# pydata/sparse

Hardware: AMD Instinct MI355X
Metric: GCXS x dense SpMM throughput (GFLOP/s) (higher is better)
Workload: dtype f32; 1 GPU; GCXS(CSR) 1000000x10000 @ 0.01 (100000000 nnz, int32 idx) in 1 nnz-balanced row block(s) x dense 10000x128 fp32; world_size=1, rows_rank0=1000000, idx_dtype=int32, parallelism=row-block x1, mul_add=fma, nan_warning=deferred, prewarm_products=40, default_settings=NAN_WARNING="sync" (verdict read inside every product), kernel=spmm_tiled (cached block stream)

## Files before the change

sparse_amd/_kernels.py:

```python
import os

import numpy as np
import torch

from . import _ffi
from ._device import code_of, np_dtype, ptr, require_hip, stream_ptr, torch_dtype


def dot_dtype(dt1, dt2):
    return (np.zeros((), dtype=np_dtype(dt1)) * np.zeros((), dtype=np_dtype(dt2))).dtype


_COMPLEX_CODE = {torch.complex64: _ffi.C64, torch.complex128: _ffi.C128}


def product_code(dt):
    dt = torch_dtype(dt)
    code = _COMPLEX_CODE.get(dt)
    return code_of(dt) if code is None else code


def _as_reals(t):
    return torch.view_as_real(t).reshape(-1) if t.is_complex() else t

# ... 1310 lines not shown

def csr_tiled_layout(a_data, a_indices, a_indptr, M, Kd, force_sort=False, dtype=None, defer_check=False, balance=None):
    dev = require_hip(a_data, a_indices, a_indptr)
    if dtype is None:
        dtype = a_data.dtype if a_data.dtype in TILED_DTYPES else torch.float32
    dtype = torch_dtype(dtype)
    vc = code_of(_tiled_layout_dtype(dtype))
    rg, kb, gpb, epb, slack, direct_max, _ = tiled_params(dtype)
    nnz = int(a_data.numel())
    ntiles = -(-Kd // kb)
    groups = -(-(-(-M // rg)) // gpb) * gpb
    nseg = groups * ntiles
    s = stream_ptr(dev)
    vals = a_data.to(dtype).contiguous()
    if dtype == torch.int32:
        vals = vals.view(torch.float32)
    if not index_dtype_ok(a_indices) or a_indices.dtype != a_indptr.dtype:
        a_indices, a_indptr = a_indices.to(torch.int64), a_indptr.to(torch.int64)

    def finish(blk_off, fill):
        total = int(blk_off[-1])
        if total >= 2 ** 31:
            raise ValueError("tiled SpMM layout: more than 2^31 blocks")
        blocks = torch.empty((total + slack) * 16, dtype=torch.int32, device=dev)
        fill(blk_off, total, blocks)
        return TiledLayout(blocks, convert(blk_off, torch.int32), dtype, total / max(nseg, 1))

    may_balance = (ntiles <= direct_max and not force_sort and TILED_ONE_PASS_INSPECTOR and TILED_BALANCE and balance is not False
                   and nnz >= TILED_BALANCE_MIN_NNZ and 0 < M < 2 ** 31)
    if may_balance and (balance or not defer_check):
        lay = _balanced_tiled_layout(vals, a_indices.contiguous(), a_indptr.contiguous(), M, Kd, dtype, nnz, defer_check, dev, s)
        if lay is not None:
            return lay
        may_balance = False
    if ntiles <= direct_max and not force_sort and TILED_ONE_PASS_INSPECTOR:
        ic = code_of(a_indices.dtype)
        ind, ptr_ = a_indices.contiguous(), a_indptr.contiguous()
        upper = -(-nnz // epb) + nseg
        if upper < 2 ** 31:
            blocks = torch.empty((upper + slack) * 16, dtype=torch.int32, device=dev)
            blk_off = torch.empty(groups * (ntiles + 1), dtype=torch.int32, device=dev)
            state = torch.empty(9, dtype=torch.int64, device=dev)
            _ffi.call("spamd_spmm_tiled_inspect", vc, ic, M, Kd, ptr(vals), ptr(ind), ptr(ptr_), ptr(state), ptr(blk_off),
                      ptr(blocks), s)
            if defer_check:
                lay = TiledLayout(blocks, blk_off, dtype, nnz / epb / max(nseg, 1) + 0.5, group_ends=True, pending=state)
                if may_balance:
                    _ffi.call("spamd_spmm_tiled_map_stats", ic, M, Kd, 32, ptr(ptr_), None, None, ptr(state) + 8, s)
                    lay.skew_mean = nnz * rg / max(M, 1)
                return lay
            if int(state[0]) == 0:
                return TiledLayout(blocks, blk_off, dtype, nnz / epb / max(nseg, 1) + 0.5, group_ends=True)
    elif ntiles <= direct_max and not force_sort:
        nblk = torch.empty(nseg + 1, dtype=torch.int64, device=dev)
        flags = torch.empty(1, dtype=torch.int32, device=dev)
        ic = code_of(a_indices.dtype)
        ind, ptr_ = a_indices.contiguous(), a_indptr.contiguous()
        _ffi.call("spamd_spmm_tiled_count", vc, ic, M, Kd, ptr(ind), ptr(ptr_), ptr(nblk), ptr(flags), s)
        blk_off = exclusive_scan(nblk)
        if int(flags[0]) == 0:
            return finish(blk_off, lambda bo, total, blocks: _ffi.call(
                "spamd_spmm_tiled_fill", vc, ic, M, Kd, ptr(vals), ptr(ind), ptr(ptr_), ptr(bo), total, ptr(blocks), s))
    rc = csr_to_keys(a_indptr, a_indices, M, Kd)
    tk = torch.empty_like(rc)
    _ffi.call("spamd_spmm_tiled_keys", nnz, ptr(rc), Kd, ptr(tk), s)
    del rc
    tk, vals = sort_key_value(tk, vals, max(nseg * rg * kb - 1, 1))
    seg_start = torch.empty(nseg + 1, dtype=torch.int64, device=dev)
    nblk = torch.empty(nseg + 1, dtype=torch.int64, device=dev)
    _ffi.call("spamd_spmm_tiled_lists", vc, nnz, ptr(tk), M, Kd, ptr(seg_start), ptr(nblk), s)
    return finish(exclusive_scan(nblk), lambda bo, total, blocks: _ffi.call(
        "spamd_spmm_tiled_pack", vc, nnz, ptr(tk), ptr(vals), ptr(seg_start), ptr(bo), total, ptr(blocks), s))


TILED_BALANCE = True
TILED_BALANCE_MIN_NNZ = 1 << 20
TILED_BALANCE_SKEW = 1.6
TILED_BALANCE_CAPMUL = 2
TILED_BALANCE_STATS = {}


def _balanced_tiled_layout(vals, ind, ptr_, M, Kd, dtype, nnz, defer_check, dev, s):
    rg, kb, gpb, epb, slack, direct_max, _ = tiled_params(dtype)
    ntiles = -(-Kd // kb)
    ic, vc = code_of(ind.dtype), code_of(_tiled_layout_dtype(dtype))
    mean_group = nnz * rg / max(M, 1)
    cap = 32
    while cap < TILED_BALANCE_CAPMUL * mean_group:
        cap *= 2
    stats = torch.empty(8, dtype=torch.int64, device=dev)
    _ffi.call("spamd_spmm_tiled_map_stats", ic, M, Kd, cap, ptr(ptr_), None, None, ptr(stats), s)
    st = stats.tolist()
    skew = st[6] / max(mean_group, 1.0)
    TILED_BALANCE_STATS.update(cap=cap, class_rows=st[:6], natural_max_group=st[6], skew=skew, balanced=False)
    if skew <= TILED_BALANCE_SKEW:
        return None
    keys = torch.empty(M, dtype=torch.int64, device=dev)
    rows = torch.empty(M, dtype=torch.int32, device=dev)
    _ffi.call("spamd_spmm_tiled_map_stats", ic, M, Kd, cap, ptr(ptr_), ptr(keys), ptr(rows), ptr(stats), s)
    st = stats.tolist()
    TILED_BALANCE_STATS.update(class_rows=st[:6])
    counts = _harr64(st[:6])
    groups = int(_ffi.lib().spamd_spmm_tiled_map_groups(counts))
    nseg = groups * ntiles
    upper = -(-nnz // epb) + nseg
    if groups <= 0 or upper >= 2 ** 31:
        return None
    keys, rows = sort_key_value(keys, rows, max(Kd, 1))
    rowmap = torch.empty(groups * rg + 16, dtype=torch.int32, device=dev)
    gload = torch.empty(groups + 1, dtype=torch.int64, device=dev)
    _ffi.call("spamd_spmm_tiled_map_build", ic, M, cap, ptr(ptr_), ptr(rows), counts, ptr(rowmap), ptr(gload), s)
    vstart = exclusive_scan(gload)
    blocks = torch.empty((upper + slack) * 16, dtype=torch.int32, device=dev)
    blk_off = torch.empty(groups * (ntiles + 1), dtype=torch.int32, device=dev)
    state = torch.empty(1, dtype=torch.int64, device=dev)
    _ffi.call("spamd_spmm_tiled_inspect_mapped", vc, ic, M, Kd, groups, ptr(vals), ptr(ind), ptr(ptr_), ptr(rowmap), ptr(vstart),
              ptr(state), ptr(blk_off), ptr(blocks), s)
    TILED_BALANCE_STATS.update(balanced=True, groups=groups)
    lay = TiledLayout(blocks, blk_off, dtype, nnz / epb / max(nseg, 1) + 0.5, group_ends=True, pending=state if defer_check else None,
                      rowmap=rowmap, groups=groups)
    if not defer_check and int(state[0]) != 0:
        return None
    return lay


def csc_tiled_layout(a_data, a_indices, a_indptr, M, Kd, dtype=None):
    dev = require_hip(a_data, a_indices, a_indptr)
    if dtype is None:
        dtype = a_data.dtype if a_data.dtype in TILED_DTYPES else torch.float32
    dtype = torch_dtype(dtype)
    rg, kb, gpb, epb, slack, direct_max, _ = tiled_params(dtype)
    nnz = int(a_data.numel())
    ntiles = -(-Kd // kb)
    groups = -(-(-(-M // rg)) // gpb) * gpb
    nseg = groups * ntiles
    upper = -(-nnz // epb) + nseg
    if ntiles > direct_max or upper >= 2 ** 31 or groups == 0 or not TILED_ONE_PASS_INSPECTOR:
        return None
    if not index_dtype_ok(a_indices) or a_indices.dtype != a_indptr.dtype:
        a_indices, a_indptr = a_indices.to(torch.int64), a_indptr.to(torch.int64)
    vals = a_data.to(dtype).contiguous()
    if dtype == torch.int32:
        vals = vals.view(torch.float32)
    blocks = torch.empty((upper + slack) * 16, dtype=torch.int32, device=dev)
    blk_off = torch.empty(groups * (ntiles + 1), dtype=torch.int32, device=dev)
    split = torch.empty(int(_ffi.lib().spamd_spmm_tiled_inspect_csc_ws(M, Kd)), dtype=torch.int32, device=dev)
    state = torch.empty(1, dtype=torch.int64, device=dev)
    _ffi.call("spamd_spmm_tiled_inspect_csc", code_of(_tiled_layout_dtype(dtype)), code_of(a_indices.dtype), M, Kd, ptr(vals),
              ptr(a_indices.contiguous()), ptr(a_indptr.contiguous()), ptr(split), ptr(state), ptr(blk_off), ptr(blocks),
              stream_ptr(dev))
    return TiledLayout(blocks, blk_off, dtype, nnz / epb / max(nseg, 1) + 0.5, group_ends=True, pending=state)


def dot_csr_ndarray_tiled(layout, out_shape, Kd, b, out=None, exact=False):
    blocks, blk_off, dtype = layout
    M, N = int(out_shape[0]), int(b.shape[1])
    Nout = int(out_shape[1])
    panel = 64 if dtype == torch.float64 else 128
    if N % panel or not (N - panel < Nout <= N):
        raise ValueError(f"tiled executor: B has {N} columns (whole {panel}-column panels expected), result {Nout}")
    last_cols = (Nout - (N - panel)) % panel
    dev = require_hip(blocks, blk_off, b)
    if b.dtype != dtype:
        raise TypeError(f"tiled layout holds {dtype} values, B is {b.dtype}")
    b = b.contiguous()
    if out is None:
        out = torch.empty((M, Nout), dtype=dtype, device=dev)
    lists = max(int(blk_off.numel()) - 1, 1)
    mean_blocks = getattr(layout, "mean_blocks", None) or (int(blocks.numel()) // 16) / lists
    hint = min(64, max(6, int(1.5 * mean_blocks) + 3))
    if _TOUCH_OVERRIDE:
        hint = _TOUCH_OVERRIDE
    ends = _ffi.TILED_GROUP_ENDS if getattr(layout, "group_ends", False) else 0
    ints = _ffi.TILED_INT32 if dtype == torch.int32 else 0
    flags = (_ffi.EXACT_MULADD if exact and not ints else 0) | ends | ints | (hint << 8) | (last_cols << 16)
    rowmap = getattr(layout, "rowmap", None)
    if rowmap is not None:
        _ffi.call("spamd_spmm_tiled_mapped", code_of(_tiled_layout_dtype(dtype)), M, int(layout.groups), Kd, N, ptr(blocks), ptr(blk_off),
                  ptr(rowmap), ptr(b), N, ptr(out), Nout, flags, stream_ptr(dev))
    else:
        _ffi.call("spamd_spmm_tiled", code_of(_tiled_layout_dtype(dtype)), M, Kd, N, ptr(blocks), ptr(blk_off), ptr(b), N, ptr(out), Nout,
                  flags, stream_ptr(dev))
    pending = getattr(layout, "pending", None)
    if pending is not None:
        layout.pending = None
        words = pending.tolist()
        mean = getattr(layout, "skew_mean", None)
        if mean and len(words) >= 8 and words[7] > TILED_BALANCE_SKEW * max(mean, 1.0):
            layout.rebalance = True
        if int(words[0]) != 0:
            raise UnsortedColumns("tiled layout built from rows with unsorted column indices")
    return out
```

sparse_amd/csrc/build.py:

```python
import concurrent.futures as cf
import glob
import os
import shutil
import subprocess
import sys

HERE = os.path.dirname(os.path.abspath(__file__))
PKG = os.path.dirname(HERE)
OUT_DIR = os.path.join(PKG, "_lib")
OBJ_DIR = os.path.join(OUT_DIR, "obj")
LIB = os.path.join(OUT_DIR, "libsparse_amd.so")
ARCH = "gfx950"
CXXFLAGS = [
    f"--offload-arch={ARCH}", "-O3", "-std=c++17", "-fPIC", "-ffp-contract=off",
    "-fno-gpu-rdc", "-Wall", "-Wno-unused-function", "-Wno-unused-variable",
]


def _hipcc():
    for c in (os.environ.get("HIPCC"), shutil.which("hipcc"), "/opt/rocm/bin/hipcc"):
        if c and os.path.exists(c):
            return c
    raise RuntimeError("hipcc not found (need ROCm to build libsparse_amd.so)")


def sources():
    return sorted(glob.glob(os.path.join(HERE, "*.hip")))


def _deps():
    return sorted(glob.glob(os.path.join(HERE, "*.h"))) + sorted(glob.glob(os.path.join(HERE, "*.inc"))) + [
        os.path.join(os.path.dirname(PKG), "include", "sparse_amd.h"), os.path.abspath(__file__)]


def is_stale():
    if not os.path.exists(LIB):
        return True
    t = os.path.getmtime(LIB)
    return any(os.path.getmtime(p) > t for p in sources() + _deps())


def _own_deps(src, obj):
    dep = obj[:-2] + ".d"
    if not os.path.exists(dep):
        return _deps()
    words = open(dep).read().replace("\\\n", " ").split()
    files = [w for w in words[1:] if not w.startswith("/opt/") and not w.startswith("/usr/")]
    if any(not os.path.exists(f) for f in files):
        return _deps()
    return files + [os.path.abspath(__file__)]


NO_SPILL = {"spmm_tiled.hip": "spmm_tiled_kernel"}


def _spills(remarks, needle):
    out, name, sg = [], None, 0
    for ln in remarks.splitlines():
        if "Function Name:" in ln:
            name = ln.split("Function Name:")[1].split()[0]
        elif "SGPRs Spill:" in ln:
            sg = int(ln.split("SGPRs Spill:")[1].split()[0])
        elif "VGPRs Spill:" in ln and name is not None:
            vg = int(ln.split("VGPRs Spill:")[1].split()[0])
            if needle in name and (sg or vg):
                out.append((name, sg, vg))
    return out


def _compile(src, force):
    obj = os.path.join(OBJ_DIR, os.path.basename(src)[:-4] + ".o")
    newest = max(os.path.getmtime(p) for p in [src] + _own_deps(src, obj))
    if not force and os.path.exists(obj) and os.path.getmtime(obj) >= newest:
        return obj, ""
    needle = NO_SPILL.get(os.path.basename(src))
    extra = ["-Rpass-analysis=kernel-resource-usage"] if needle else []
    cmd = [_hipcc(), *CXXFLAGS, *extra, "-MD", "-MF", obj[:-2] + ".d", "-c", src, "-o", obj]
    r = subprocess.run(cmd, capture_output=True, text=True)
    if r.returncode != 0:
        raise RuntimeError(f"hipcc failed for {src}:\n{' '.join(cmd)}\n{r.stdout}\n{r.stderr}")
    if needle:
        bad = _spills(r.stderr, needle)
        if bad:
            os.remove(obj)
            raise RuntimeError(f"{os.path.basename(src)}: the compiler spilled registers in " +
                               ", ".join(f"{n[:60]} ({s} SGPR, {v} VGPR)" for n, s, v in bad[:4]) +
                               " - refused (see NO_SPILL in sparse_amd/csrc/build.py)")
        return obj, "\n".join(ln for ln in r.stderr.splitlines() if "-Rpass-analysis" not in ln and "remark:" not in ln)
    return obj, r.stderr


def build(force=False, verbose=False, jobs=None):
    if not force and not is_stale():
        return LIB
    os.makedirs(OBJ_DIR, exist_ok=True)
    srcs = sources()
    jobs = jobs or min(len(srcs), os.cpu_count() or 1)
    with cf.ThreadPoolExecutor(max_workers=jobs) as ex:
        results = list(ex.map(lambda s: _compile(s, force), srcs))
    objs = [o for o, _ in results]
    if verbose:
        for _, w in results:
            if w.strip():
                print(w, file=sys.stderr)
    cmd = [_hipcc(), f"--offload-arch={ARCH}", "-shared", "-fPIC", "-o", LIB + ".tmp", *objs]
    r = subprocess.run(cmd, capture_output=True, text=True)
    if r.returncode != 0:
        raise RuntimeError(f"link failed:\n{' '.join(cmd)}\n{r.stdout}\n{r.stderr}")
    os.replace(LIB + ".tmp", LIB)
    return LIB


if __name__ == "__main__":
    p = build(force="--force" in sys.argv, verbose=True)
    print(p)
```

sparse_amd/csrc/spmm_tiled.hip:

```cpp
#include "common.h"
#include "spmm_tiled_asm.inc"
#include <stdlib.h>
#include <mutex>
#include <set>

namespace spamd {

constexpr int TL_RG = TL_ASM_RG;
constexpr int TL_WAVES = TL_ASM_WAVES;
#ifndef SPAMD_TL_EXPERIMENTAL
static_assert(TL_RG == 35 && TL_WAVES == 16, "experimental tiled-SpMM geometry: build with -DSPAMD_TL_EXPERIMENTAL");
#endif
constexpr int TL_KB = TL_ASM_KB;
constexpr int TL_NBUF = 2;
__host__ __device__ constexpr int tl_d0(int lc, int lr) { return ((lc >> 1) << 11) | ((lc & 1) << 9) | (2 + 2 * lr); }
constexpr int TL_BLOCK_INTS = 16;

template <typename T>
struct TlFmt;
template <>
struct TlFmt<float> {
  static constexpr int EPB = 8, PANEL = 128;
  __device__ static void put(int* stream, int64_t entry, int d0, float v) {
    int* b = stream + (entry / EPB) * TL_BLOCK_INTS + (entry % EPB) * 2;
// ... 156 lines not shown
}

template <typename I, typename T, bool MAPPED>
__global__ void __launch_bounds__(256) tl_inspect_kernel(int64_t M, int ntiles, int64_t groups, const T* __restrict__ vals,
                                                         const I* __restrict__ indices, const I* __restrict__ indptr,
                                                         unsigned long long* __restrict__ state, int* __restrict__ blk_off,
                                                         int* __restrict__ stream, const int* __restrict__ rowmap,
                                                         const int64_t* __restrict__ vstart) {
  extern __shared__ int tl_fill_lds[];
  __shared__ __attribute__((aligned(16))) int64_t rsab[2 * (TL_RG + 1)];
  __shared__ int wtot[5];
  __shared__ int group_bad;
  constexpr int EPB = TlFmt<T>::EPB;
  int* const before = tl_fill_lds;
  int* const runstart = before + TL_RG * ntiles;
  int* const loff = runstart + TL_RG * ntiles;
  const int tid = threadIdx.x;
  const int64_t g = blockIdx.x;
  const int64_t r0 = g * TL_RG;
  if (tid < TL_RG) {
    if constexpr (MAPPED) {
      const int r = rowmap[r0 + tid];
      rsab[2 * (tid)] = r >= 0 ? (int64_t)indptr[r] : 0;
      rsab[2 * (tid) + 1] = r >= 0 ? (int64_t)indptr[r + 1] : 0;
    } else {
      const int64_t r = r0 + tid;
      rsab[2 * (tid)] = (int64_t)indptr[r < M ? r : M];
      rsab[2 * (tid) + 1] = (int64_t)indptr[r + 1 < M ? r + 1 : M];
    }
  }
  for (int i = tid; i < TL_RG * ntiles; i += 256) before[i] = 0;
  if (tid == 0) group_bad = 0;
  __syncthreads();
  const int64_t e0 = MAPPED ? vstart[g] : rsab[2 * (0)], e1 = MAPPED ? vstart[g + 1] : rsab[2 * (TL_RG - 1) + 1];
  bool bad = false;
  constexpr int RPW = (TL_RG + 3) / 4;
  constexpr int TL_PRE = 2;
  const int wv = tid >> 6, lane = tid & 63;
  unsigned cpre[RPW][TL_PRE];
  T vpre[RPW][TL_PRE];
#pragma unroll
  for (int i = 0; i < RPW; ++i) {
    const int lr = wv + 4 * i;
    const int64_t ra = lr < TL_RG ? rsab[2 * (lr)] : 0, rb = lr < TL_RG ? rsab[2 * (lr) + 1] : 0;
#pragma unroll
    for (int p = 0; p < TL_PRE; ++p) {
      const int64_t e = ra + lane + 64 * p;
      cpre[i][p] = e < rb ? (unsigned)indices[e] : 0xffffffffu;
      vpre[i][p] = e < rb ? vals[e] : T(0);
    }
  }
  auto count_one = [&](int lr, int64_t ra, int64_t e, unsigned c, unsigned cp, bool row_start) {
    const int t = (int)(c / (unsigned)TL_KB);
    atomicAdd(&before[lr * ntiles + t], 1);
    if (!row_start && cp > c) bad = true;
    if (row_start || (int)(cp / (unsigned)TL_KB) != t) runstart[lr * ntiles + t] = (int)(e - (MAPPED ? ra : e0));
  };
#pragma unroll
  for (int i = 0; i < RPW; ++i) {
    const int lr = wv + 4 * i;
    if (lr >= TL_RG) break;
    const int64_t ra = rsab[2 * (lr)], rb = rsab[2 * (lr) + 1];
#pragma unroll
    for (int p = 0; p < TL_PRE; ++p) {
      const int64_t e = ra + lane + 64 * p;
      const unsigned c = cpre[i][p];
      unsigned cp = (unsigned)__shfl_up((int)c, 1, 64);
      if (p > 0) {
        const unsigned last = (unsigned)__builtin_amdgcn_readlane((int)cpre[i][p > 0 ? p - 1 : 0], 63);
        if (lane == 0) cp = last;
      }
      if (e < rb) count_one(lr, ra, e, c, cp, p == 0 && lane == 0);
    }
    for (int64_t e = ra + lane + 64 * TL_PRE; e < rb; e += 64)
      count_one(lr, ra, e, (unsigned)indices[e], (unsigned)indices[e - 1], false);
  }
  if (bad) {
    atomicOr(&state[0], 1ull);
    group_bad = 1;
  }
  __syncthreads();
  int nb = 0, cnt_t = 0;
  for (int t = tid; t < ntiles; t += 256) {
    int c[TL_RG];
#pragma unroll
    for (int lr = 0; lr < TL_RG; ++lr) c[lr] = before[lr * ntiles + t];
    int run = 0;
#pragma unroll
    for (int lr = 0; lr < TL_RG; ++lr) {
      before[lr * ntiles + t] = run;
      run += c[lr];
    }
    cnt_t = run;
    nb = (run + EPB - 1) / EPB;
  }
  const int wid = wv;
  int x = nb;
#pragma unroll
  for (int d = 1; d < 64; d <<= 1) {
    const int y = __shfl_up(x, d, 64);
    if (lane >= d) x += y;
  }
  if (lane == 63) wtot[wid] = x;
  __syncthreads();
  int woff = 0;
  for (int w = 0; w < wid; ++w) woff += wtot[w];
  const int gtotal = wtot[0] + wtot[1] + wtot[2] + wtot[3];
  const int my_off = woff + x - nb;
  const int64_t goff = tl_group_first_block(e0, g, ntiles, EPB);
  const int64_t gnext = tl_group_first_block(e1, g + 1, ntiles, EPB);
  if (tid < ntiles) loff[tid] = my_off;
  __syncthreads();
  if (tid < ntiles) blk_off[g * (ntiles + 1) + tid] = (int)(goff + my_off);
  if (tid == 0) blk_off[g * (ntiles + 1) + ntiles] = (int)(goff + gtotal);
  for (int64_t i = (goff + gtotal) * TL_BLOCK_INTS + tid; i < gnext * TL_BLOCK_INTS; i += 256) stream[i] = 0;
  if (group_bad) {
    for (int64_t i = goff * TL_BLOCK_INTS + tid; i < (goff + gtotal) * TL_BLOCK_INTS; i += 256) stream[i] = 0;
    return;
  }
  auto fill_one = [&](int lr, int64_t ra, int64_t e, unsigned c, T v) {
    const int t = (int)(c / (unsigned)TL_KB);
    const int lc = (int)(c - (unsigned)t * (unsigned)TL_KB);
    const int64_t dst = (goff + loff[t]) * EPB + before[lr * ntiles + t] + ((int)(e - (MAPPED ? ra : e0)) - runstart[lr * ntiles + t]);
    TlFmt<T>::put(stream, dst, tl_d0(lc, lr), v);
  };
#pragma unroll
  for (int i = 0; i < RPW; ++i) {
    const int lr = wv + 4 * i;
    if (lr >= TL_RG) break;
    const int64_t ra = rsab[2 * (lr)], rb = rsab[2 * (lr) + 1];
#pragma unroll
    for (int p = 0; p < TL_PRE; ++p) {
      const int64_t e = ra + lane + 64 * p;
      if (e < rb) fill_one(lr, ra, e, cpre[i][p], vpre[i][p]);
    }
    for (int64_t e = ra + lane + 64 * TL_PRE; e < rb; e += 64) fill_one(lr, ra, e, (unsigned)indices[e], vals[e]);
  }
  if (tid < ntiles) {
    const int64_t first = (goff + my_off) * EPB;
    for (int i = cnt_t; i < nb * EPB; ++i) TlFmt<T>::put(stream, first + i, 0, T(0));
  }
}

__device__ __forceinline__ void tl_dma16(unsigned lds_base, const void* src) {
  asm volatile("s_mov_b32 m0, %0\n\ts_nop 0\n\tglobal_load_lds_dwordx4 %1, off"
               :
               : "s"(lds_base), "v"(src)
               : "memory", "m0");
}

template <int MODE>
__device__ __forceinline__ void tl_phases(const int* stream, int t0, int te, int o0, int o1, int o2, int offreg, int obase,
                                          int ntiles, int nfull, int toff, int mask, unsigned m0wave,
                                          unsigned row_step, int voff, tl_srd_t srd, unsigned& soff) {
  const int lane = threadIdx.x & 63;
  const unsigned blo = (unsigned)((uintptr_t)stream & 0xffffffffu), bhi = (unsigned)((uintptr_t)stream >> 32);
  const int lane8 = lane * 8;
#define TL_PHASES_OPERANDS                                                                                        \
  [soff] "+s"(soff)                                                                                               \
  : [blo] "s"(blo), [bhi] "s"(bhi), [t0] "s"(t0), [te] "s"(te), [o0] "s"(o0), [o1] "s"(o1), [o2] "s"(o2),         \
    [obase] "s"(obase), [ntiles] "s"(ntiles), [nfull] "s"(nfull), [m0wave] "s"(m0wave), [step] "s"(row_step),      \
    [toff] "v"(toff), [lane8] "v"(lane8), [mask] "v"(mask), [offreg] "v"(offreg), [voff] "v"(voff), [srd] "s"(srd)  \
  : "memory", "m0", "scc", "vcc", TL_CLOB_SGPR, TL_CLOB_TMP, TL_CLOB_ACC
  if (MODE == 6)
    asm volatile(TL_ASM_PHASES_I32 : TL_PHASES_OPERANDS);
  else if (MODE == 4)
    asm volatile(TL_ASM_PHASES_F64 : TL_PHASES_OPERANDS);
  else if (MODE == 5)
    asm volatile(TL_ASM_PHASES_F64_EXACT : TL_PHASES_OPERANDS);
  else if (MODE == 3)
    asm volatile(TL_ASM_PHASES_EXACT : TL_PHASES_OPERANDS);
  else if (MODE == 1)
    asm volatile(TL_ASM_PHASES_NOFMA : TL_PHASES_OPERANDS);
  else if (MODE == 2)
    asm volatile(TL_ASM_PHASES_NOLDS : TL_PHASES_OPERANDS);
  else
    asm volatile(TL_ASM_PHASES : TL_PHASES_OPERANDS);
#undef TL_PHASES_OPERANDS
}

__device__ __forceinline__ void tl_block_map(unsigned L, int npanels, int nblocks, int& bx, int& by) {
  const unsigned pin = npanels > 1 ? 2u : 1u;
  const unsigned per_chunk = (unsigned)((nblocks + 7) / 8) * 8u * pin;
  const unsigned chunk = L / per_chunk, l = L % per_chunk;
  const unsigned seq = l >> 3;
  by = uniform((int)(chunk * pin + seq % pin));
  bx = uniform((int)((seq / pin) * 8u + (l & 7u)));
}

template <int DBG, int MODE, typename T>
__global__ void __launch_bounds__(TL_WAVES * 64) __attribute__((amdgpu_num_vgpr(TL_ASM_COMP)))
spmm_tiled_kernel(int64_t M, int64_t K, int ntiles, int touch_lines, const int* __restrict__ stream,
                  const int* __restrict__ blk_off, const T* __restrict__ b, int64_t ldb,
                  T* __restrict__ out, int64_t ldo, int last_cols, int npanels, int nblocks, const int* __restrict__ rowmap) {
  constexpr int PANEL = TlFmt<T>::PANEL;
  constexpr int CPL = PANEL / 64;
  extern __shared__ __attribute__((aligned(16))) char lds[];
  const int tid = threadIdx.x;
  const int lane = tid & 63;
  const int wv = uniform(tid >> 6);
  int bx, by;
  tl_block_map(blockIdx.x, npanels, nblocks, bx, by);
  if (bx >= nblocks || by >= npanels) return;
  const int g = bx * TL_WAVES + wv;
  b += (int64_t)by * PANEL;
  out += (int64_t)by * PANEL;

  asm volatile(TL_ASM_ZERO ::: "memory", TL_CLOB_ACC);

  const int nfull = DBG == 2 ? 0 : (int)(K / TL_KB);
  const unsigned row_step = (unsigned)((2 * TL_WAVES) * ldb * (int64_t)sizeof(T));
  const unsigned m0wave = (unsigned)wv * 2048u;
  const uint64_t bbase = (uint64_t)(uintptr_t)b;
  tl_srd_t srd;
  srd[0] = (int)(bbase & 0xffffffffu);
  srd[1] = (int)((bbase >> 32) & 0xffffu);
  srd[2] = (int)0xffffffffu;
  srd[3] = 0x00020000;
  const int voff = (int)((int64_t)(tid >> 5) * ldb * (int64_t)sizeof(T)) + (tid & 31) * 16;
  unsigned soff = 0;
  auto issue_partial = [&](int t) {
#pragma unroll
    for (int i = 0; i < TL_DMA_PER_TILE; ++i) {
      const int e = (i * (TL_WAVES * 64) + tid) * 16;
      int64_t r = (int64_t)t * TL_KB + (e >> 9);
      if (r >= K) r = K - 1;
      tl_dma16(((unsigned)(i * TL_WAVES + wv) * 2u + (unsigned)(t & 1)) * 1024u,
               reinterpret_cast<const char*>(b + r * ldb) + (e & 511));
    }
  };
  const bool has_partial = DBG != 2 && (int64_t)nfull * TL_KB < K;

  if (nfull > 0)
    asm volatile(TL_ASM_TILE0 : [soff] "+s"(soff) : [m0wave] "s"(m0wave), [step] "s"(row_step), [voff] "v"(voff), [srd] "s"(srd) : "memory", "m0", "scc", "vcc", "s89");
  else if (has_partial)
    issue_partial(0);
  asm volatile("s_waitcnt vmcnt(0)" ::: "memory");
  __syncthreads();

  const int* const myoff = blk_off + (int64_t)g * (ntiles + (touch_lines >> 16));
  touch_lines &= 0xffff;
  const int toff = (lane < touch_lines ? lane : touch_lines - 1) * 64;
  int t = 0;
  while (t < ntiles) {
    const int obase = t;
    const int q = obase + lane;
    int offreg = myoff[q < ntiles ? q : ntiles];
    asm volatile("" : "+v"(offreg));
    int te = obase + 61 < ntiles ? obase + 61 : ntiles;
    if (has_partial && t < nfull - 1 && nfull - 1 < te) te = nfull - 1;
    if (has_partial && t == nfull - 1) issue_partial(nfull);
    auto o = [&](int tt) { return wave_bcast(offreg, (tt < ntiles ? tt : ntiles) - obase); };
    const int o0 = o(t), o1 = o(t + 1), o2 = o(t + 2);
    if (t == 0) {
      const int n = o2 - o0, l = lane < n ? lane : 0;
      asm volatile("global_load_dword " TL_ASM_TOUCH ", %0, off" ::"v"(reinterpret_cast<const char*>(stream + (int64_t)o0 * 16) + l * 64)
                   : "memory", TL_ASM_TOUCH);
    }
    tl_phases<MODE>(stream, t, te, o0, o1, o2, offreg, obase, ntiles, nfull, toff, (int)0xfffffe00, m0wave, row_step, voff, srd, soff);
    t = te;
  }
  asm volatile("s_waitcnt vmcnt(0) lgkmcnt(0)" ::: "memory");

  const int64_t row0 = (int64_t)g * TL_RG;
  const int64_t left = M - row0;
  const int nvalid = left <= 0 ? 0 : (left < TL_RG ? (int)left : TL_RG);
  T* const obase_p = out + row0 * ldo + lane * CPL;
  const int64_t stride_bytes = ldo * (int64_t)sizeof(T);
  int bx2, by2;
  tl_block_map(blockIdx.x, npanels, nblocks, bx2, by2);
  const int ncols = (last_cols > 0 && by2 == npanels - 1) ? last_cols : PANEL;
  if (rowmap) {
    const int* const rm = rowmap + (int64_t)g * TL_RG;
    T* const base_p = out + lane * CPL;
    if (lane * CPL + CPL <= ncols)
      asm volatile(TL_ASM_STORE_PERM
                   :
                   : [lo] "v"((unsigned)((uintptr_t)base_p & 0xffffffffu)), [hi] "v"((unsigned)((uintptr_t)base_p >> 32)),
                     [stride] "s"((unsigned)stride_bytes), [rm] "s"(rm)
                   : "memory", "scc", TL_CLOB_SGPR, TL_CLOB_TMP, TL_CLOB_ACC);
    if constexpr (CPL == 2) {
      if (lane * CPL + 1 == ncols)
        asm volatile(TL_ASM_STORE1_PERM
                     :
                     : [lo] "v"((unsigned)((uintptr_t)base_p & 0xffffffffu)), [hi] "v"((unsigned)((uintptr_t)base_p >> 32)),
                       [stride] "s"((unsigned)stride_bytes), [rm] "s"(rm)
                     : "memory", "scc", TL_CLOB_SGPR, TL_CLOB_TMP);
    }
    return;
  }
  if (lane * CPL + CPL <= ncols)
    asm volatile(TL_ASM_STORE
                 :
                 : [lo] "v"((unsigned)((uintptr_t)obase_p & 0xffffffffu)), [hi] "v"((unsigned)((uintptr_t)obase_p >> 32)),
                   [stride] "s"(stride_bytes), [n] "s"(nvalid)
                 : "memory", "scc", "s36", TL_ASM_BASE, TL_ASM_TOUCH, TL_CLOB_ACC);
  if constexpr (CPL == 2) {
    if (lane * CPL + 1 == ncols)
      asm volatile(TL_ASM_STORE1
                   :
                   : [lo] "v"((unsigned)((uintptr_t)obase_p & 0xffffffffu)), [hi] "v"((unsigned)((uintptr_t)obase_p >> 32)),
                     [stride] "s"(stride_bytes), [n] "s"(nvalid)
                   : "memory", "scc", "s36", TL_ASM_BASE, TL_ASM_TOUCH);
  }
}

static int64_t tl_grid_groups(int64_t M) { return ceil_div(ceil_div(M, (int64_t)TL_RG), (int64_t)TL_WAVES) * TL_WAVES; }

}

using namespace spamd;

static int tl_epb(int val_dtype) { return val_dtype == SPAMD_F32 ? TlFmt<float>::EPB : (val_dtype == SPAMD_F64 ? TlFmt<double>::EPB : 0); }

extern "C" int spamd_spmm_tiled_params(int val_dtype, int* rows_per_group, int* tile_rows, int* groups_per_block,
                                       int* entries_per_block, int* slack_blocks, int* direct_max_tiles,
                                       int* panel_cols) {
  if (!tl_epb(val_dtype)) return SPAMD_ETYPE;
  if (direct_max_tiles) *direct_max_tiles = TL_DIRECT_MAX_TILES;
  if (rows_per_group) *rows_per_group = TL_RG;
  if (tile_rows) *tile_rows = TL_KB;
  if (groups_per_block) *groups_per_block = TL_WAVES;
  if (entries_per_block) *entries_per_block = tl_epb(val_dtype);
  if (slack_blocks) *slack_blocks = TL_SLACK_BLOCKS;
  if (panel_cols) *panel_cols = val_dtype == SPAMD_F32 ? TlFmt<float>::PANEL : TlFmt<double>::PANEL;
  return 0;
}

static unsigned tl_blocks_for(int64_t n) {
  int64_t blocks = ceil_div(n, (int64_t)256);
  if (blocks > 8192) blocks = 8192;
  if (blocks < 1) blocks = 1;
  return (unsigned)blocks;
}

extern "C" int spamd_spmm_tiled_keys(int64_t nnz, const int64_t* rowcol_keys, int64_t K, int64_t* tiled_keys,
                                     void* stream) {
  if (nnz < 0 || K <= 0) return SPAMD_EINVAL;
  if (nnz == 0) return 0;
  hipLaunchKernelGGL(tl_keys_kernel, dim3(tl_blocks_for(nnz)), dim3(256), 0, (hipStream_t)stream, rowcol_keys, nnz, K,
                     ceil_div(K, (int64_t)TL_KB), tiled_keys);
  return launch_status();
}

extern "C" int spamd_spmm_tiled_lists(int val_dtype, int64_t nnz, const int64_t* tiled_keys_sorted, int64_t M, int64_t K,
                                      int64_t* seg_start, int64_t* nblk, void* stream) {
  if (nnz < 0 || M < 0 || K <= 0) return SPAMD_EINVAL;
  if (!tl_epb(val_dtype)) return SPAMD_ETYPE;
  const int64_t nseg = tl_grid_groups(M) * ceil_div(K, (int64_t)TL_KB);
  hipLaunchKernelGGL(tl_seg_start_kernel, dim3(tl_blocks_for(nnz + 1)), dim3(256), 0, (hipStream_t)stream,
                     tiled_keys_sorted, nnz, nseg, seg_start);
  hipLaunchKernelGGL(tl_blocks_kernel, dim3(tl_blocks_for(nseg + 1)), dim3(256), 0, (hipStream_t)stream, seg_start,
                     nseg, tl_epb(val_dtype), nblk);
  return launch_status();
}

static int tl_clear_blocks(int64_t total_blocks, int* blocks, hipStream_t s) {
  return (int)hipMemsetAsync(blocks, 0, (size_t)(total_blocks + TL_SLACK_BLOCKS) * TL_BLOCK_INTS * sizeof(int), s);
}

extern "C" int spamd_spmm_tiled_pack(int val_dtype, int64_t nnz, const int64_t* tiled_keys_sorted, const void* vals_sorted,
                                     const int64_t* seg_start, const int64_t* blk_off, int64_t total_blocks,
                                     int* blocks, void* stream) {
  if (nnz < 0 || total_blocks < 0) return SPAMD_EINVAL;
  if (!tl_epb(val_dtype)) return SPAMD_ETYPE;
  int rc = tl_clear_blocks(total_blocks, blocks, (hipStream_t)stream);
  if (rc) return rc;
  if (nnz == 0) return 0;
  if (val_dtype == SPAMD_F32)
    hipLaunchKernelGGL(tl_pack_kernel<float>, dim3(tl_blocks_for(nnz)), dim3(256), 0, (hipStream_t)stream, tiled_keys_sorted,
                       (const float*)vals_sorted, nnz, seg_start, blk_off, blocks);
  else
    hipLaunchKernelGGL(tl_pack_kernel<double>, dim3(tl_blocks_for(nnz)), dim3(256), 0, (hipStream_t)stream, tiled_keys_sorted,
                       (const double*)vals_sorted, nnz, seg_start, blk_off, blocks);
  return launch_status();
}

extern "C" int spamd_spmm_tiled_count(int val_dtype, int idx_dtype, int64_t M, int64_t K, const void* a_indices,
                                      const void* a_indptr, int64_t* nblk, int* flags, void* stream) {
  if (M < 0 || K <= 0) return SPAMD_EINVAL;
  if (!tl_epb(val_dtype)) return SPAMD_ETYPE;
  const int64_t ntiles = ceil_div(K, (int64_t)TL_KB);
  if (ntiles > TL_DIRECT_MAX_TILES) return SPAMD_EINVAL;
  const int64_t groups = tl_grid_groups(M);
  hipError_t e = hipMemsetAsync(flags, 0, sizeof(int), (hipStream_t)stream);
  if (e != hipSuccess) return (int)e;
  e = hipMemsetAsync(nblk + groups * ntiles, 0, sizeof(int64_t), (hipStream_t)stream);
  if (e != hipSuccess) return (int)e;
  if (groups == 0) return 0;
  SPAMD_DISPATCH_IDX(idx_dtype, I, hipLaunchKernelGGL(tl_count_kernel<I>, dim3((unsigned)groups), dim3(256), 0,
                                                    (hipStream_t)stream, M, (int)ntiles, tl_epb(val_dtype),
                                                    (const I*)a_indices, (const I*)a_indptr, nblk, flags))
  return launch_status();
}

template <typename I, typename T>
static int tl_launch_fill(int64_t M, int64_t ntiles, const T* a_data, const I* a_indices, const I* a_indptr,
                          const int64_t* blk_off, int* blocks, hipStream_t s) {
  const int lds = (int)(2 * TL_RG * ntiles * sizeof(int));
  auto kern = &tl_fill_kernel<I, T>;
  if (lds > 48 * 1024) {
    hipError_t e = hipFuncSetAttribute(reinterpret_cast<const void*>(kern), hipFuncAttributeMaxDynamicSharedMemorySize, lds);
    if (e != hipSuccess) return (int)e;
  }
  hipLaunchKernelGGL(kern, dim3((unsigned)tl_grid_groups(M)), dim3(256), lds, s, M, (int)ntiles, a_data, a_indices, a_indptr,
                     blk_off, blocks);
  return launch_status();
}

extern "C" int spamd_spmm_tiled_fill(int val_dtype, int idx_dtype, int64_t M, int64_t K, const void* a_data,
                                     const void* a_indices, const void* a_indptr, const int64_t* blk_off,
                                     int64_t total_blocks, int* blocks, void* stream) {
  if (M < 0 || K <= 0 || total_blocks < 0) return SPAMD_EINVAL;
  if (!tl_epb(val_dtype)) return SPAMD_ETYPE;
  const int64_t ntiles = ceil_div(K, (int64_t)TL_KB);
  if (ntiles > TL_DIRECT_MAX_TILES) return SPAMD_EINVAL;
  int rc = tl_clear_blocks(total_blocks, blocks, (hipStream_t)stream);
  if (rc) return rc;
  if (tl_grid_groups(M) == 0) return 0;
  SPAMD_DISPATCH_IDX(idx_dtype, I, {
    if (val_dtype == SPAMD_F32)
      return tl_launch_fill<I, float>(M, ntiles, (const float*)a_data, (const I*)a_indices, (const I*)a_indptr, blk_off,
                                      blocks, (hipStream_t)stream);
    return tl_launch_fill<I, double>(M, ntiles, (const double*)a_data, (const I*)a_indices, (const I*)a_indptr, blk_off,
                                     blocks, (hipStream_t)stream);
  })
  return SPAMD_ETYPE;
}

template <typename I, typename T>
static int tl_launch_inspect(int64_t M, int64_t ntiles, const T* a_data, const I* a_indices, const I* a_indptr,
                             unsigned long long* state, int* blk_off, int* blocks, hipStream_t s, int64_t map_groups = 0,
                             const int* rowmap = nullptr, const int64_t* vstart = nullptr) {
  const int64_t groups = rowmap ? map_groups : tl_grid_groups(M);
  const int lds = (int)((2 * TL_RG * ntiles + ntiles + 1) * sizeof(int));
  auto kern = rowmap ? &tl_inspect_kernel<I, T, true> : &tl_inspect_kernel<I, T, false>;
  if (lds > 48 * 1024) {
    hipError_t e = hipFuncSetAttribute(reinterpret_cast<const void*>(kern), hipFuncAttributeMaxDynamicSharedMemorySize, lds);
    if (e != hipSuccess) return (int)e;
  }
  hipLaunchKernelGGL(kern, dim3((unsigned)groups), dim3(256), lds, s, M, (int)ntiles, groups, a_data, a_indices, a_indptr,
                     state, blk_off, blocks, rowmap, vstart);
  return launch_status();
}

constexpr int TL_MAP_CLASSES = 6;
__host__ __device__ inline int tl_map_slots(int c) { return c == 5 ? TL_RG : (1 << c); }
__host__ __device__ inline int tl_map_class(int64_t len, int64_t cap) {
  return len > cap / 2 ? 0 : (len > cap / 4 ? 1 : (len > cap / 8 ? 2 : (len > cap / 16 ? 3 : (len > cap / 32 ? 4 : 5))));
}

template <typename I>
__global__ void __launch_bounds__(256) tl_map_stats_kernel(int64_t M, int64_t cap, int64_t maxlen, const I* __restrict__ indptr,
                                                           int64_t* __restrict__ keys, int* __restrict__ rows,
                                                           unsigned long long* __restrict__ stats) {
  __shared__ unsigned cnt[TL_MAP_CLASSES];
// ... 616 lines not shown
        if (ch == 0) {
          tbase[gi] += all;
          const int nb = (tbase[gi] + EPB - 1) / EPB;
          static_assert(GPB == 16, "a DPP row");
          unsigned x = (unsigned)nb;
          x += dpp_shift0<0x111, 0xf>(x);
          x += dpp_shift0<0x112, 0xf>(x);
          x += dpp_shift0<0x114, 0xf>(x);
          x += dpp_shift0<0x118, 0xf>(x);
          ib[gi] = (int)x - nb;
          if (gi == GPB - 1) tsum_s = x;
        }
      }
      __syncthreads();
      const bool img_path = total <= TL_CSC_STAGE && tsum_s <= TL_CSC_IMG_BLOCKS;
      if (img_path) {
        for (int i = tid; i < tsum_s * TL_BLOCK_INTS; i += 256) img[i] = 0;
        __syncthreads();
      }
#if SPAMD_CSC_ABL == 5
      if (false)
#endif
#pragma unroll
      for (int p = 0; p < PER; ++p) {
        const int k = w0 + tid + 256 * p;
        if (k < w1) {
          const int gi = grp[p], lr = rr[p] - gi * TL_RG;
          const int pos = ccnt[(wv + 4 * p) * GPB + gi] + rank[p];
          if (img_path) {
            const int q = pos / EPB, slot = pos - q * EPB;
            const int base = (ib[gi] + q) * TL_BLOCK_INTS;
            const int d0 = tl_d0(col[p], lr);
            bdst[ib[gi] + q] = gbase[gi] + q;
            if constexpr (sizeof(T) == 4) {
              typedef int int2v __attribute__((ext_vector_type(2)));
              int2v ent;
              ent.x = d0;
              ent.y = __builtin_bit_cast(int, vv[p]);
              *reinterpret_cast<int2v*>(&img[base + slot * 2]) = ent;
            } else {
              img[base + slot] = d0;
              *reinterpret_cast<long long*>(&img[base + 6 + 2 * slot]) = __builtin_bit_cast(long long, vv[p]);
            }
          } else {
            const int64_t dst = (int64_t)gbase[gi] * EPB + pos;
            TlFmt<T>::put(stream, dst, tl_d0(col[p], lr), vv[p]);
          }
        }
      }
      __syncthreads();
#pragma unroll
      for (int p = 0; p < PER; ++p) asm volatile("" ::"v"(vv[p]), "v"(rr[p]));
      take();
      if (img_path && SPAMD_CSC_ABL != 5) {
        typedef int int4v __attribute__((ext_vector_type(4)));
        const int nvec = tsum_s * (TL_BLOCK_INTS / 4);
        for (int i = tid; i < nvec; i += 256) {
          const int64_t dst = (int64_t)bdst[i >> 2] * TL_BLOCK_INTS + (i & 3) * 4;
#if SPAMD_CSC_ABL == 1
          if (bdst[i >> 2] == 0x7fffffff)
#endif
          *reinterpret_cast<int4v*>(stream + dst) = *reinterpret_cast<const int4v*>(&img[i * 4]);
        }
        __syncthreads();
        padded = true;
      }
    }
    if (!padded && tid < GPB) {
      const int c = tbase[tid], nb = (c + EPB - 1) / EPB;
      const int64_t first = (goff_s[tid] + lo16[tid]) * EPB;
      for (int q = c; q < nb * EPB; ++q) TlFmt<T>::put(stream, first + q, 0, T(0));
    }
    __syncthreads();
  }
}

template <typename I, typename T>
static int tl_launch_inspect_csc(int64_t M, int64_t K, int64_t ntiles, const T* a_data, const I* a_indices, const I* a_indptr,
                                 int* ws, unsigned long long* state, int* blk_off, int* blocks, hipStream_t s) {
  const int64_t groups = tl_grid_groups(M);
  const int64_t nblocks = groups / TL_WAVES;
  if (nblocks >= ((int64_t)1 << 31)) return SPAMD_EINVAL;
  const bool hist = groups <= TL_CSC_HIST_GROUPS;
  int* const split = ws;
  int* const cnt = split + (nblocks + 1) * K;
  int* const rel = cnt + TL_CSC_HIST_PARTS * groups * ntiles;
  const int64_t words = ((nblocks + 1) * K + TL_CSC_HIST_PARTS * groups * ntiles + groups * (ntiles + 1) + 1) & ~(int64_t)1;
  unsigned long long* const look = reinterpret_cast<unsigned long long*>(ws + words);
  long long* const e0 = reinterpret_cast<long long*>(look) + groups;
  const int64_t owgs = ceil_div(groups, (int64_t)64);
  const int nlook = (int)(owgs + 2);
  static_assert(TL_WAVES >= 3, "groups (a multiple of TL_WAVES) >= ceil(groups / 64) + 2");
  if (!hist) {
    const unsigned sgrid = (unsigned)std::min<int64_t>(K, (int64_t)256 * 64);
    hipLaunchKernelGGL((tl_csc_split_kernel<I>), dim3(sgrid), dim3(256), 0, s, M, K, nblocks, a_indices, a_indptr, split, state, look, nlook);
  }
  const dim3 grid((unsigned)nblocks, (unsigned)ceil_div(ntiles, (int64_t)TL_CSC_TC));
  if (hist) {
    auto hk = &tl_csc_hist_kernel<I>;
    const int lds = (int)((groups + 1) / 2 * sizeof(int));
    if (lds > 48 * 1024) {
      hipError_t e = hipFuncSetAttribute(reinterpret_cast<const void*>(hk), hipFuncAttributeMaxDynamicSharedMemorySize, lds);
      if (e != hipSuccess) return (int)e;
    }
    hipLaunchKernelGGL(hk, dim3((unsigned)ntiles, TL_CSC_HIST_PARTS), dim3(1024), lds, s, M, K, (int)ntiles, groups, nblocks,
                       a_indices, a_indptr, cnt, split, state, look, nlook);
  } else {
    hipLaunchKernelGGL((tl_csc_count_kernel<I>), grid, dim3(256), 0, s, K, (int)ntiles, nblocks, groups, a_indices, a_indptr, (const int*)split,
                       (const unsigned long long*)state, cnt);
  }
  if (hist)
    hipLaunchKernelGGL((tl_csc_offsets_kernel<TlFmt<T>::EPB, TL_CSC_HIST_PARTS>), dim3((unsigned)owgs), dim3(64), 0, s,
                       groups, (int)ntiles, (const int*)cnt, (const unsigned long long*)state, rel, look, e0);
  else
    hipLaunchKernelGGL((tl_csc_offsets_kernel<TlFmt<T>::EPB, 1>), dim3((unsigned)owgs), dim3(64), 0, s,
                       groups, (int)ntiles, (const int*)cnt, (const unsigned long long*)state, rel, look, e0);
  const int64_t fgrid = 8 * ceil_div(nblocks, (int64_t)8) * ceil_div(ntiles, (int64_t)TL_CSC_TC);
  if (fgrid >= ((int64_t)1 << 31)) return SPAMD_EINVAL;
  hipLaunchKernelGGL((tl_csc_fill_kernel<I, T>), dim3((unsigned)fgrid), dim3(256), 0, s, K, (int)ntiles, a_data, a_indices,
                     a_indptr, (const int*)split, (const unsigned long long*)state, (const int*)rel, (const long long*)e0, nblocks,
                     blk_off, blocks);
  return launch_status();
}

extern "C" int64_t spamd_spmm_tiled_inspect_csc_ws(int64_t M, int64_t K) {
  if (M < 0 || K <= 0) return -1;
  const int64_t ntiles = ceil_div(K, (int64_t)TL_KB), groups = tl_grid_groups(M), nblocks = groups / TL_WAVES;
  return (nblocks + 1) * K + TL_CSC_HIST_PARTS * groups * ntiles + groups * (ntiles + 1) + 2 + 2 * (2 * groups + 1) + 16;
}

extern "C" int spamd_spmm_tiled_inspect_csc(int val_dtype, int idx_dtype, int64_t M, int64_t K, const void* a_data,
                                            const void* a_indices, const void* a_indptr, int* ws, void* state, int* blk_off,
                                            int* blocks, void* stream) {
  if (M < 0 || K <= 0) return SPAMD_EINVAL;
  if (!tl_epb(val_dtype)) return SPAMD_ETYPE;
  if ((uintptr_t)ws % 8) return SPAMD_EINVAL;
  const int64_t ntiles = ceil_div(K, (int64_t)TL_KB);
  if (ntiles > TL_DIRECT_MAX_TILES) return SPAMD_EINVAL;
  hipError_t e = hipMemsetAsync(state, 0, sizeof(unsigned long long), (hipStream_t)stream);
  if (e != hipSuccess) return (int)e;
  if (tl_grid_groups(M) == 0) return 0;
  SPAMD_DISPATCH_IDX(idx_dtype, I, {
    if (val_dtype == SPAMD_F32)
      return tl_launch_inspect_csc<I, float>(M, K, ntiles, (const float*)a_data, (const I*)a_indices, (const I*)a_indptr, ws,
                                             (unsigned long long*)state, blk_off, blocks, (hipStream_t)stream);
    return tl_launch_inspect_csc<I, double>(M, K, ntiles, (const double*)a_data, (const I*)a_indices, (const I*)a_indptr, ws,
                                            (unsigned long long*)state, blk_off, blocks, (hipStream_t)stream);
  })
  return SPAMD_ETYPE;
}

static int tl_set_lds_once(const void* kern) { return set_max_dynamic_lds(kern, TL_LDS); }

template <typename T, typename KERN>
static int tl_launch(KERN kern, int64_t M, int64_t K, int64_t N, const int* blocks, const int* blk_off, const T* b,
                     int64_t ldb, T* out, int64_t ldo, int touch_lines, bool group_ends, int last_cols, hipStream_t s,
                     const int* rowmap = nullptr, int64_t map_groups = 0) {
  if (int rc = tl_set_lds_once(reinterpret_cast<const void*>(kern))) return rc;
  const int64_t blocks_n = (rowmap ? map_groups : tl_grid_groups(M)) / TL_WAVES;
  const int64_t npanels = N / TlFmt<T>::PANEL;
  const int64_t grid = ceil_div(blocks_n, (int64_t)8) * 8 * (npanels > 1 ? ceil_div(npanels, (int64_t)2) * 2 : 1);
  if (grid >= ((int64_t)1 << 31) || blocks_n >= ((int64_t)1 << 31)) return SPAMD_EINVAL;
  hipLaunchKernelGGL(kern, dim3((unsigned)grid), dim3(TL_WAVES * 64), TL_LDS, s, M, K,
                     (int)ceil_div(K, (int64_t)TL_KB), touch_lines | (group_ends ? 1 << 16 : 0), blocks, blk_off, b, ldb, out, ldo,
                     last_cols, (int)npanels, (int)blocks_n, rowmap);
  return launch_status();
}

static int tl_product(int val_dtype, int64_t M, int64_t K, int64_t N, const int* blocks, const int* blk_off, const void* b,
                      int64_t ldb, void* out, int64_t ldo, unsigned flags, void* stream, const int* rowmap, int64_t map_groups);

extern "C" int spamd_spmm_tiled(int val_dtype, int64_t M, int64_t K, int64_t N, const int* blocks, const int* blk_off,
                                const void* b, int64_t ldb, void* out, int64_t ldo, unsigned flags, void* stream) {
  return tl_product(val_dtype, M, K, N, blocks, blk_off, b, ldb, out, ldo, flags, stream, nullptr, 0);
}

extern "C" int spamd_spmm_tiled_mapped(int val_dtype, int64_t M, int64_t groups, int64_t K, int64_t N, const int* blocks,
                                       const int* blk_off, const int* rowmap, const void* b, int64_t ldb, void* out, int64_t ldo,
                                       unsigned flags, void* stream) {
  if (!rowmap || groups <= 0 || groups % TL_WAVES) return SPAMD_EINVAL;
  if (ldo * (val_dtype == SPAMD_F32 ? 4 : 8) >= ((int64_t)1 << 32)) return SPAMD_EINVAL;
  return tl_product(val_dtype, M, K, N, blocks, blk_off, b, ldb, out, ldo, flags | SPAMD_TILED_GROUP_ENDS, stream, rowmap, groups);
}

static int tl_product(int val_dtype, int64_t M, int64_t K, int64_t N, const int* blocks, const int* blk_off, const void* b,
                      int64_t ldb, void* out, int64_t ldo, unsigned flags, void* stream, const int* rowmap, int64_t map_groups) {
  if (!tl_epb(val_dtype)) return SPAMD_ETYPE;
  const int panel = val_dtype == SPAMD_F32 ? TlFmt<float>::PANEL : TlFmt<double>::PANEL;
  const int esz = val_dtype == SPAMD_F32 ? 4 : 8;
  if (M < 0 || K <= 0 || N <= 0 || N % panel != 0 || N / panel > 65535 || K / TL_KB >= ((int64_t)1 << 30)) return SPAMD_EINVAL;
  if (M == 0) return 0;
  if (((uintptr_t)b % 16) || ((ldb * esz) % 16) || ((uintptr_t)out % esz) || ((uintptr_t)blocks % 64))
    return SPAMD_EINVAL;
  if ((K + 2 * TL_KB) * ldb * esz >= ((int64_t)1 << 32)) return SPAMD_EINVAL;
  hipStream_t s = (hipStream_t)stream;
  const bool exact = (flags & SPAMD_EXACT_MULADD) != 0;
  const bool ends = (flags & SPAMD_TILED_GROUP_ENDS) != 0;
  const bool i32 = (flags & SPAMD_TILED_INT32) != 0;
  if (i32 && val_dtype != SPAMD_F32) return SPAMD_EINVAL;
  const int last_cols = (int)((flags >> 16) & 0xffu);
  if (last_cols > panel) return SPAMD_EINVAL;
  if (ldo < N - panel + (last_cols ? last_cols : panel)) return SPAMD_EINVAL;
  int touch = (int)((flags >> 8) & 0xffu);
  if (touch == 0) touch = 12;
  if (touch > 64) touch = 64;
  if (val_dtype == SPAMD_F64) {
    const double* bb = (const double*)b;
    double* oo = (double*)out;
    return exact ? tl_launch<double>(&spmm_tiled_kernel<0, 5, double>, M, K, N, blocks, blk_off, bb, ldb, oo, ldo, touch, ends, last_cols, s, rowmap, map_groups)
                 : tl_launch<double>(&spmm_tiled_kernel<0, 4, double>, M, K, N, blocks, blk_off, bb, ldb, oo, ldo, touch, ends, last_cols, s, rowmap, map_groups);
  }
  const float* bb = (const float*)b;
  float* oo = (float*)out;
#ifdef SPAMD_TUNING
  const char* dbg_env = getenv("SPAMD_TILED_DBG");
  const int dbg = dbg_env ? atoi(dbg_env) : 0;
  if (dbg == 2) return tl_launch<float>(&spmm_tiled_kernel<2, 0, float>, M, K, N, blocks, blk_off, bb, ldb, oo, ldo, touch, ends, last_cols, s, rowmap, map_groups);
  if (dbg == 5) return tl_launch<float>(&spmm_tiled_kernel<0, 1, float>, M, K, N, blocks, blk_off, bb, ldb, oo, ldo, touch, ends, last_cols, s, rowmap, map_groups);
  if (dbg == 6) return tl_launch<float>(&spmm_tiled_kernel<0, 2, float>, M, K, N, blocks, blk_off, bb, ldb, oo, ldo, touch, ends, last_cols, s, rowmap, map_groups);
  if (dbg == 7) return tl_launch<float>(&spmm_tiled_kernel<2, 2, float>, M, K, N, blocks, blk_off, bb, ldb, oo, ldo, touch, ends, last_cols, s, rowmap, map_groups);
#endif
  if (i32) return tl_launch<float>(&spmm_tiled_kernel<0, 6, float>, M, K, N, blocks, blk_off, bb, ldb, oo, ldo, touch, ends, last_cols, s, rowmap, map_groups);
  return exact ? tl_launch<float>(&spmm_tiled_kernel<0, 3, float>, M, K, N, blocks, blk_off, bb, ldb, oo, ldo, touch, ends, last_cols, s, rowmap, map_groups)
               : tl_launch<float>(&spmm_tiled_kernel<0, 0, float>, M, K, N, blocks, blk_off, bb, ldb, oo, ldo, touch, ends, last_cols, s, rowmap, map_groups);
}
```

sparse_amd/csrc/spmm_tiled_asm.inc:

```

#define TL_ASM_KB 160
#define TL_ASM_DMA_PER_TILE 5
#define TL_ASM_RG 35
#define TL_ASM_WAVES 16
#define TL_ASM_COMP 22
#define TL_ASM_TOUCH "v23"
#define TL_ASM_BASE "v22"

#define TL_ASM_PHASES \
  "s_mov_b32 s39, 0\n\t" \
  "s_mov_b32 s90, %[t0]\n\t" \
  "s_mov_b32 s91, %[o0]\n\t" \
  "s_mov_b32 s92, %[o1]\n\t" \
  "s_mov_b32 s93, %[o2]\n\t" \
  "s_add_u32 s88, s90, 1\n\t" \
  "s_and_b32 s88, s88, 1\n\t" \
  "s_lshl_b32 s88, s88, 10\n\t" \
  "s_add_u32 s89, s88, %[m0wave]\n\t" \
  "s_and_b32 s88, s90, 1\n\t" \
  "s_lshl_b32 s88, s88, 10\n\t" \
  "v_or_b32 v22, s88, %[lane8]\n\t" \
  "s_lshl_b32 s36, s91, 6\n\t" \
  "s_lshr_b32 s37, s91, 26\n\t" \
  "s_add_u32 s36, s36, %[blo]\n\t" \
  "s_addc_u32 s37, s37, %[bhi]\n\t" \
  "s_sub_u32 s88, s92, s91\n\t" \
  "s_cmp_lt_u32 s88, 3\n\t" \
  "s_cbranch_scc1 22f\n\t" \
  "s_load_dwordx16 s[40:55], s[36:37], 0x0\n\t" \
  "s_load_dwordx16 s[56:71], s[36:37], 0x40\n\t" \
  "s_load_dwordx16 s[72:87], s[36:37], 0x80\n\t" \
  "20:\n\t" \
  "1:\n\t" \
  "s_sub_u32 s38, s92, s91\n\t" \
  "s_add_u32 s88, s90, 1\n\t" \
  "s_cmp_lt_u32 s88, %[nfull]\n\t" \
  "s_cselect_b64 vcc, 31, 0\n\t" \
  "s_cmp_eq_u32 s38, 0\n\t" \
  "s_cbranch_scc1 12f\n\t" \
  "s_cbranch_vccz 6f\n\t" \
  "s_mov_b32 m0, s89\n\t" \
  "s_add_u32 s89, s89, 0x8000\n\t" \
  "buffer_load_dwordx4 %[voff], %[srd], %[soff] offen lds\n\t" \
  "s_add_u32 %[soff], %[soff], %[step]\n\t" \
  "s_lshr_b64 vcc, vcc, 1\n\t" \
  "6:\n\t" \
  "s_cbranch_vccz 6f\n\t" \
  "s_mov_b32 m0, s89\n\t" \
  "s_add_u32 s89, s89, 0x8000\n\t" \
  "buffer_load_dwordx4 %[voff], %[srd], %[soff] offen lds\n\t" \
  "s_add_u32 %[soff], %[soff], %[step]\n\t" \
  "s_lshr_b64 vcc, vcc, 1\n\t" \
  "6:\n\t" \
  "s_waitcnt lgkmcnt(0)\n\t" \
  "v_and_or_b32 v40, s40, %[mask], v22\n\t" \
  "v_and_or_b32 v42, s42, %[mask], v22\n\t" \
  "v_and_or_b32 v44, s44, %[mask], v22\n\t" \
  "v_and_or_b32 v46, s46, %[mask], v22\n\t" \
  "ds_read_b64 v[40:41], v40\n\t" \
  "ds_read_b64 v[42:43], v42\n\t" \
  "ds_read_b64 v[44:45], v44\n\t" \
  "ds_read_b64 v[46:47], v46\n\t" \
  "v_and_or_b32 v48, s48, %[mask], v22\n\t" \
  "v_and_or_b32 v50, s50, %[mask], v22\n\t" \
  "v_and_or_b32 v52, s52, %[mask], v22\n\t" \
  "v_and_or_b32 v54, s54, %[mask], v22\n\t" \
  "ds_read_b64 v[48:49], v48\n\t" \
  "ds_read_b64 v[50:51], v50\n\t" \
  "ds_read_b64 v[52:53], v52\n\t" \
  "ds_read_b64 v[54:55], v54\n\t" \
  "s_waitcnt lgkmcnt(0)\n\t" \
  "s_cmp_lt_u32 s38, 4\n\t" \
  "s_cbranch_scc1 40f\n\t" \
  "s_sub_u32 s38, s38, 3\n\t" \
  "11:\n\t" \
  "s_sub_u32 s38, s38, 1\n\t" \
  "s_cbranch_scc1 30f\n\t" \
  "v_and_or_b32 v24, s56, %[mask], v22\n\t" \
  "v_and_or_b32 v26, s58, %[mask], v22\n\t" \
  "v_and_or_b32 v28, s60, %[mask], v22\n\t" \
  "v_and_or_b32 v30, s62, %[mask], v22\n\t" \
  "ds_read_b64 v[24:25], v24\n\t" \
  "ds_read_b64 v[26:27], v26\n\t" \
  "ds_read_b64 v[28:29], v28\n\t" \
  "ds_read_b64 v[30:31], v30\n\t" \
  "v_and_or_b32 v32, s64, %[mask], v22\n\t" \
  "v_and_or_b32 v34, s66, %[mask], v22\n\t" \
  "v_and_or_b32 v36, s68, %[mask], v22\n\t" \
  "v_and_or_b32 v38, s70, %[mask], v22\n\t" \
  "ds_read_b64 v[32:33], v32\n\t" \
  "ds_read_b64 v[34:35], v34\n\t" \
  "ds_read_b64 v[36:37], v36\n\t" \
  "ds_read_b64 v[38:39], v38\n\t" \
  "s_set_gpr_idx_on s40, gpr_idx(SRC2,DST)\n\t" \
  "v_pk_fma_f32 v[56:57], v[40:41], s[40:41], v[56:57] op_sel:[0,1,0] op_sel_hi:[1,1,1]\n\t" \
  "s_set_gpr_idx_idx s42\n\t" \
  "v_pk_fma_f32 v[56:57], v[42:43], s[42:43], v[56:57] op_sel:[0,1,0] op_sel_hi:[1,1,1]\n\t" \
  "s_set_gpr_idx_idx s44\n\t" \
  "v_pk_fma_f32 v[56:57], v[44:45], s[44:45], v[56:57] op_sel:[0,1,0] op_sel_hi:[1,1,1]\n\t" \
  "s_set_gpr_idx_idx s46\n\t" \
  "v_pk_fma_f32 v[56:57], v[46:47], s[46:47], v[56:57] op_sel:[0,1,0] op_sel_hi:[1,1,1]\n\t" \
  "s_set_gpr_idx_idx s48\n\t" \
  "v_pk_fma_f32 v[56:57], v[48:49], s[48:49], v[56:57] op_sel:[0,1,0] op_sel_hi:[1,1,1]\n\t" \
  "s_set_gpr_idx_idx s50\n\t" \
  "v_pk_fma_f32 v[56:57], v[50:51], s[50:51], v[56:57] op_sel:[0,1,0] op_sel_hi:[1,1,1]\n\t" \
  "s_set_gpr_idx_idx s52\n\t" \
  "v_pk_fma_f32 v[56:57], v[52:53], s[52:53], v[56:57] op_sel:[0,1,0] op_sel_hi:[1,1,1]\n\t" \
  "s_set_gpr_idx_idx s54\n\t" \
  "v_pk_fma_f32 v[56:57], v[54:55], s[54:55], v[56:57] op_sel:[0,1,0] op_sel_hi:[1,1,1]\n\t" \
  "s_set_gpr_idx_off\n\t" \
  "s_waitcnt lgkmcnt(0)\n\t" \
  "s_load_dwordx16 s[40:55], s[36:37], 0xc0\n\t" \
  "s_cbranch_vccz 6f\n\t" \
  "s_mov_b32 m0, s89\n\t" \
  "s_add_u32 s89, s89, 0x8000\n\t" \
  "buffer_load_dwordx4 %[voff], %[srd], %[soff] offen lds\n\t" \
  "s_add_u32 %[soff], %[soff], %[step]\n\t" \
  "s_lshr_b64 vcc, vcc, 1\n\t" \
  "6:\n\t" \
  "s_sub_u32 s38, s38, 1\n\t" \
  "s_cbranch_scc1 31f\n\t" \
  "v_and_or_b32 v40, s72, %[mask], v22\n\t" \
  "v_and_or_b32 v42, s74, %[mask], v22\n\t" \
  "v_and_or_b32 v44, s76, %[mask], v22\n\t" \
  "v_and_or_b32 v46, s78, %[mask], v22\n\t" \
  "ds_read_b64 v[40:41], v40\n\t" \
  "ds_read_b64 v[42:43], v42\n\t" \
  "ds_read_b64 v[44:45], v44\n\t" \
  "ds_read_b64 v[46:47], v46\n\t" \
  "v_and_or_b32 v48, s80, %[mask], v22\n\t" \
  "v_and_or_b32 v50, s82, %[mask], v22\n\t" \
  "v_and_or_b32 v52, s84, %[mask], v22\n\t" \
  "v_and_or_b32 v54, s86, %[mask], v22\n\t" \
  "ds_read_b64 v[48:49], v48\n\t" \
  "ds_read_b64 v[50:51], v50\n\t" \
  "ds_read_b64 v[52:53], v52\n\t" \
  "ds_read_b64 v[54:55], v54\n\t" \
  "s_set_gpr_idx_on s56, gpr_idx(SRC2,DST)\n\t" \
  "v_pk_fma_f32 v[56:57], v[24:25], s[56:57], v[56:57] op_sel:[0,1,0] op_sel_hi:[1,1,1]\n\t" \
  "s_set_gpr_idx_idx s58\n\t" \
  "v_pk_fma_f32 v[56:57], v[26:27], s[58:59], v[56:57] op_sel:[0,1,0] op_sel_hi:[1,1,1]\n\t" \
  "s_set_gpr_idx_idx s60\n\t" \
  "v_pk_fma_f32 v[56:57], v[28:29], s[60:61], v[56:57] op_sel:[0,1,0] op_sel_hi:[1,1,1]\n\t" \
  "s_set_gpr_idx_idx s62\n\t" \
  "v_pk_fma_f32 v[56:57], v[30:31], s[62:63], v[56:57] op_sel:[0,1,0] op_sel_hi:[1,1,1]\n\t" \
  "s_set_gpr_idx_idx s64\n\t" \
  "v_pk_fma_f32 v[56:57], v[32:33], s[64:65], v[56:57] op_sel:[0,1,0] op_sel_hi:[1,1,1]\n\t" \
  "s_set_gpr_idx_idx s66\n\t" \
  "v_pk_fma_f32 v[56:57], v[34:35], s[66:67], v[56:57] op_sel:[0,1,0] op_sel_hi:[1,1,1]\n\t" \
  "s_set_gpr_idx_idx s68\n\t" \
  "v_pk_fma_f32 v[56:57], v[36:37], s[68:69], v[56:57] op_sel:[0,1,0] op_sel_hi:[1,1,1]\n\t" \
  "s_set_gpr_idx_idx s70\n\t" \
  "v_pk_fma_f32 v[56:57], v[38:39], s[70:71], v[56:57] op_sel:[0,1,0] op_sel_hi:[1,1,1]\n\t" \
  "s_set_gpr_idx_off\n\t" \
  "s_waitcnt lgkmcnt(0)\n\t" \
  "s_load_dwordx16 s[56:71], s[36:37], 0x100\n\t" \
  "s_cbranch_vccz 6f\n\t" \
  "s_mov_b32 m0, s89\n\t" \
  "s_add_u32 s89, s89, 0x8000\n\t" \
  "buffer_load_dwordx4 %[voff], %[srd], %[soff] offen lds\n\t" \
  "s_add_u32 %[soff], %[soff], %[step]\n\t" \
  "s_lshr_b64 vcc, vcc, 1\n\t" \
  "6:\n\t" \
  "s_sub_u32 s38, s38, 1\n\t" \
  "s_cbranch_scc1 32f\n\t" \
  "v_and_or_b32 v24, s40, %[mask], v22\n\t" \
  "v_and_or_b32 v26, s42, %[mask], v22\n\t" \
  "v_and_or_b32 v28, s44, %[mask], v22\n\t" \
  "v_and_or_b32 v30, s46, %[mask], v22\n\t" \
  "ds_read_b64 v[24:25], v24\n\t" \
  "ds_read_b64 v[26:27], v26\n\t" \
  "ds_read_b64 v[28:29], v28\n\t" \
// ... 762 lines not shown
  "s_set_gpr_idx_idx s54\n\t" \
  "v_pk_fma_f32 v[56:57], v[54:55], s[54:55], v[56:57] op_sel:[0,1,0] op_sel_hi:[1,1,1]\n\t" \
  "s_set_gpr_idx_off\n\t" \
  "s_waitcnt lgkmcnt(0)\n\t" \
  "s_cbranch_vccz 6f\n\t" \
  "s_mov_b32 m0, s89\n\t" \
  "s_add_u32 s89, s89, 0x8000\n\t" \
  "buffer_load_dwordx4 %[voff], %[srd], %[soff] offen lds\n\t" \
  "s_add_u32 %[soff], %[soff], %[step]\n\t" \
  "s_lshr_b64 vcc, vcc, 1\n\t" \
  "6:\n\t" \
  "s_cmp_lt_u32 s38, 2\n\t" \
  "s_cbranch_scc1 12f\n\t" \
  "s_cmp_lt_u32 s38, 3\n\t" \
  "s_cbranch_scc1 7f\n\t" \
  "v_and_or_b32 v40, s72, %[mask], v22\n\t" \
  "v_and_or_b32 v42, s74, %[mask], v22\n\t" \
  "v_and_or_b32 v44, s76, %[mask], v22\n\t" \
  "v_and_or_b32 v46, s78, %[mask], v22\n\t" \
  "ds_read_b64 v[40:41], v40\n\t" \
  "ds_read_b64 v[42:43], v42\n\t" \
  "ds_read_b64 v[44:45], v44\n\t" \
  "ds_read_b64 v[46:47], v46\n\t" \
  "v_and_or_b32 v48, s80, %[mask], v22\n\t" \
  "v_and_or_b32 v50, s82, %[mask], v22\n\t" \
  "v_and_or_b32 v52, s84, %[mask], v22\n\t" \
  "v_and_or_b32 v54, s86, %[mask], v22\n\t" \
  "ds_read_b64 v[48:49], v48\n\t" \
  "ds_read_b64 v[50:51], v50\n\t" \
  "ds_read_b64 v[52:53], v52\n\t" \
  "ds_read_b64 v[54:55], v54\n\t" \
  "7:\n\t" \
  "s_set_gpr_idx_on s56, gpr_idx(SRC2,DST)\n\t" \
  "v_pk_fma_f32 v[56:57], v[24:25], s[56:57], v[56:57] op_sel:[0,1,0] op_sel_hi:[1,1,1]\n\t" \
  "s_set_gpr_idx_idx s58\n\t" \
  "v_pk_fma_f32 v[56:57], v[26:27], s[58:59], v[56:57] op_sel:[0,1,0] op_sel_hi:[1,1,1]\n\t" \
  "s_set_gpr_idx_idx s60\n\t" \
  "v_pk_fma_f32 v[56:57], v[28:29], s[60:61], v[56:57] op_sel:[0,1,0] op_sel_hi:[1,1,1]\n\t" \
  "s_set_gpr_idx_idx s62\n\t" \
  "v_pk_fma_f32 v[56:57], v[30:31], s[62:63], v[56:57] op_sel:[0,1,0] op_sel_hi:[1,1,1]\n\t" \
  "s_set_gpr_idx_idx s64\n\t" \
  "v_pk_fma_f32 v[56:57], v[32:33], s[64:65], v[56:57] op_sel:[0,1,0] op_sel_hi:[1,1,1]\n\t" \
  "s_set_gpr_idx_idx s66\n\t" \
  "v_pk_fma_f32 v[56:57], v[34:35], s[66:67], v[56:57] op_sel:[0,1,0] op_sel_hi:[1,1,1]\n\t" \
  "s_set_gpr_idx_idx s68\n\t" \
  "v_pk_fma_f32 v[56:57], v[36:37], s[68:69], v[56:57] op_sel:[0,1,0] op_sel_hi:[1,1,1]\n\t" \
  "s_set_gpr_idx_idx s70\n\t" \
  "v_pk_fma_f32 v[56:57], v[38:39], s[70:71], v[56:57] op_sel:[0,1,0] op_sel_hi:[1,1,1]\n\t" \
  "s_set_gpr_idx_off\n\t" \
  "s_waitcnt lgkmcnt(0)\n\t" \
  "s_cbranch_vccz 6f\n\t" \
  "s_mov_b32 m0, s89\n\t" \
  "s_add_u32 s89, s89, 0x8000\n\t" \
  "buffer_load_dwordx4 %[voff], %[srd], %[soff] offen lds\n\t" \
  "s_add_u32 %[soff], %[soff], %[step]\n\t" \
  "s_lshr_b64 vcc, vcc, 1\n\t" \
  "6:\n\t" \
  "s_cmp_lt_u32 s38, 3\n\t" \
  "s_cbranch_scc1 12f\n\t" \
  "s_set_gpr_idx_on s72, gpr_idx(SRC2,DST)\n\t" \
  "v_pk_fma_f32 v[56:57], v[40:41], s[72:73], v[56:57] op_sel:[0,1,0] op_sel_hi:[1,1,1]\n\t" \
  "s_set_gpr_idx_idx s74\n\t" \
  "v_pk_fma_f32 v[56:57], v[42:43], s[74:75], v[56:57] op_sel:[0,1,0] op_sel_hi:[1,1,1]\n\t" \
  "s_set_gpr_idx_idx s76\n\t" \
  "v_pk_fma_f32 v[56:57], v[44:45], s[76:77], v[56:57] op_sel:[0,1,0] op_sel_hi:[1,1,1]\n\t" \
  "s_set_gpr_idx_idx s78\n\t" \
  "v_pk_fma_f32 v[56:57], v[46:47], s[78:79], v[56:57] op_sel:[0,1,0] op_sel_hi:[1,1,1]\n\t" \
  "s_set_gpr_idx_idx s80\n\t" \
  "v_pk_fma_f32 v[56:57], v[48:49], s[80:81], v[56:57] op_sel:[0,1,0] op_sel_hi:[1,1,1]\n\t" \
  "s_set_gpr_idx_idx s82\n\t" \
  "v_pk_fma_f32 v[56:57], v[50:51], s[82:83], v[56:57] op_sel:[0,1,0] op_sel_hi:[1,1,1]\n\t" \
  "s_set_gpr_idx_idx s84\n\t" \
  "v_pk_fma_f32 v[56:57], v[52:53], s[84:85], v[56:57] op_sel:[0,1,0] op_sel_hi:[1,1,1]\n\t" \
  "s_set_gpr_idx_idx s86\n\t" \
  "v_pk_fma_f32 v[56:57], v[54:55], s[86:87], v[56:57] op_sel:[0,1,0] op_sel_hi:[1,1,1]\n\t" \
  "s_set_gpr_idx_off\n\t" \
  "s_cbranch_vccz 6f\n\t" \
  "s_mov_b32 m0, s89\n\t" \
  "s_add_u32 s89, s89, 0x8000\n\t" \
  "buffer_load_dwordx4 %[voff], %[srd], %[soff] offen lds\n\t" \
  "s_add_u32 %[soff], %[soff], %[step]\n\t" \
  "s_lshr_b64 vcc, vcc, 1\n\t" \
  "6:\n\t" \
  "12:\n\t" \
  "13:\n\t" \
  "s_cbranch_vccz 14f\n\t" \
  "s_mov_b32 m0, s89\n\t" \
  "s_add_u32 s89, s89, 0x8000\n\t" \
  "buffer_load_dwordx4 %[voff], %[srd], %[soff] offen lds\n\t" \
  "s_add_u32 %[soff], %[soff], %[step]\n\t" \
  "s_lshr_b64 vcc, vcc, 1\n\t" \
  "s_branch 13b\n\t" \
  "14:\n\t" \
  "s_add_u32 s88, s90, 1\n\t" \
  "s_cmp_lt_u32 s88, %[te]\n\t" \
  "s_cbranch_scc0 21f\n\t" \
  "s_lshl_b32 s36, s92, 6\n\t" \
  "s_lshr_b32 s37, s92, 26\n\t" \
  "s_add_u32 s36, s36, %[blo]\n\t" \
  "s_addc_u32 s37, s37, %[bhi]\n\t" \
  "s_sub_u32 s88, s93, s92\n\t" \
  "s_cmp_lt_u32 s88, 3\n\t" \
  "s_cbranch_scc1 23f\n\t" \
  "s_load_dwordx16 s[40:55], s[36:37], 0x0\n\t" \
  "s_load_dwordx16 s[56:71], s[36:37], 0x40\n\t" \
  "s_load_dwordx16 s[72:87], s[36:37], 0x80\n\t" \
  "21:\n\t" \
  "s_add_u32 s38, s90, 3\n\t" \
  "s_min_u32 s38, s38, %[ntiles]\n\t" \
  "s_sub_u32 s38, s38, %[obase]\n\t" \
  "s_lshl_b32 s94, s93, 6\n\t" \
  "s_lshr_b32 s95, s93, 26\n\t" \
  "s_add_u32 s94, s94, %[blo]\n\t" \
  "s_addc_u32 s95, s95, %[bhi]\n\t" \
  "v_readlane_b32 s88, %[offreg], s38\n\t" \
  "s_mov_b32 s91, s92\n\t" \
  "s_mov_b32 s92, s93\n\t" \
  "v_xor_b32 v22, 0x400, v22\n\t" \
  "s_sub_u32 s89, s89, 0x28000\n\t" \
  "s_xor_b32 s89, s89, 0x400\n\t" \
  "global_load_dword v23, %[toff], s[94:95]\n\t" \
  "s_mov_b32 s93, s88\n\t" \
  "s_waitcnt vmcnt(1)\n\t" \
  "s_barrier\n\t" \
  "s_add_u32 s90, s90, 1\n\t" \
  "s_cmp_lt_u32 s90, %[te]\n\t" \
  "s_cbranch_scc1 1b\n\t" \
  "s_waitcnt lgkmcnt(0)\n\t" \
  "s_branch 29f\n\t" \
  "22:\n\t" \
  "s_cmp_eq_u32 s88, 0\n\t" \
  "s_cbranch_scc1 20b\n\t" \
  "s_load_dwordx16 s[40:55], s[36:37], 0x0\n\t" \
  "s_cmp_lt_u32 s88, 2\n\t" \
  "s_cbranch_scc1 20b\n\t" \
  "s_load_dwordx16 s[56:71], s[36:37], 0x40\n\t" \
  "s_branch 20b\n\t" \
  "23:\n\t" \
  "s_cmp_eq_u32 s88, 0\n\t" \
  "s_cbranch_scc1 21b\n\t" \
  "s_load_dwordx16 s[40:55], s[36:37], 0x0\n\t" \
  "s_cmp_lt_u32 s88, 2\n\t" \
  "s_cbranch_scc1 21b\n\t" \
  "s_load_dwordx16 s[56:71], s[36:37], 0x40\n\t" \
  "s_branch 21b\n\t" \
  "29:\n\t"

#define TL_ASM_PHASES_EXACT \
  "s_mov_b32 s39, 0\n\t" \
  "s_mov_b32 s90, %[t0]\n\t" \
  "s_mov_b32 s91, %[o0]\n\t" \
  "s_mov_b32 s92, %[o1]\n\t" \
  "s_mov_b32 s93, %[o2]\n\t" \
  "s_add_u32 s88, s90, 1\n\t" \
  "s_and_b32 s88, s88, 1\n\t" \
  "s_lshl_b32 s88, s88, 10\n\t" \
  "s_add_u32 s89, s88, %[m0wave]\n\t" \
  "s_and_b32 s88, s90, 1\n\t" \
  "s_lshl_b32 s88, s88, 10\n\t" \
  "v_or_b32 v22, s88, %[lane8]\n\t" \
  "s_lshl_b32 s36, s91, 6\n\t" \
  "s_lshr_b32 s37, s91, 26\n\t" \
  "s_add_u32 s36, s36, %[blo]\n\t" \
  "s_addc_u32 s37, s37, %[bhi]\n\t" \
  "s_sub_u32 s88, s92, s91\n\t" \
  "s_cmp_lt_u32 s88, 3\n\t" \
  "s_cbranch_scc1 22f\n\t" \
  "s_load_dwordx16 s[40:55], s[36:37], 0x0\n\t" \
  "s_load_dwordx16 s[56:71], s[36:37], 0x40\n\t" \
  "s_load_dwordx16 s[72:87], s[36:37], 0x80\n\t" \
  "20:\n\t" \
  "1:\n\t" \
  "s_sub_u32 s38, s92, s91\n\t" \
  "s_add_u32 s88, s90, 1\n\t" \
  "s_cmp_lt_u32 s88, %[nfull]\n\t" \
  "s_cselect_b64 vcc, 31, 0\n\t" \
  "s_cmp_eq_u32 s38, 0\n\t" \
  "s_cbranch_scc1 12f\n\t" \
  "s_cbranch_vccz 6f\n\t" \
  "s_mov_b32 m0, s89\n\t" \
  "s_add_u32 s89, s89, 0x8000\n\t" \
  "buffer_load_dwordx4 %[voff], %[srd], %[soff] offen lds\n\t" \
  "s_add_u32 %[soff], %[soff], %[step]\n\t" \
  "s_lshr_b64 vcc, vcc, 1\n\t" \
  "6:\n\t" \
  "s_cbranch_vccz 6f\n\t" \
  "s_mov_b32 m0, s89\n\t" \
  "s_add_u32 s89, s89, 0x8000\n\t" \
  "buffer_load_dwordx4 %[voff], %[srd], %[soff] offen lds\n\t" \
  "s_add_u32 %[soff], %[soff], %[step]\n\t" \
  "s_lshr_b64 vcc, vcc, 1\n\t" \
  "6:\n\t" \
  "s_waitcnt lgkmcnt(0)\n\t" \
  "v_and_or_b32 v40, s40, %[mask], v22\n\t" \
  "v_and_or_b32 v42, s42, %[mask], v22\n\t" \
  "v_and_or_b32 v44, s44, %[mask], v22\n\t" \
  "v_and_or_b32 v46, s46, %[mask], v22\n\t" \
  "ds_read_b64 v[40:41], v40\n\t" \
  "ds_read_b64 v[42:43], v42\n\t" \
  "ds_read_b64 v[44:45], v44\n\t" \
  "ds_read_b64 v[46:47], v46\n\t" \
  "v_and_or_b32 v48, s48, %[mask], v22\n\t" \
  "v_and_or_b32 v50, s50, %[mask], v22\n\t" \
  "v_and_or_b32 v52, s52, %[mask], v22\n\t" \
  "v_and_or_b32 v54, s54, %[mask], v22\n\t" \
  "ds_read_b64 v[48:49], v48\n\t" \
  "ds_read_b64 v[50:51], v50\n\t" \
  "ds_read_b64 v[52:53], v52\n\t" \
  "ds_read_b64 v[54:55], v54\n\t" \
  "s_waitcnt lgkmcnt(0)\n\t" \
  "s_cmp_lt_u32 s38, 4\n\t" \
  "s_cbranch_scc1 40f\n\t" \
  "s_sub_u32 s38, s38, 3\n\t" \
  "11:\n\t" \
  "s_sub_u32 s38, s38, 1\n\t" \
  "s_cbranch_scc1 30f\n\t" \
  "v_and_or_b32 v24, s56, %[mask], v22\n\t" \
  "v_and_or_b32 v26, s58, %[mask], v22\n\t" \
  "v_and_or_b32 v28, s60, %[mask], v22\n\t" \
  "v_and_or_b32 v30, s62, %[mask], v22\n\t" \
  "ds_read_b64 v[24:25], v24\n\t" \
  "ds_read_b64 v[26:27], v26\n\t" \
  "ds_read_b64 v[28:29], v28\n\t" \
  "ds_read_b64 v[30:31], v30\n\t" \
  "v_and_or_b32 v32, s64, %[mask], v22\n\t" \
  "v_and_or_b32 v34, s66, %[mask], v22\n\t" \
  "v_and_or_b32 v36, s68, %[mask], v22\n\t" \
  "v_and_or_b32 v38, s70, %[mask], v22\n\t" \
  "ds_read_b64 v[32:33], v32\n\t" \
  "ds_read_b64 v[34:35], v34\n\t" \
  "ds_read_b64 v[36:37], v36\n\t" \
  "ds_read_b64 v[38:39], v38\n\t" \
  "v_pk_mul_f32 v[40:41], v[40:41], s[40:41] op_sel:[0,1] op_sel_hi:[1,1]\n\t" \
  "v_pk_mul_f32 v[42:43], v[42:43], s[42:43] op_sel:[0,1] op_sel_hi:[1,1]\n\t" \
  "v_pk_mul_f32 v[44:45], v[44:45], s[44:45] op_sel:[0,1] op_sel_hi:[1,1]\n\t" \
  "v_pk_mul_f32 v[46:47], v[46:47], s[46:47] op_sel:[0,1] op_sel_hi:[1,1]\n\t" \
  "v_pk_mul_f32 v[48:49], v[48:49], s[48:49] op_sel:[0,1] op_sel_hi:[1,1]\n\t" \
  "v_pk_mul_f32 v[50:51], v[50:51], s[50:51] op_sel:[0,1] op_sel_hi:[1,1]\n\t" \
  "v_pk_mul_f32 v[52:53], v[52:53], s[52:53] op_sel:[0,1] op_sel_hi:[1,1]\n\t" \
  "v_pk_mul_f32 v[54:55], v[54:55], s[54:55] op_sel:[0,1] op_sel_hi:[1,1]\n\t" \
  "s_set_gpr_idx_on s40, gpr_idx(SRC1,DST)\n\t" \
  "v_pk_add_f32 v[56:57], v[40:41], v[56:57]\n\t" \
  "s_set_gpr_idx_idx s42\n\t" \
  "v_pk_add_f32 v[56:57], v[42:43], v[56:57]\n\t" \
  "s_set_gpr_idx_idx s44\n\t" \
  "v_pk_add_f32 v[56:57], v[44:45], v[56:57]\n\t" \
  "s_set_gpr_idx_idx s46\n\t" \
  "v_pk_add_f32 v[56:57], v[46:47], v[56:57]\n\t" \
  "s_set_gpr_idx_idx s48\n\t" \
  "v_pk_add_f32 v[56:57], v[48:49], v[56:57]\n\t" \
  "s_set_gpr_idx_idx s50\n\t" \
  "v_pk_add_f32 v[56:57], v[50:51], v[56:57]\n\t" \
  "s_set_gpr_idx_idx s52\n\t" \
  "v_pk_add_f32 v[56:57], v[52:53], v[56:57]\n\t" \
  "s_set_gpr_idx_idx s54\n\t" \
  "v_pk_add_f32 v[56:57], v[54:55], v[56:57]\n\t" \
  "s_set_gpr_idx_off\n\t" \
  "s_waitcnt lgkmcnt(0)\n\t" \
  "s_load_dwordx16 s[40:55], s[36:37], 0xc0\n\t" \
  "s_cbranch_vccz 6f\n\t" \
  "s_mov_b32 m0, s89\n\t" \
  "s_add_u32 s89, s89, 0x8000\n\t" \
  "buffer_load_dwordx4 %[voff], %[srd], %[soff] offen lds\n\t" \
  "s_add_u32 %[soff], %[soff], %[step]\n\t" \
  "s_lshr_b64 vcc, vcc, 1\n\t" \
  "6:\n\t" \
  "s_sub_u32 s38, s38, 1\n\t" \
  "s_cbranch_scc1 31f\n\t" \
  "v_and_or_b32 v40, s72, %[mask], v22\n\t" \
  "v_and_or_b32 v42, s74, %[mask], v22\n\t" \
  "v_and_or_b32 v44, s76, %[mask], v22\n\t" \
  "v_and_or_b32 v46, s78, %[mask], v22\n\t" \
  "ds_read_b64 v[40:41], v40\n\t" \
  "ds_read_b64 v[42:43], v42\n\t" \
  "ds_read_b64 v[44:45], v44\n\t" \
  "ds_read_b64 v[46:47], v46\n\t" \
  "v_and_or_b32 v48, s80, %[mask], v22\n\t" \
  "v_and_or_b32 v50, s82, %[mask], v22\n\t" \
  "v_and_or_b32 v52, s84, %[mask], v22\n\t" \
  "v_and_or_b32 v54, s86, %[mask], v22\n\t" \
  "ds_read_b64 v[48:49], v48\n\t" \
  "ds_read_b64 v[50:51], v50\n\t" \
  "ds_read_b64 v[52:53], v52\n\t" \
  "ds_read_b64 v[54:55], v54\n\t" \
  "v_pk_mul_f32 v[24:25], v[24:25], s[56:57] op_sel:[0,1] op_sel_hi:[1,1]\n\t" \
  "v_pk_mul_f32 v[26:27], v[26:27], s[58:59] op_sel:[0,1] op_sel_hi:[1,1]\n\t" \
  "v_pk_mul_f32 v[28:29], v[28:29], s[60:61] op_sel:[0,1] op_sel_hi:[1,1]\n\t" \
  "v_pk_mul_f32 v[30:31], v[30:31], s[62:63] op_sel:[0,1] op_sel_hi:[1,1]\n\t" \
  "v_pk_mul_f32 v[32:33], v[32:33], s[64:65] op_sel:[0,1] op_sel_hi:[1,1]\n\t" \
  "v_pk_mul_f32 v[34:35], v[34:35], s[66:67] op_sel:[0,1] op_sel_hi:[1,1]\n\t" \
  "v_pk_mul_f32 v[36:37], v[36:37], s[68:69] op_sel:[0,1] op_sel_hi:[1,1]\n\t" \
  "v_pk_mul_f32 v[38:39], v[38:39], s[70:71] op_sel:[0,1] op_sel_hi:[1,1]\n\t" \
  "s_set_gpr_idx_on s56, gpr_idx(SRC1,DST)\n\t" \
  "v_pk_add_f32 v[56:57], v[24:25], v[56:57]\n\t" \
  "s_set_gpr_idx_idx s58\n\t" \
  "v_pk_add_f32 v[56:57], v[26:27], v[56:57]\n\t" \
  "s_set_gpr_idx_idx s60\n\t" \
  "v_pk_add_f32 v[56:57], v[28:29], v[56:57]\n\t" \
  "s_set_gpr_idx_idx s62\n\t" \
  "v_pk_add_f32 v[56:57], v[30:31], v[56:57]\n\t" \
  "s_set_gpr_idx_idx s64\n\t" \
  "v_pk_add_f32 v[56:57], v[32:33], v[56:57]\n\t" \
  "s_set_gpr_idx_idx s66\n\t" \
  "v_pk_add_f32 v[56:57], v[34:35], v[56:57]\n\t" \
  "s_set_gpr_idx_idx s68\n\t" \
  "v_pk_add_f32 v[56:57], v[36:37], v[56:57]\n\t" \
  "s_set_gpr_idx_idx s70\n\t" \
  "v_pk_add_f32 v[56:57], v[38:39], v[56:57]\n\t" \
  "s_set_gpr_idx_off\n\t" \
  "s_waitcnt lgkmcnt(0)\n\t" \
  "s_load_dwordx16 s[56:71], s[36:37], 0x100\n\t" \
// ... 996 lines not shown
  "v_and_or_b32 v42, s74, %[mask], v22\n\t" \
  "v_and_or_b32 v44, s76, %[mask], v22\n\t" \
  "v_and_or_b32 v46, s78, %[mask], v22\n\t" \
  "ds_read_b64 v[40:41], v40\n\t" \
  "ds_read_b64 v[42:43], v42\n\t" \
  "ds_read_b64 v[44:45], v44\n\t" \
  "ds_read_b64 v[46:47], v46\n\t" \
  "v_and_or_b32 v48, s80, %[mask], v22\n\t" \
  "v_and_or_b32 v50, s82, %[mask], v22\n\t" \
  "v_and_or_b32 v52, s84, %[mask], v22\n\t" \
  "v_and_or_b32 v54, s86, %[mask], v22\n\t" \
  "ds_read_b64 v[48:49], v48\n\t" \
  "ds_read_b64 v[50:51], v50\n\t" \
  "ds_read_b64 v[52:53], v52\n\t" \
  "ds_read_b64 v[54:55], v54\n\t" \
  "7:\n\t" \
  "v_pk_mul_f32 v[24:25], v[24:25], s[56:57] op_sel:[0,1] op_sel_hi:[1,1]\n\t" \
  "v_pk_mul_f32 v[26:27], v[26:27], s[58:59] op_sel:[0,1] op_sel_hi:[1,1]\n\t" \
  "v_pk_mul_f32 v[28:29], v[28:29], s[60:61] op_sel:[0,1] op_sel_hi:[1,1]\n\t" \
  "v_pk_mul_f32 v[30:31], v[30:31], s[62:63] op_sel:[0,1] op_sel_hi:[1,1]\n\t" \
  "v_pk_mul_f32 v[32:33], v[32:33], s[64:65] op_sel:[0,1] op_sel_hi:[1,1]\n\t" \
  "v_pk_mul_f32 v[34:35], v[34:35], s[66:67] op_sel:[0,1] op_sel_hi:[1,1]\n\t" \
  "v_pk_mul_f32 v[36:37], v[36:37], s[68:69] op_sel:[0,1] op_sel_hi:[1,1]\n\t" \
  "v_pk_mul_f32 v[38:39], v[38:39], s[70:71] op_sel:[0,1] op_sel_hi:[1,1]\n\t" \
  "s_set_gpr_idx_on s56, gpr_idx(SRC1,DST)\n\t" \
  "v_pk_add_f32 v[56:57], v[24:25], v[56:57]\n\t" \
  "s_set_gpr_idx_idx s58\n\t" \
  "v_pk_add_f32 v[56:57], v[26:27], v[56:57]\n\t" \
  "s_set_gpr_idx_idx s60\n\t" \
  "v_pk_add_f32 v[56:57], v[28:29], v[56:57]\n\t" \
  "s_set_gpr_idx_idx s62\n\t" \
  "v_pk_add_f32 v[56:57], v[30:31], v[56:57]\n\t" \
  "s_set_gpr_idx_idx s64\n\t" \
  "v_pk_add_f32 v[56:57], v[32:33], v[56:57]\n\t" \
  "s_set_gpr_idx_idx s66\n\t" \
  "v_pk_add_f32 v[56:57], v[34:35], v[56:57]\n\t" \
  "s_set_gpr_idx_idx s68\n\t" \
  "v_pk_add_f32 v[56:57], v[36:37], v[56:57]\n\t" \
  "s_set_gpr_idx_idx s70\n\t" \
  "v_pk_add_f32 v[56:57], v[38:39], v[56:57]\n\t" \
  "s_set_gpr_idx_off\n\t" \
  "s_waitcnt lgkmcnt(0)\n\t" \
  "s_cbranch_vccz 6f\n\t" \
  "s_mov_b32 m0, s89\n\t" \
  "s_add_u32 s89, s89, 0x8000\n\t" \
  "buffer_load_dwordx4 %[voff], %[srd], %[soff] offen lds\n\t" \
  "s_add_u32 %[soff], %[soff], %[step]\n\t" \
  "s_lshr_b64 vcc, vcc, 1\n\t" \
  "6:\n\t" \
  "s_cmp_lt_u32 s38, 3\n\t" \
  "s_cbranch_scc1 12f\n\t" \
  "v_pk_mul_f32 v[40:41], v[40:41], s[72:73] op_sel:[0,1] op_sel_hi:[1,1]\n\t" \
  "v_pk_mul_f32 v[42:43], v[42:43], s[74:75] op_sel:[0,1] op_sel_hi:[1,1]\n\t" \
  "v_pk_mul_f32 v[44:45], v[44:45], s[76:77] op_sel:[0,1] op_sel_hi:[1,1]\n\t" \
  "v_pk_mul_f32 v[46:47], v[46:47], s[78:79] op_sel:[0,1] op_sel_hi:[1,1]\n\t" \
  "v_pk_mul_f32 v[48:49], v[48:49], s[80:81] op_sel:[0,1] op_sel_hi:[1,1]\n\t" \
  "v_pk_mul_f32 v[50:51], v[50:51], s[82:83] op_sel:[0,1] op_sel_hi:[1,1]\n\t" \
  "v_pk_mul_f32 v[52:53], v[52:53], s[84:85] op_sel:[0,1] op_sel_hi:[1,1]\n\t" \
  "v_pk_mul_f32 v[54:55], v[54:55], s[86:87] op_sel:[0,1] op_sel_hi:[1,1]\n\t" \
  "s_set_gpr_idx_on s72, gpr_idx(SRC1,DST)\n\t" \
  "v_pk_add_f32 v[56:57], v[40:41], v[56:57]\n\t" \
  "s_set_gpr_idx_idx s74\n\t" \
  "v_pk_add_f32 v[56:57], v[42:43], v[56:57]\n\t" \
  "s_set_gpr_idx_idx s76\n\t" \
  "v_pk_add_f32 v[56:57], v[44:45], v[56:57]\n\t" \
  "s_set_gpr_idx_idx s78\n\t" \
  "v_pk_add_f32 v[56:57], v[46:47], v[56:57]\n\t" \
  "s_set_gpr_idx_idx s80\n\t" \
  "v_pk_add_f32 v[56:57], v[48:49], v[56:57]\n\t" \
  "s_set_gpr_idx_idx s82\n\t" \
  "v_pk_add_f32 v[56:57], v[50:51], v[56:57]\n\t" \
  "s_set_gpr_idx_idx s84\n\t" \
  "v_pk_add_f32 v[56:57], v[52:53], v[56:57]\n\t" \
  "s_set_gpr_idx_idx s86\n\t" \
  "v_pk_add_f32 v[56:57], v[54:55], v[56:57]\n\t" \
  "s_set_gpr_idx_off\n\t" \
  "s_cbranch_vccz 6f\n\t" \
  "s_mov_b32 m0, s89\n\t" \
  "s_add_u32 s89, s89, 0x8000\n\t" \
  "buffer_load_dwordx4 %[voff], %[srd], %[soff] offen lds\n\t" \
  "s_add_u32 %[soff], %[soff], %[step]\n\t" \
  "s_lshr_b64 vcc, vcc, 1\n\t" \
  "6:\n\t" \
  "12:\n\t" \
  "13:\n\t" \
  "s_cbranch_vccz 14f\n\t" \
  "s_mov_b32 m0, s89\n\t" \
  "s_add_u32 s89, s89, 0x8000\n\t" \
  "buffer_load_dwordx4 %[voff], %[srd], %[soff] offen lds\n\t" \
  "s_add_u32 %[soff], %[soff], %[step]\n\t" \
  "s_lshr_b64 vcc, vcc, 1\n\t" \
  "s_branch 13b\n\t" \
  "14:\n\t" \
  "s_add_u32 s88, s90, 1\n\t" \
  "s_cmp_lt_u32 s88, %[te]\n\t" \
  "s_cbranch_scc0 21f\n\t" \
  "s_lshl_b32 s36, s92, 6\n\t" \
  "s_lshr_b32 s37, s92, 26\n\t" \
  "s_add_u32 s36, s36, %[blo]\n\t" \
  "s_addc_u32 s37, s37, %[bhi]\n\t" \
  "s_sub_u32 s88, s93, s92\n\t" \
  "s_cmp_lt_u32 s88, 3\n\t" \
  "s_cbranch_scc1 23f\n\t" \
  "s_load_dwordx16 s[40:55], s[36:37], 0x0\n\t" \
  "s_load_dwordx16 s[56:71], s[36:37], 0x40\n\t" \
  "s_load_dwordx16 s[72:87], s[36:37], 0x80\n\t" \
  "21:\n\t" \
  "s_add_u32 s38, s90, 3\n\t" \
  "s_min_u32 s38, s38, %[ntiles]\n\t" \
  "s_sub_u32 s38, s38, %[obase]\n\t" \
  "s_lshl_b32 s94, s93, 6\n\t" \
  "s_lshr_b32 s95, s93, 26\n\t" \
  "s_add_u32 s94, s94, %[blo]\n\t" \
  "s_addc_u32 s95, s95, %[bhi]\n\t" \
  "v_readlane_b32 s88, %[offreg], s38\n\t" \
  "s_mov_b32 s91, s92\n\t" \
  "s_mov_b32 s92, s93\n\t" \
  "v_xor_b32 v22, 0x400, v22\n\t" \
  "s_sub_u32 s89, s89, 0x28000\n\t" \
  "s_xor_b32 s89, s89, 0x400\n\t" \
  "global_load_dword v23, %[toff], s[94:95]\n\t" \
  "s_mov_b32 s93, s88\n\t" \
  "s_waitcnt vmcnt(1)\n\t" \
  "s_barrier\n\t" \
  "s_add_u32 s90, s90, 1\n\t" \
  "s_cmp_lt_u32 s90, %[te]\n\t" \
  "s_cbranch_scc1 1b\n\t" \
  "s_waitcnt lgkmcnt(0)\n\t" \
  "s_branch 29f\n\t" \
  "22:\n\t" \
  "s_cmp_eq_u32 s88, 0\n\t" \
  "s_cbranch_scc1 20b\n\t" \
  "s_load_dwordx16 s[40:55], s[36:37], 0x0\n\t" \
  "s_cmp_lt_u32 s88, 2\n\t" \
  "s_cbranch_scc1 20b\n\t" \
  "s_load_dwordx16 s[56:71], s[36:37], 0x40\n\t" \
  "s_branch 20b\n\t" \
  "23:\n\t" \
  "s_cmp_eq_u32 s88, 0\n\t" \
  "s_cbranch_scc1 21b\n\t" \
  "s_load_dwordx16 s[40:55], s[36:37], 0x0\n\t" \
  "s_cmp_lt_u32 s88, 2\n\t" \
  "s_cbranch_scc1 21b\n\t" \
  "s_load_dwordx16 s[56:71], s[36:37], 0x40\n\t" \
  "s_branch 21b\n\t" \
  "29:\n\t"

#define TL_ASM_PHASES_NOFMA \
  "s_mov_b32 s39, 0\n\t" \
  "s_mov_b32 s90, %[t0]\n\t" \
  "s_mov_b32 s91, %[o0]\n\t" \
  "s_mov_b32 s92, %[o1]\n\t" \
  "s_mov_b32 s93, %[o2]\n\t" \
  "s_add_u32 s88, s90, 1\n\t" \
  "s_and_b32 s88, s88, 1\n\t" \
  "s_lshl_b32 s88, s88, 10\n\t" \
  "s_add_u32 s89, s88, %[m0wave]\n\t" \
  "s_and_b32 s88, s90, 1\n\t" \
  "s_lshl_b32 s88, s88, 10\n\t" \
  "v_or_b32 v22, s88, %[lane8]\n\t" \
  "s_lshl_b32 s36, s91, 6\n\t" \
  "s_lshr_b32 s37, s91, 26\n\t" \
  "s_add_u32 s36, s36, %[blo]\n\t" \
  "s_addc_u32 s37, s37, %[bhi]\n\t" \
  "s_sub_u32 s88, s92, s91\n\t" \
  "s_cmp_lt_u32 s88, 3\n\t" \
  "s_cbranch_scc1 22f\n\t" \
  "s_load_dwordx16 s[40:55], s[36:37], 0x0\n\t" \
  "s_load_dwordx16 s[56:71], s[36:37], 0x40\n\t" \
  "s_load_dwordx16 s[72:87], s[36:37], 0x80\n\t" \
  "20:\n\t" \
  "1:\n\t" \
  "s_sub_u32 s38, s92, s91\n\t" \
  "s_add_u32 s88, s90, 1\n\t" \
  "s_cmp_lt_u32 s88, %[nfull]\n\t" \
  "s_cselect_b64 vcc, 31, 0\n\t" \
  "s_cmp_eq_u32 s38, 0\n\t" \
  "s_cbranch_scc1 12f\n\t" \
  "s_cbranch_vccz 6f\n\t" \
  "s_mov_b32 m0, s89\n\t" \
  "s_add_u32 s89, s89, 0x8000\n\t" \
  "buffer_load_dwordx4 %[voff], %[srd], %[soff] offen lds\n\t" \
  "s_add_u32 %[soff], %[soff], %[step]\n\t" \
  "s_lshr_b64 vcc, vcc, 1\n\t" \
  "6:\n\t" \
  "s_cbranch_vccz 6f\n\t" \
  "s_mov_b32 m0, s89\n\t" \
  "s_add_u32 s89, s89, 0x8000\n\t" \
  "buffer_load_dwordx4 %[voff], %[srd], %[soff] offen lds\n\t" \
  "s_add_u32 %[soff], %[soff], %[step]\n\t" \
  "s_lshr_b64 vcc, vcc, 1\n\t" \
  "6:\n\t" \
  "s_waitcnt lgkmcnt(0)\n\t" \
  "v_and_or_b32 v40, s40, %[mask], v22\n\t" \
  "v_and_or_b32 v42, s42, %[mask], v22\n\t" \
  "v_and_or_b32 v44, s44, %[mask], v22\n\t" \
  "v_and_or_b32 v46, s46, %[mask], v22\n\t" \
  "ds_read_b64 v[40:41], v40\n\t" \
  "ds_read_b64 v[42:43], v42\n\t" \
  "ds_read_b64 v[44:45], v44\n\t" \
  "ds_read_b64 v[46:47], v46\n\t" \
  "v_and_or_b32 v48, s48, %[mask], v22\n\t" \
  "v_and_or_b32 v50, s50, %[mask], v22\n\t" \
  "v_and_or_b32 v52, s52, %[mask], v22\n\t" \
  "v_and_or_b32 v54, s54, %[mask], v22\n\t" \
  "ds_read_b64 v[48:49], v48\n\t" \
  "ds_read_b64 v[50:51], v50\n\t" \
  "ds_read_b64 v[52:53], v52\n\t" \
  "ds_read_b64 v[54:55], v54\n\t" \
  "s_waitcnt lgkmcnt(0)\n\t" \
  "s_cmp_lt_u32 s38, 4\n\t" \
  "s_cbranch_scc1 40f\n\t" \
  "s_sub_u32 s38, s38, 3\n\t" \
  "11:\n\t" \
  "s_sub_u32 s38, s38, 1\n\t" \
  "s_cbranch_scc1 30f\n\t" \
  "v_and_or_b32 v24, s56, %[mask], v22\n\t" \
  "v_and_or_b32 v26, s58, %[mask], v22\n\t" \
  "v_and_or_b32 v28, s60, %[mask], v22\n\t" \
  "v_and_or_b32 v30, s62, %[mask], v22\n\t" \
  "ds_read_b64 v[24:25], v24\n\t" \
  "ds_read_b64 v[26:27], v26\n\t" \
  "ds_read_b64 v[28:29], v28\n\t" \
  "ds_read_b64 v[30:31], v30\n\t" \
  "v_and_or_b32 v32, s64, %[mask], v22\n\t" \
  "v_and_or_b32 v34, s66, %[mask], v22\n\t" \
  "v_and_or_b32 v36, s68, %[mask], v22\n\t" \
  "v_and_or_b32 v38, s70, %[mask], v22\n\t" \
  "ds_read_b64 v[32:33], v32\n\t" \
  "ds_read_b64 v[34:35], v34\n\t" \
  "ds_read_b64 v[36:37], v36\n\t" \
  "ds_read_b64 v[38:39], v38\n\t" \
  "s_waitcnt lgkmcnt(0)\n\t" \
  "s_load_dwordx16 s[40:55], s[36:37], 0xc0\n\t" \
  "s_cbranch_vccz 6f\n\t" \
  "s_mov_b32 m0, s89\n\t" \
  "s_add_u32 s89, s89, 0x8000\n\t" \
  "buffer_load_dwordx4 %[voff], %[srd], %[soff] offen lds\n\t" \
  "s_add_u32 %[soff], %[soff], %[step]\n\t" \
  "s_lshr_b64 vcc, vcc, 1\n\t" \
  "6:\n\t" \
  "s_sub_u32 s38, s38, 1\n\t" \
  "s_cbranch_scc1 31f\n\t" \
  "v_and_or_b32 v40, s72, %[mask], v22\n\t" \
  "v_and_or_b32 v42, s74, %[mask], v22\n\t" \
  "v_and_or_b32 v44, s76, %[mask], v22\n\t" \
  "v_and_or_b32 v46, s78, %[mask], v22\n\t" \
  "ds_read_b64 v[40:41], v40\n\t" \
  "ds_read_b64 v[42:43], v42\n\t" \
  "ds_read_b64 v[44:45], v44\n\t" \
  "ds_read_b64 v[46:47], v46\n\t" \
  "v_and_or_b32 v48, s80, %[mask], v22\n\t" \
  "v_and_or_b32 v50, s82, %[mask], v22\n\t" \
  "v_and_or_b32 v52, s84, %[mask], v22\n\t" \
  "v_and_or_b32 v54, s86, %[mask], v22\n\t" \
  "ds_read_b64 v[48:49], v48\n\t" \
  "ds_read_b64 v[50:51], v50\n\t" \
  "ds_read_b64 v[52:53], v52\n\t" \
  "ds_read_b64 v[54:55], v54\n\t" \
  "s_waitcnt lgkmcnt(0)\n\t" \
  "s_load_dwordx16 s[56:71], s[36:37], 0x100\n\t" \
  "s_cbranch_vccz 6f\n\t" \
  "s_mov_b32 m0, s89\n\t" \
  "s_add_u32 s89, s89, 0x8000\n\t" \
  "buffer_load_dwordx4 %[voff], %[srd], %[soff] offen lds\n\t" \
  "s_add_u32 %[soff], %[soff], %[step]\n\t" \
  "s_lshr_b64 vcc, vcc, 1\n\t" \
  "6:\n\t" \
  "s_sub_u32 s38, s38, 1\n\t" \
  "s_cbranch_scc1 32f\n\t" \
  "v_and_or_b32 v24, s40, %[mask], v22\n\t" \
  "v_and_or_b32 v26, s42, %[mask], v22\n\t" \
  "v_and_or_b32 v28, s44, %[mask], v22\n\t" \
  "v_and_or_b32 v30, s46, %[mask], v22\n\t" \
  "ds_read_b64 v[24:25], v24\n\t" \
  "ds_read_b64 v[26:27], v26\n\t" \
  "ds_read_b64 v[28:29], v28\n\t" \
  "ds_read_b64 v[30:31], v30\n\t" \
  "v_and_or_b32 v32, s48, %[mask], v22\n\t" \
  "v_and_or_b32 v34, s50, %[mask], v22\n\t" \
  "v_and_or_b32 v36, s52, %[mask], v22\n\t" \
  "v_and_or_b32 v38, s54, %[mask], v22\n\t" \
  "ds_read_b64 v[32:33], v32\n\t" \
  "ds_read_b64 v[34:35], v34\n\t" \
  "ds_read_b64 v[36:37], v36\n\t" \
  "ds_read_b64 v[38:39], v38\n\t" \
  "s_waitcnt lgkmcnt(0)\n\t" \
  "s_load_dwordx16 s[72:87], s[36:37], 0x140\n\t" \
  "s_cbranch_vccz 6f\n\t" \
  "s_mov_b32 m0, s89\n\t" \
  "s_add_u32 s89, s89, 0x8000\n\t" \
  "buffer_load_dwordx4 %[voff], %[srd], %[soff] offen lds\n\t" \
  "s_add_u32 %[soff], %[soff], %[step]\n\t" \
  "s_lshr_b64 vcc, vcc, 1\n\t" \
  "6:\n\t" \
  "s_sub_u32 s38, s38, 1\n\t" \
  "s_cbranch_scc1 33f\n\t" \
  "v_and_or_b32 v40, s56, %[mask], v22\n\t" \
  "v_and_or_b32 v42, s58, %[mask], v22\n\t" \
  "v_and_or_b32 v44, s60, %[mask], v22\n\t" \
  "v_and_or_b32 v46, s62, %[mask], v22\n\t" \
  "ds_read_b64 v[40:41], v40\n\t" \
  "ds_read_b64 v[42:43], v42\n\t" \
  "ds_read_b64 v[44:45], v44\n\t" \
  "ds_read_b64 v[46:47], v46\n\t" \
  "v_and_or_b32 v48, s64, %[mask], v22\n\t" \
  "v_and_or_b32 v50, s66, %[mask], v22\n\t" \
  "v_and_or_b32 v52, s68, %[mask], v22\n\t" \
  "v_and_or_b32 v54, s70, %[mask], v22\n\t" \
  "ds_read_b64 v[48:49], v48\n\t" \
  "ds_read_b64 v[50:51], v50\n\t" \
// ... 285 lines not shown
  "ds_read_b64 v[24:25], v24\n\t" \
  "ds_read_b64 v[26:27], v26\n\t" \
  "ds_read_b64 v[28:29], v28\n\t" \
  "ds_read_b64 v[30:31], v30\n\t" \
  "s_cmp_eq_u32 s64, 0\n\t" \
  "s_cbranch_scc1 8f\n\t" \
  "v_and_or_b32 v32, s64, %[mask], v22\n\t" \
  "v_and_or_b32 v34, s66, %[mask], v22\n\t" \
  "v_and_or_b32 v36, s68, %[mask], v22\n\t" \
  "v_and_or_b32 v38, s70, %[mask], v22\n\t" \
  "ds_read_b64 v[32:33], v32\n\t" \
  "ds_read_b64 v[34:35], v34\n\t" \
  "ds_read_b64 v[36:37], v36\n\t" \
  "ds_read_b64 v[38:39], v38\n\t" \
  "8:\n\t" \
  "s_waitcnt lgkmcnt(0)\n\t" \
  "s_branch 12f\n\t" \
  "40:\n\t" \
  "s_cmp_lt_u32 s38, 2\n\t" \
  "s_cbranch_scc1 7f\n\t" \
  "v_and_or_b32 v24, s56, %[mask], v22\n\t" \
  "v_and_or_b32 v26, s58, %[mask], v22\n\t" \
  "v_and_or_b32 v28, s60, %[mask], v22\n\t" \
  "v_and_or_b32 v30, s62, %[mask], v22\n\t" \
  "ds_read_b64 v[24:25], v24\n\t" \
  "ds_read_b64 v[26:27], v26\n\t" \
  "ds_read_b64 v[28:29], v28\n\t" \
  "ds_read_b64 v[30:31], v30\n\t" \
  "v_and_or_b32 v32, s64, %[mask], v22\n\t" \
  "v_and_or_b32 v34, s66, %[mask], v22\n\t" \
  "v_and_or_b32 v36, s68, %[mask], v22\n\t" \
  "v_and_or_b32 v38, s70, %[mask], v22\n\t" \
  "ds_read_b64 v[32:33], v32\n\t" \
  "ds_read_b64 v[34:35], v34\n\t" \
  "ds_read_b64 v[36:37], v36\n\t" \
  "ds_read_b64 v[38:39], v38\n\t" \
  "7:\n\t" \
  "s_waitcnt lgkmcnt(0)\n\t" \
  "s_cbranch_vccz 6f\n\t" \
  "s_mov_b32 m0, s89\n\t" \
  "s_add_u32 s89, s89, 0x8000\n\t" \
  "buffer_load_dwordx4 %[voff], %[srd], %[soff] offen lds\n\t" \
  "s_add_u32 %[soff], %[soff], %[step]\n\t" \
  "s_lshr_b64 vcc, vcc, 1\n\t" \
  "6:\n\t" \
  "s_cmp_lt_u32 s38, 2\n\t" \
  "s_cbranch_scc1 12f\n\t" \
  "s_cmp_lt_u32 s38, 3\n\t" \
  "s_cbranch_scc1 7f\n\t" \
  "v_and_or_b32 v40, s72, %[mask], v22\n\t" \
  "v_and_or_b32 v42, s74, %[mask], v22\n\t" \
  "v_and_or_b32 v44, s76, %[mask], v22\n\t" \
  "v_and_or_b32 v46, s78, %[mask], v22\n\t" \
  "ds_read_b64 v[40:41], v40\n\t" \
  "ds_read_b64 v[42:43], v42\n\t" \
  "ds_read_b64 v[44:45], v44\n\t" \
  "ds_read_b64 v[46:47], v46\n\t" \
  "v_and_or_b32 v48, s80, %[mask], v22\n\t" \
  "v_and_or_b32 v50, s82, %[mask], v22\n\t" \
  "v_and_or_b32 v52, s84, %[mask], v22\n\t" \
  "v_and_or_b32 v54, s86, %[mask], v22\n\t" \
  "ds_read_b64 v[48:49], v48\n\t" \
  "ds_read_b64 v[50:51], v50\n\t" \
  "ds_read_b64 v[52:53], v52\n\t" \
  "ds_read_b64 v[54:55], v54\n\t" \
  "7:\n\t" \
  "s_waitcnt lgkmcnt(0)\n\t" \
  "s_cbranch_vccz 6f\n\t" \
  "s_mov_b32 m0, s89\n\t" \
  "s_add_u32 s89, s89, 0x8000\n\t" \
  "buffer_load_dwordx4 %[voff], %[srd], %[soff] offen lds\n\t" \
  "s_add_u32 %[soff], %[soff], %[step]\n\t" \
  "s_lshr_b64 vcc, vcc, 1\n\t" \
  "6:\n\t" \
  "s_cmp_lt_u32 s38, 3\n\t" \
  "s_cbranch_scc1 12f\n\t" \
  "s_cbranch_vccz 6f\n\t" \
  "s_mov_b32 m0, s89\n\t" \
  "s_add_u32 s89, s89, 0x8000\n\t" \
  "buffer_load_dwordx4 %[voff], %[srd], %[soff] offen lds\n\t" \
  "s_add_u32 %[soff], %[soff], %[step]\n\t" \
  "s_lshr_b64 vcc, vcc, 1\n\t" \
  "6:\n\t" \
  "12:\n\t" \
  "13:\n\t" \
  "s_cbranch_vccz 14f\n\t" \
  "s_mov_b32 m0, s89\n\t" \
  "s_add_u32 s89, s89, 0x8000\n\t" \
  "buffer_load_dwordx4 %[voff], %[srd], %[soff] offen lds\n\t" \
  "s_add_u32 %[soff], %[soff], %[step]\n\t" \
  "s_lshr_b64 vcc, vcc, 1\n\t" \
  "s_branch 13b\n\t" \
  "14:\n\t" \
  "s_add_u32 s88, s90, 1\n\t" \
  "s_cmp_lt_u32 s88, %[te]\n\t" \
  "s_cbranch_scc0 21f\n\t" \
  "s_lshl_b32 s36, s92, 6\n\t" \
  "s_lshr_b32 s37, s92, 26\n\t" \
  "s_add_u32 s36, s36, %[blo]\n\t" \
  "s_addc_u32 s37, s37, %[bhi]\n\t" \
  "s_sub_u32 s88, s93, s92\n\t" \
  "s_cmp_lt_u32 s88, 3\n\t" \
  "s_cbranch_scc1 23f\n\t" \
  "s_load_dwordx16 s[40:55], s[36:37], 0x0\n\t" \
  "s_load_dwordx16 s[56:71], s[36:37], 0x40\n\t" \
  "s_load_dwordx16 s[72:87], s[36:37], 0x80\n\t" \
  "21:\n\t" \
  "s_add_u32 s38, s90, 3\n\t" \
  "s_min_u32 s38, s38, %[ntiles]\n\t" \
  "s_sub_u32 s38, s38, %[obase]\n\t" \
  "s_lshl_b32 s94, s93, 6\n\t" \
  "s_lshr_b32 s95, s93, 26\n\t" \
  "s_add_u32 s94, s94, %[blo]\n\t" \
  "s_addc_u32 s95, s95, %[bhi]\n\t" \
  "v_readlane_b32 s88, %[offreg], s38\n\t" \
  "s_mov_b32 s91, s92\n\t" \
  "s_mov_b32 s92, s93\n\t" \
  "v_xor_b32 v22, 0x400, v22\n\t" \
  "s_sub_u32 s89, s89, 0x28000\n\t" \
  "s_xor_b32 s89, s89, 0x400\n\t" \
  "global_load_dword v23, %[toff], s[94:95]\n\t" \
  "s_mov_b32 s93, s88\n\t" \
  "s_waitcnt vmcnt(1)\n\t" \
  "s_barrier\n\t" \
  "s_add_u32 s90, s90, 1\n\t" \
  "s_cmp_lt_u32 s90, %[te]\n\t" \
  "s_cbranch_scc1 1b\n\t" \
  "s_waitcnt lgkmcnt(0)\n\t" \
  "s_branch 29f\n\t" \
  "22:\n\t" \
  "s_cmp_eq_u32 s88, 0\n\t" \
  "s_cbranch_scc1 20b\n\t" \
  "s_load_dwordx16 s[40:55], s[36:37], 0x0\n\t" \
  "s_cmp_lt_u32 s88, 2\n\t" \
  "s_cbranch_scc1 20b\n\t" \
  "s_load_dwordx16 s[56:71], s[36:37], 0x40\n\t" \
  "s_branch 20b\n\t" \
  "23:\n\t" \
  "s_cmp_eq_u32 s88, 0\n\t" \
  "s_cbranch_scc1 21b\n\t" \
  "s_load_dwordx16 s[40:55], s[36:37], 0x0\n\t" \
  "s_cmp_lt_u32 s88, 2\n\t" \
  "s_cbranch_scc1 21b\n\t" \
  "s_load_dwordx16 s[56:71], s[36:37], 0x40\n\t" \
  "s_branch 21b\n\t" \
  "29:\n\t"

#define TL_ASM_PHASES_NOLDS \
  "s_mov_b32 s39, 0\n\t" \
  "s_mov_b32 s90, %[t0]\n\t" \
  "s_mov_b32 s91, %[o0]\n\t" \
  "s_mov_b32 s92, %[o1]\n\t" \
  "s_mov_b32 s93, %[o2]\n\t" \
  "s_add_u32 s88, s90, 1\n\t" \
  "s_and_b32 s88, s88, 1\n\t" \
  "s_lshl_b32 s88, s88, 10\n\t" \
  "s_add_u32 s89, s88, %[m0wave]\n\t" \
  "s_and_b32 s88, s90, 1\n\t" \
  "s_lshl_b32 s88, s88, 10\n\t" \
  "v_or_b32 v22, s88, %[lane8]\n\t" \
  "s_lshl_b32 s36, s91, 6\n\t" \
  "s_lshr_b32 s37, s91, 26\n\t" \
  "s_add_u32 s36, s36, %[blo]\n\t" \
  "s_addc_u32 s37, s37, %[bhi]\n\t" \
  "s_sub_u32 s88, s92, s91\n\t" \
  "s_cmp_lt_u32 s88, 3\n\t" \
  "s_cbranch_scc1 22f\n\t" \
  "s_load_dwordx16 s[40:55], s[36:37], 0x0\n\t" \
  "s_load_dwordx16 s[56:71], s[36:37], 0x40\n\t" \
  "s_load_dwordx16 s[72:87], s[36:37], 0x80\n\t" \
  "20:\n\t" \
  "1:\n\t" \
  "s_sub_u32 s38, s92, s91\n\t" \
  "s_add_u32 s88, s90, 1\n\t" \
  "s_cmp_lt_u32 s88, %[nfull]\n\t" \
  "s_cselect_b64 vcc, 31, 0\n\t" \
  "s_cmp_eq_u32 s38, 0\n\t" \
  "s_cbranch_scc1 12f\n\t" \
  "s_cbranch_vccz 6f\n\t" \
  "s_mov_b32 m0, s89\n\t" \
  "s_add_u32 s89, s89, 0x8000\n\t" \
  "buffer_load_dwordx4 %[voff], %[srd], %[soff] offen lds\n\t" \
  "s_add_u32 %[soff], %[soff], %[step]\n\t" \
  "s_lshr_b64 vcc, vcc, 1\n\t" \
  "6:\n\t" \
  "s_cbranch_vccz 6f\n\t" \
  "s_mov_b32 m0, s89\n\t" \
  "s_add_u32 s89, s89, 0x8000\n\t" \
  "buffer_load_dwordx4 %[voff], %[srd], %[soff] offen lds\n\t" \
  "s_add_u32 %[soff], %[soff], %[step]\n\t" \
  "s_lshr_b64 vcc, vcc, 1\n\t" \
  "6:\n\t" \
  "s_waitcnt lgkmcnt(0)\n\t" \
  "s_waitcnt lgkmcnt(0)\n\t" \
  "s_cmp_lt_u32 s38, 4\n\t" \
  "s_cbranch_scc1 40f\n\t" \
  "s_sub_u32 s38, s38, 3\n\t" \
  "11:\n\t" \
  "s_sub_u32 s38, s38, 1\n\t" \
  "s_cbranch_scc1 30f\n\t" \
  "s_waitcnt lgkmcnt(0)\n\t" \
  "s_load_dwordx16 s[40:55], s[36:37], 0xc0\n\t" \
  "s_cbranch_vccz 6f\n\t" \
  "s_mov_b32 m0, s89\n\t" \
  "s_add_u32 s89, s89, 0x8000\n\t" \
  "buffer_load_dwordx4 %[voff], %[srd], %[soff] offen lds\n\t" \
  "s_add_u32 %[soff], %[soff], %[step]\n\t" \
  "s_lshr_b64 vcc, vcc, 1\n\t" \
  "6:\n\t" \
  "s_sub_u32 s38, s38, 1\n\t" \
  "s_cbranch_scc1 31f\n\t" \
  "s_waitcnt lgkmcnt(0)\n\t" \
  "s_load_dwordx16 s[56:71], s[36:37], 0x100\n\t" \
  "s_cbranch_vccz 6f\n\t" \
  "s_mov_b32 m0, s89\n\t" \
  "s_add_u32 s89, s89, 0x8000\n\t" \
  "buffer_load_dwordx4 %[voff], %[srd], %[soff] offen lds\n\t" \
  "s_add_u32 %[soff], %[soff], %[step]\n\t" \
  "s_lshr_b64 vcc, vcc, 1\n\t" \
  "6:\n\t" \
  "s_sub_u32 s38, s38, 1\n\t" \
  "s_cbranch_scc1 32f\n\t" \
  "s_waitcnt lgkmcnt(0)\n\t" \
  "s_load_dwordx16 s[72:87], s[36:37], 0x140\n\t" \
  "s_cbranch_vccz 6f\n\t" \
  "s_mov_b32 m0, s89\n\t" \
  "s_add_u32 s89, s89, 0x8000\n\t" \
  "buffer_load_dwordx4 %[voff], %[srd], %[soff] offen lds\n\t" \
  "s_add_u32 %[soff], %[soff], %[step]\n\t" \
  "s_lshr_b64 vcc, vcc, 1\n\t" \
  "6:\n\t" \
  "s_sub_u32 s38, s38, 1\n\t" \
  "s_cbranch_scc1 33f\n\t" \
  "s_waitcnt lgkmcnt(0)\n\t" \
  "s_load_dwordx16 s[40:55], s[36:37], 0x180\n\t" \
  "s_cbranch_vccz 6f\n\t" \
  "s_mov_b32 m0, s89\n\t" \
  "s_add_u32 s89, s89, 0x8000\n\t" \
  "buffer_load_dwordx4 %[voff], %[srd], %[soff] offen lds\n\t" \
  "s_add_u32 %[soff], %[soff], %[step]\n\t" \
  "s_lshr_b64 vcc, vcc, 1\n\t" \
  "6:\n\t" \
  "s_sub_u32 s38, s38, 1\n\t" \
  "s_cbranch_scc1 34f\n\t" \
  "s_waitcnt lgkmcnt(0)\n\t" \
  "s_load_dwordx16 s[56:71], s[36:37], 0x1c0\n\t" \
  "s_cbranch_vccz 6f\n\t" \
  "s_mov_b32 m0, s89\n\t" \
  "s_add_u32 s89, s89, 0x8000\n\t" \
  "buffer_load_dwordx4 %[voff], %[srd], %[soff] offen lds\n\t" \
  "s_add_u32 %[soff], %[soff], %[step]\n\t" \
  "s_lshr_b64 vcc, vcc, 1\n\t" \
  "6:\n\t" \
  "s_sub_u32 s38, s38, 1\n\t" \
  "s_cbranch_scc1 35f\n\t" \
  "s_waitcnt lgkmcnt(0)\n\t" \
  "s_load_dwordx16 s[72:87], s[36:37], 0x200\n\t" \
  "s_cbranch_vccz 6f\n\t" \
  "s_mov_b32 m0, s89\n\t" \
  "s_add_u32 s89, s89, 0x8000\n\t" \
  "buffer_load_dwordx4 %[voff], %[srd], %[soff] offen lds\n\t" \
  "s_add_u32 %[soff], %[soff], %[step]\n\t" \
  "s_lshr_b64 vcc, vcc, 1\n\t" \
  "6:\n\t" \
  "s_add_u32 s36, s36, 0x180\n\t" \
  "s_addc_u32 s37, s37, 0\n\t" \
  "s_branch 11b\n\t" \
  "30:\n\t" \
  "s_waitcnt lgkmcnt(0)\n\t" \
  "s_waitcnt lgkmcnt(0)\n\t" \
  "s_branch 12f\n\t" \
  "31:\n\t" \
  "s_waitcnt lgkmcnt(0)\n\t" \
  "s_waitcnt lgkmcnt(0)\n\t" \
  "s_branch 12f\n\t" \
  "32:\n\t" \
  "s_waitcnt lgkmcnt(0)\n\t" \
  "s_waitcnt lgkmcnt(0)\n\t" \
  "s_branch 12f\n\t" \
  "33:\n\t" \
  "s_waitcnt lgkmcnt(0)\n\t" \
  "s_waitcnt lgkmcnt(0)\n\t" \
  "s_branch 12f\n\t" \
  "34:\n\t" \
  "s_waitcnt lgkmcnt(0)\n\t" \
  "s_waitcnt lgkmcnt(0)\n\t" \
  "s_branch 12f\n\t" \
  "35:\n\t" \
  "s_waitcnt lgkmcnt(0)\n\t" \
  "s_waitcnt lgkmcnt(0)\n\t" \
  "s_branch 12f\n\t" \
  "40:\n\t" \
  "s_cmp_lt_u32 s38, 2\n\t" \
  "s_cbranch_scc1 7f\n\t" \
  "7:\n\t" \
  "s_waitcnt lgkmcnt(0)\n\t" \
  "s_cbranch_vccz 6f\n\t" \
  "s_mov_b32 m0, s89\n\t" \
  "s_add_u32 s89, s89, 0x8000\n\t" \
  "buffer_load_dwordx4 %[voff], %[srd], %[soff] offen lds\n\t" \
  "s_add_u32 %[soff], %[soff], %[step]\n\t" \
  "s_lshr_b64 vcc, vcc, 1\n\t" \
  "6:\n\t" \
  "s_cmp_lt_u32 s38, 2\n\t" \
  "s_cbranch_scc1 12f\n\t" \
  "s_cmp_lt_u32 s38, 3\n\t" \
  "s_cbranch_scc1 7f\n\t" \
  "7:\n\t" \
  "s_waitcnt lgkmcnt(0)\n\t" \
  "s_cbranch_vccz 6f\n\t" \
  "s_mov_b32 m0, s89\n\t" \
  "s_add_u32 s89, s89, 0x8000\n\t" \
  "buffer_load_dwordx4 %[voff], %[srd], %[soff] offen lds\n\t" \
  "s_add_u32 %[soff], %[soff], %[step]\n\t" \
  "s_lshr_b64 vcc, vcc, 1\n\t" \
  "6:\n\t" \
  "s_cmp_lt_u32 s38, 3\n\t" \
  "s_cbranch_scc1 12f\n\t" \
  "s_cbranch_vccz 6f\n\t" \
  "s_mov_b32 m0, s89\n\t" \
  "s_add_u32 s89, s89, 0x8000\n\t" \
  "buffer_load_dwordx4 %[voff], %[srd], %[soff] offen lds\n\t" \
  "s_add_u32 %[soff], %[soff], %[step]\n\t" \
  "s_lshr_b64 vcc, vcc, 1\n\t" \
  "6:\n\t" \
  "12:\n\t" \
  "13:\n\t" \
  "s_cbranch_vccz 14f\n\t" \
  "s_mov_b32 m0, s89\n\t" \
  "s_add_u32 s89, s89, 0x8000\n\t" \
  "buffer_load_dwordx4 %[voff], %[srd], %[soff] offen lds\n\t" \
  "s_add_u32 %[soff], %[soff], %[step]\n\t" \
  "s_lshr_b64 vcc, vcc, 1\n\t" \
  "s_branch 13b\n\t" \
  "14:\n\t" \
  "s_add_u32 s88, s90, 1\n\t" \
  "s_cmp_lt_u32 s88, %[te]\n\t" \
  "s_cbranch_scc0 21f\n\t" \
  "s_lshl_b32 s36, s92, 6\n\t" \
  "s_lshr_b32 s37, s92, 26\n\t" \
  "s_add_u32 s36, s36, %[blo]\n\t" \
  "s_addc_u32 s37, s37, %[bhi]\n\t" \
  "s_sub_u32 s88, s93, s92\n\t" \
  "s_cmp_lt_u32 s88, 3\n\t" \
  "s_cbranch_scc1 23f\n\t" \
  "s_load_dwordx16 s[40:55], s[36:37], 0x0\n\t" \
  "s_load_dwordx16 s[56:71], s[36:37], 0x40\n\t" \
  "s_load_dwordx16 s[72:87], s[36:37], 0x80\n\t" \
  "21:\n\t" \
  "s_add_u32 s38, s90, 3\n\t" \
  "s_min_u32 s38, s38, %[ntiles]\n\t" \
  "s_sub_u32 s38, s38, %[obase]\n\t" \
  "s_lshl_b32 s94, s93, 6\n\t" \
  "s_lshr_b32 s95, s93, 26\n\t" \
  "s_add_u32 s94, s94, %[blo]\n\t" \
  "s_addc_u32 s95, s95, %[bhi]\n\t" \
  "v_readlane_b32 s88, %[offreg], s38\n\t" \
  "s_mov_b32 s91, s92\n\t" \
  "s_mov_b32 s92, s93\n\t" \
  "v_xor_b32 v22, 0x400, v22\n\t" \
  "s_sub_u32 s89, s89, 0x28000\n\t" \
  "s_xor_b32 s89, s89, 0x400\n\t" \
  "global_load_dword v23, %[toff], s[94:95]\n\t" \
  "s_mov_b32 s93, s88\n\t" \
  "s_waitcnt vmcnt(1)\n\t" \
  "s_barrier\n\t" \
  "s_add_u32 s90, s90, 1\n\t" \
  "s_cmp_lt_u32 s90, %[te]\n\t" \
  "s_cbranch_scc1 1b\n\t" \
  "s_waitcnt lgkmcnt(0)\n\t" \
  "s_branch 29f\n\t" \
  "22:\n\t" \
  "s_cmp_eq_u32 s88, 0\n\t" \
  "s_cbranch_scc1 20b\n\t" \
  "s_load_dwordx16 s[40:55], s[36:37], 0x0\n\t" \
  "s_cmp_lt_u32 s88, 2\n\t" \
  "s_cbranch_scc1 20b\n\t" \
  "s_load_dwordx16 s[56:71], s[36:37], 0x40\n\t" \
  "s_branch 20b\n\t" \
  "23:\n\t" \
  "s_cmp_eq_u32 s88, 0\n\t" \
  "s_cbranch_scc1 21b\n\t" \
  "s_load_dwordx16 s[40:55], s[36:37], 0x0\n\t" \
  "s_cmp_lt_u32 s88, 2\n\t" \
  "s_cbranch_scc1 21b\n\t" \
  "s_load_dwordx16 s[56:71], s[36:37], 0x40\n\t" \
  "s_branch 21b\n\t" \
  "29:\n\t"

#define TL_ASM_PHASES_F64 \
  "s_mov_b32 s39, 0\n\t" \
  "s_mov_b32 s90, %[t0]\n\t" \
  "s_mov_b32 s91, %[o0]\n\t" \
  "s_mov_b32 s92, %[o1]\n\t" \
  "s_mov_b32 s93, %[o2]\n\t" \
  "s_add_u32 s88, s90, 1\n\t" \
  "s_and_b32 s88, s88, 1\n\t" \
  "s_lshl_b32 s88, s88, 10\n\t" \
  "s_add_u32 s89, s88, %[m0wave]\n\t" \
  "s_and_b32 s88, s90, 1\n\t" \
  "s_lshl_b32 s88, s88, 10\n\t" \
  "v_or_b32 v22, s88, %[lane8]\n\t" \
  "s_lshl_b32 s36, s91, 6\n\t" \
  "s_lshr_b32 s37, s91, 26\n\t" \
  "s_add_u32 s36, s36, %[blo]\n\t" \
  "s_addc_u32 s37, s37, %[bhi]\n\t" \
  "s_sub_u32 s88, s92, s91\n\t" \
  "s_cmp_lt_u32 s88, 3\n\t" \
  "s_cbranch_scc1 22f\n\t" \
  "s_load_dwordx16 s[40:55], s[36:37], 0x0\n\t" \
  "s_load_dwordx16 s[56:71], s[36:37], 0x40\n\t" \
  "s_load_dwordx16 s[72:87], s[36:37], 0x80\n\t" \
  "20:\n\t" \
  "1:\n\t" \
  "s_sub_u32 s38, s92, s91\n\t" \
  "s_add_u32 s88, s90, 1\n\t" \
  "s_cmp_lt_u32 s88, %[nfull]\n\t" \
  "s_cselect_b64 vcc, 31, 0\n\t" \
  "s_cmp_eq_u32 s38, 0\n\t" \
  "s_cbranch_scc1 12f\n\t" \
  "s_cbranch_vccz 6f\n\t" \
  "s_mov_b32 m0, s89\n\t" \
  "s_add_u32 s89, s89, 0x8000\n\t" \
  "buffer_load_dwordx4 %[voff], %[srd], %[soff] offen lds\n\t" \
  "s_add_u32 %[soff], %[soff], %[step]\n\t" \
  "s_lshr_b64 vcc, vcc, 1\n\t" \
  "6:\n\t" \
  "s_cbranch_vccz 6f\n\t" \
  "s_mov_b32 m0, s89\n\t" \
  "s_add_u32 s89, s89, 0x8000\n\t" \
  "buffer_load_dwordx4 %[voff], %[srd], %[soff] offen lds\n\t" \
  "s_add_u32 %[soff], %[soff], %[step]\n\t" \
  "s_lshr_b64 vcc, vcc, 1\n\t" \
  "6:\n\t" \
  "s_waitcnt lgkmcnt(0)\n\t" \
  "v_and_or_b32 v40, s40, %[mask], v22\n\t" \
  "v_and_or_b32 v42, s41, %[mask], v22\n\t" \
  "v_and_or_b32 v44, s42, %[mask], v22\n\t" \
  "v_and_or_b32 v46, s43, %[mask], v22\n\t" \
  "ds_read_b64 v[40:41], v40\n\t" \
  "ds_read_b64 v[42:43], v42\n\t" \
  "ds_read_b64 v[44:45], v44\n\t" \
  "ds_read_b64 v[46:47], v46\n\t" \
  "v_and_or_b32 v48, s44, %[mask], v22\n\t" \
  "ds_read_b64 v[48:49], v48\n\t" \
  "s_waitcnt lgkmcnt(0)\n\t" \
  "s_cmp_lt_u32 s38, 4\n\t" \
  "s_cbranch_scc1 40f\n\t" \
  "s_sub_u32 s38, s38, 3\n\t" \
  "11:\n\t" \
  "s_sub_u32 s38, s38, 1\n\t" \
  "s_cbranch_scc1 30f\n\t" \
  "v_and_or_b32 v24, s56, %[mask], v22\n\t" \
  "v_and_or_b32 v26, s57, %[mask], v22\n\t" \
  "v_and_or_b32 v28, s58, %[mask], v22\n\t" \
  "v_and_or_b32 v30, s59, %[mask], v22\n\t" \
  "ds_read_b64 v[24:25], v24\n\t" \
  "ds_read_b64 v[26:27], v26\n\t" \
  "ds_read_b64 v[28:29], v28\n\t" \
  "ds_read_b64 v[30:31], v30\n\t" \
  "v_and_or_b32 v32, s60, %[mask], v22\n\t" \
  "ds_read_b64 v[32:33], v32\n\t" \
  "s_set_gpr_idx_on s40, gpr_idx(SRC2,DST)\n\t" \
  "v_fma_f64 v[56:57], s[46:47], v[40:41], v[56:57]\n\t" \
  "s_set_gpr_idx_idx s41\n\t" \
  "v_fma_f64 v[56:57], s[48:49], v[42:43], v[56:57]\n\t" \
  "s_set_gpr_idx_idx s42\n\t" \
  "v_fma_f64 v[56:57], s[50:51], v[44:45], v[56:57]\n\t" \
  "s_set_gpr_idx_idx s43\n\t" \
  "v_fma_f64 v[56:57], s[52:53], v[46:47], v[56:57]\n\t" \
  "s_set_gpr_idx_idx s44\n\t" \
  "v_fma_f64 v[56:57], s[54:55], v[48:49], v[56:57]\n\t" \
  "s_set_gpr_idx_off\n\t" \
  "s_waitcnt lgkmcnt(0)\n\t" \
  "s_load_dwordx16 s[40:55], s[36:37], 0xc0\n\t" \
  "s_cbranch_vccz 6f\n\t" \
  "s_mov_b32 m0, s89\n\t" \
  "s_add_u32 s89, s89, 0x8000\n\t" \
  "buffer_load_dwordx4 %[voff], %[srd], %[soff] offen lds\n\t" \
  "s_add_u32 %[soff], %[soff], %[step]\n\t" \
  "s_lshr_b64 vcc, vcc, 1\n\t" \
  "6:\n\t" \
  "s_sub_u32 s38, s38, 1\n\t" \
  "s_cbranch_scc1 31f\n\t" \
  "v_and_or_b32 v40, s72, %[mask], v22\n\t" \
  "v_and_or_b32 v42, s73, %[mask], v22\n\t" \
  "v_and_or_b32 v44, s74, %[mask], v22\n\t" \
  "v_and_or_b32 v46, s75, %[mask], v22\n\t" \
  "ds_read_b64 v[40:41], v40\n\t" \
  "ds_read_b64 v[42:43], v42\n\t" \
  "ds_read_b64 v[44:45], v44\n\t" \
  "ds_read_b64 v[46:47], v46\n\t" \
  "v_and_or_b32 v48, s76, %[mask], v22\n\t" \
  "ds_read_b64 v[48:49], v48\n\t" \
  "s_set_gpr_idx_on s56, gpr_idx(SRC2,DST)\n\t" \
  "v_fma_f64 v[56:57], s[62:63], v[24:25], v[56:57]\n\t" \
  "s_set_gpr_idx_idx s57\n\t" \
  "v_fma_f64 v[56:57], s[64:65], v[26:27], v[56:57]\n\t" \
  "s_set_gpr_idx_idx s58\n\t" \
  "v_fma_f64 v[56:57], s[66:67], v[28:29], v[56:57]\n\t" \
  "s_set_gpr_idx_idx s59\n\t" \
  "v_fma_f64 v[56:57], s[68:69], v[30:31], v[56:57]\n\t" \
  "s_set_gpr_idx_idx s60\n\t" \
  "v_fma_f64 v[56:57], s[70:71], v[32:33], v[56:57]\n\t" \
  "s_set_gpr_idx_off\n\t" \
  "s_waitcnt lgkmcnt(0)\n\t" \
  "s_load_dwordx16 s[56:71], s[36:37], 0x100\n\t" \
  "s_cbranch_vccz 6f\n\t" \
  "s_mov_b32 m0, s89\n\t" \
  "s_add_u32 s89, s89, 0x8000\n\t" \
  "buffer_load_dwordx4 %[voff], %[srd], %[soff] offen lds\n\t" \
  "s_add_u32 %[soff], %[soff], %[step]\n\t" \
  "s_lshr_b64 vcc, vcc, 1\n\t" \
  "6:\n\t" \
  "s_sub_u32 s38, s38, 1\n\t" \
  "s_cbranch_scc1 32f\n\t" \
  "v_and_or_b32 v24, s40, %[mask], v22\n\t" \
  "v_and_or_b32 v26, s41, %[mask], v22\n\t" \
  "v_and_or_b32 v28, s42, %[mask], v22\n\t" \
  "v_and_or_b32 v30, s43, %[mask], v22\n\t" \
  "ds_read_b64 v[24:25], v24\n\t" \
  "ds_read_b64 v[26:27], v26\n\t" \
  "ds_read_b64 v[28:29], v28\n\t" \
  "ds_read_b64 v[30:31], v30\n\t" \
  "v_and_or_b32 v32, s44, %[mask], v22\n\t" \
  "ds_read_b64 v[32:33], v32\n\t" \
  "s_set_gpr_idx_on s72, gpr_idx(SRC2,DST)\n\t" \
  "v_fma_f64 v[56:57], s[78:79], v[40:41], v[56:57]\n\t" \
  "s_set_gpr_idx_idx s73\n\t" \
  "v_fma_f64 v[56:57], s[80:81], v[42:43], v[56:57]\n\t" \
  "s_set_gpr_idx_idx s74\n\t" \
  "v_fma_f64 v[56:57], s[82:83], v[44:45], v[56:57]\n\t" \
  "s_set_gpr_idx_idx s75\n\t" \
  "v_fma_f64 v[56:57], s[84:85], v[46:47], v[56:57]\n\t" \
  "s_set_gpr_idx_idx s76\n\t" \
  "v_fma_f64 v[56:57], s[86:87], v[48:49], v[56:57]\n\t" \
  "s_set_gpr_idx_off\n\t" \
  "s_waitcnt lgkmcnt(0)\n\t" \
  "s_load_dwordx16 s[72:87], s[36:37], 0x140\n\t" \
  "s_cbranch_vccz 6f\n\t" \
  "s_mov_b32 m0, s89\n\t" \
  "s_add_u32 s89, s89, 0x8000\n\t" \
  "buffer_load_dwordx4 %[voff], %[srd], %[soff] offen lds\n\t" \
  "s_add_u32 %[soff], %[soff], %[step]\n\t" \
  "s_lshr_b64 vcc, vcc, 1\n\t" \
  "6:\n\t" \
  "s_sub_u32 s38, s38, 1\n\t" \
  "s_cbranch_scc1 33f\n\t" \
  "v_and_or_b32 v40, s56, %[mask], v22\n\t" \
  "v_and_or_b32 v42, s57, %[mask], v22\n\t" \
  "v_and_or_b32 v44, s58, %[mask], v22\n\t" \
  "v_and_or_b32 v46, s59, %[mask], v22\n\t" \
  "ds_read_b64 v[40:41], v40\n\t" \
// ... 474 lines not shown
  "v_and_or_b32 v26, s57, %[mask], v22\n\t" \
  "v_and_or_b32 v28, s58, %[mask], v22\n\t" \
  "v_and_or_b32 v30, s59, %[mask], v22\n\t" \
  "ds_read_b64 v[24:25], v24\n\t" \
  "ds_read_b64 v[26:27], v26\n\t" \
  "ds_read_b64 v[28:29], v28\n\t" \
  "ds_read_b64 v[30:31], v30\n\t" \
  "v_and_or_b32 v32, s60, %[mask], v22\n\t" \
  "ds_read_b64 v[32:33], v32\n\t" \
  "7:\n\t" \
  "s_set_gpr_idx_on s40, gpr_idx(SRC2,DST)\n\t" \
  "v_fma_f64 v[56:57], s[46:47], v[40:41], v[56:57]\n\t" \
  "s_set_gpr_idx_idx s41\n\t" \
  "v_fma_f64 v[56:57], s[48:49], v[42:43], v[56:57]\n\t" \
  "s_set_gpr_idx_idx s42\n\t" \
  "v_fma_f64 v[56:57], s[50:51], v[44:45], v[56:57]\n\t" \
  "s_set_gpr_idx_idx s43\n\t" \
  "v_fma_f64 v[56:57], s[52:53], v[46:47], v[56:57]\n\t" \
  "s_set_gpr_idx_idx s44\n\t" \
  "v_fma_f64 v[56:57], s[54:55], v[48:49], v[56:57]\n\t" \
  "s_set_gpr_idx_off\n\t" \
  "s_waitcnt lgkmcnt(0)\n\t" \
  "s_cbranch_vccz 6f\n\t" \
  "s_mov_b32 m0, s89\n\t" \
  "s_add_u32 s89, s89, 0x8000\n\t" \
  "buffer_load_dwordx4 %[voff], %[srd], %[soff] offen lds\n\t" \
  "s_add_u32 %[soff], %[soff], %[step]\n\t" \
  "s_lshr_b64 vcc, vcc, 1\n\t" \
  "6:\n\t" \
  "s_cmp_lt_u32 s38, 2\n\t" \
  "s_cbranch_scc1 12f\n\t" \
  "s_cmp_lt_u32 s38, 3\n\t" \
  "s_cbranch_scc1 7f\n\t" \
  "v_and_or_b32 v40, s72, %[mask], v22\n\t" \
  "v_and_or_b32 v42, s73, %[mask], v22\n\t" \
  "v_and_or_b32 v44, s74, %[mask], v22\n\t" \
  "v_and_or_b32 v46, s75, %[mask], v22\n\t" \
  "ds_read_b64 v[40:41], v40\n\t" \
  "ds_read_b64 v[42:43], v42\n\t" \
  "ds_read_b64 v[44:45], v44\n\t" \
  "ds_read_b64 v[46:47], v46\n\t" \
  "v_and_or_b32 v48, s76, %[mask], v22\n\t" \
  "ds_read_b64 v[48:49], v48\n\t" \
  "7:\n\t" \
  "s_set_gpr_idx_on s56, gpr_idx(SRC2,DST)\n\t" \
  "v_fma_f64 v[56:57], s[62:63], v[24:25], v[56:57]\n\t" \
  "s_set_gpr_idx_idx s57\n\t" \
  "v_fma_f64 v[56:57], s[64:65], v[26:27], v[56:57]\n\t" \
  "s_set_gpr_idx_idx s58\n\t" \
  "v_fma_f64 v[56:57], s[66:67], v[28:29], v[56:57]\n\t" \
  "s_set_gpr_idx_idx s59\n\t" \
  "v_fma_f64 v[56:57], s[68:69], v[30:31], v[56:57]\n\t" \
  "s_set_gpr_idx_idx s60\n\t" \
  "v_fma_f64 v[56:57], s[70:71], v[32:33], v[56:57]\n\t" \
  "s_set_gpr_idx_off\n\t" \
  "s_waitcnt lgkmcnt(0)\n\t" \
  "s_cbranch_vccz 6f\n\t" \
  "s_mov_b32 m0, s89\n\t" \
  "s_add_u32 s89, s89, 0x8000\n\t" \
  "buffer_load_dwordx4 %[voff], %[srd], %[soff] offen lds\n\t" \
  "s_add_u32 %[soff], %[soff], %[step]\n\t" \
  "s_lshr_b64 vcc, vcc, 1\n\t" \
  "6:\n\t" \
  "s_cmp_lt_u32 s38, 3\n\t" \
  "s_cbranch_scc1 12f\n\t" \
  "s_set_gpr_idx_on s72, gpr_idx(SRC2,DST)\n\t" \
  "v_fma_f64 v[56:57], s[78:79], v[40:41], v[56:57]\n\t" \
  "s_set_gpr_idx_idx s73\n\t" \
  "v_fma_f64 v[56:57], s[80:81], v[42:43], v[56:57]\n\t" \
  "s_set_gpr_idx_idx s74\n\t" \
  "v_fma_f64 v[56:57], s[82:83], v[44:45], v[56:57]\n\t" \
  "s_set_gpr_idx_idx s75\n\t" \
  "v_fma_f64 v[56:57], s[84:85], v[46:47], v[56:57]\n\t" \
  "s_set_gpr_idx_idx s76\n\t" \
  "v_fma_f64 v[56:57], s[86:87], v[48:49], v[56:57]\n\t" \
  "s_set_gpr_idx_off\n\t" \
  "s_cbranch_vccz 6f\n\t" \
  "s_mov_b32 m0, s89\n\t" \
  "s_add_u32 s89, s89, 0x8000\n\t" \
  "buffer_load_dwordx4 %[voff], %[srd], %[soff] offen lds\n\t" \
  "s_add_u32 %[soff], %[soff], %[step]\n\t" \
  "s_lshr_b64 vcc, vcc, 1\n\t" \
  "6:\n\t" \
  "12:\n\t" \
  "13:\n\t" \
  "s_cbranch_vccz 14f\n\t" \
  "s_mov_b32 m0, s89\n\t" \
  "s_add_u32 s89, s89, 0x8000\n\t" \
  "buffer_load_dwordx4 %[voff], %[srd], %[soff] offen lds\n\t" \
  "s_add_u32 %[soff], %[soff], %[step]\n\t" \
  "s_lshr_b64 vcc, vcc, 1\n\t" \
  "s_branch 13b\n\t" \
  "14:\n\t" \
  "s_add_u32 s88, s90, 1\n\t" \
  "s_cmp_lt_u32 s88, %[te]\n\t" \
  "s_cbranch_scc0 21f\n\t" \
  "s_lshl_b32 s36, s92, 6\n\t" \
  "s_lshr_b32 s37, s92, 26\n\t" \
  "s_add_u32 s36, s36, %[blo]\n\t" \
  "s_addc_u32 s37, s37, %[bhi]\n\t" \
  "s_sub_u32 s88, s93, s92\n\t" \
  "s_cmp_lt_u32 s88, 3\n\t" \
  "s_cbranch_scc1 23f\n\t" \
  "s_load_dwordx16 s[40:55], s[36:37], 0x0\n\t" \
  "s_load_dwordx16 s[56:71], s[36:37], 0x40\n\t" \
  "s_load_dwordx16 s[72:87], s[36:37], 0x80\n\t" \
  "21:\n\t" \
  "s_add_u32 s38, s90, 3\n\t" \
  "s_min_u32 s38, s38, %[ntiles]\n\t" \
  "s_sub_u32 s38, s38, %[obase]\n\t" \
  "s_lshl_b32 s94, s93, 6\n\t" \
  "s_lshr_b32 s95, s93, 26\n\t" \
  "s_add_u32 s94, s94, %[blo]\n\t" \
  "s_addc_u32 s95, s95, %[bhi]\n\t" \
  "v_readlane_b32 s88, %[offreg], s38\n\t" \
  "s_mov_b32 s91, s92\n\t" \
  "s_mov_b32 s92, s93\n\t" \
  "v_xor_b32 v22, 0x400, v22\n\t" \
  "s_sub_u32 s89, s89, 0x28000\n\t" \
  "s_xor_b32 s89, s89, 0x400\n\t" \
  "global_load_dword v23, %[toff], s[94:95]\n\t" \
  "s_mov_b32 s93, s88\n\t" \
  "s_waitcnt vmcnt(1)\n\t" \
  "s_barrier\n\t" \
  "s_add_u32 s90, s90, 1\n\t" \
  "s_cmp_lt_u32 s90, %[te]\n\t" \
  "s_cbranch_scc1 1b\n\t" \
  "s_waitcnt lgkmcnt(0)\n\t" \
  "s_branch 29f\n\t" \
  "22:\n\t" \
  "s_cmp_eq_u32 s88, 0\n\t" \
  "s_cbranch_scc1 20b\n\t" \
  "s_load_dwordx16 s[40:55], s[36:37], 0x0\n\t" \
  "s_cmp_lt_u32 s88, 2\n\t" \
  "s_cbranch_scc1 20b\n\t" \
  "s_load_dwordx16 s[56:71], s[36:37], 0x40\n\t" \
  "s_branch 20b\n\t" \
  "23:\n\t" \
  "s_cmp_eq_u32 s88, 0\n\t" \
  "s_cbranch_scc1 21b\n\t" \
  "s_load_dwordx16 s[40:55], s[36:37], 0x0\n\t" \
  "s_cmp_lt_u32 s88, 2\n\t" \
  "s_cbranch_scc1 21b\n\t" \
  "s_load_dwordx16 s[56:71], s[36:37], 0x40\n\t" \
  "s_branch 21b\n\t" \
  "29:\n\t"

#define TL_ASM_PHASES_F64_EXACT \
  "s_mov_b32 s39, 0\n\t" \
  "s_mov_b32 s90, %[t0]\n\t" \
  "s_mov_b32 s91, %[o0]\n\t" \
  "s_mov_b32 s92, %[o1]\n\t" \
  "s_mov_b32 s93, %[o2]\n\t" \
  "s_add_u32 s88, s90, 1\n\t" \
  "s_and_b32 s88, s88, 1\n\t" \
  "s_lshl_b32 s88, s88, 10\n\t" \
  "s_add_u32 s89, s88, %[m0wave]\n\t" \
  "s_and_b32 s88, s90, 1\n\t" \
  "s_lshl_b32 s88, s88, 10\n\t" \
  "v_or_b32 v22, s88, %[lane8]\n\t" \
  "s_lshl_b32 s36, s91, 6\n\t" \
  "s_lshr_b32 s37, s91, 26\n\t" \
  "s_add_u32 s36, s36, %[blo]\n\t" \
  "s_addc_u32 s37, s37, %[bhi]\n\t" \
  "s_sub_u32 s88, s92, s91\n\t" \
  "s_cmp_lt_u32 s88, 3\n\t" \
  "s_cbranch_scc1 22f\n\t" \
  "s_load_dwordx16 s[40:55], s[36:37], 0x0\n\t" \
  "s_load_dwordx16 s[56:71], s[36:37], 0x40\n\t" \
  "s_load_dwordx16 s[72:87], s[36:37], 0x80\n\t" \
  "20:\n\t" \
  "1:\n\t" \
  "s_sub_u32 s38, s92, s91\n\t" \
  "s_add_u32 s88, s90, 1\n\t" \
  "s_cmp_lt_u32 s88, %[nfull]\n\t" \
  "s_cselect_b64 vcc, 31, 0\n\t" \
  "s_cmp_eq_u32 s38, 0\n\t" \
  "s_cbranch_scc1 12f\n\t" \
  "s_cbranch_vccz 6f\n\t" \
  "s_mov_b32 m0, s89\n\t" \
  "s_add_u32 s89, s89, 0x8000\n\t" \
  "buffer_load_dwordx4 %[voff], %[srd], %[soff] offen lds\n\t" \
  "s_add_u32 %[soff], %[soff], %[step]\n\t" \
  "s_lshr_b64 vcc, vcc, 1\n\t" \
  "6:\n\t" \
  "s_cbranch_vccz 6f\n\t" \
  "s_mov_b32 m0, s89\n\t" \
  "s_add_u32 s89, s89, 0x8000\n\t" \
  "buffer_load_dwordx4 %[voff], %[srd], %[soff] offen lds\n\t" \
  "s_add_u32 %[soff], %[soff], %[step]\n\t" \
  "s_lshr_b64 vcc, vcc, 1\n\t" \
  "6:\n\t" \
  "s_waitcnt lgkmcnt(0)\n\t" \
  "v_and_or_b32 v40, s40, %[mask], v22\n\t" \
  "v_and_or_b32 v42, s41, %[mask], v22\n\t" \
  "v_and_or_b32 v44, s42, %[mask], v22\n\t" \
  "v_and_or_b32 v46, s43, %[mask], v22\n\t" \
  "ds_read_b64 v[40:41], v40\n\t" \
  "ds_read_b64 v[42:43], v42\n\t" \
  "ds_read_b64 v[44:45], v44\n\t" \
  "ds_read_b64 v[46:47], v46\n\t" \
  "v_and_or_b32 v48, s44, %[mask], v22\n\t" \
  "ds_read_b64 v[48:49], v48\n\t" \
  "s_waitcnt lgkmcnt(0)\n\t" \
  "s_cmp_lt_u32 s38, 4\n\t" \
  "s_cbranch_scc1 40f\n\t" \
  "s_sub_u32 s38, s38, 3\n\t" \
  "11:\n\t" \
  "s_sub_u32 s38, s38, 1\n\t" \
  "s_cbranch_scc1 30f\n\t" \
  "v_and_or_b32 v24, s56, %[mask], v22\n\t" \
  "v_and_or_b32 v26, s57, %[mask], v22\n\t" \
  "v_and_or_b32 v28, s58, %[mask], v22\n\t" \
  "v_and_or_b32 v30, s59, %[mask], v22\n\t" \
  "ds_read_b64 v[24:25], v24\n\t" \
  "ds_read_b64 v[26:27], v26\n\t" \
  "ds_read_b64 v[28:29], v28\n\t" \
  "ds_read_b64 v[30:31], v30\n\t" \
  "v_and_or_b32 v32, s60, %[mask], v22\n\t" \
  "ds_read_b64 v[32:33], v32\n\t" \
  "v_mul_f64 v[40:41], v[40:41], s[46:47]\n\t" \
  "v_mul_f64 v[42:43], v[42:43], s[48:49]\n\t" \
  "v_mul_f64 v[44:45], v[44:45], s[50:51]\n\t" \
  "v_mul_f64 v[46:47], v[46:47], s[52:53]\n\t" \
  "v_mul_f64 v[48:49], v[48:49], s[54:55]\n\t" \
  "s_set_gpr_idx_on s40, gpr_idx(SRC1,DST)\n\t" \
  "v_add_f64 v[56:57], v[40:41], v[56:57]\n\t" \
  "s_set_gpr_idx_idx s41\n\t" \
  "v_add_f64 v[56:57], v[42:43], v[56:57]\n\t" \
  "s_set_gpr_idx_idx s42\n\t" \
  "v_add_f64 v[56:57], v[44:45], v[56:57]\n\t" \
  "s_set_gpr_idx_idx s43\n\t" \
  "v_add_f64 v[56:57], v[46:47], v[56:57]\n\t" \
  "s_set_gpr_idx_idx s44\n\t" \
  "v_add_f64 v[56:57], v[48:49], v[56:57]\n\t" \
  "s_set_gpr_idx_off\n\t" \
  "s_waitcnt lgkmcnt(0)\n\t" \
  "s_load_dwordx16 s[40:55], s[36:37], 0xc0\n\t" \
  "s_cbranch_vccz 6f\n\t" \
  "s_mov_b32 m0, s89\n\t" \
  "s_add_u32 s89, s89, 0x8000\n\t" \
  "buffer_load_dwordx4 %[voff], %[srd], %[soff] offen lds\n\t" \
  "s_add_u32 %[soff], %[soff], %[step]\n\t" \
  "s_lshr_b64 vcc, vcc, 1\n\t" \
  "6:\n\t" \
  "s_sub_u32 s38, s38, 1\n\t" \
  "s_cbranch_scc1 31f\n\t" \
  "v_and_or_b32 v40, s72, %[mask], v22\n\t" \
  "v_and_or_b32 v42, s73, %[mask], v22\n\t" \
  "v_and_or_b32 v44, s74, %[mask], v22\n\t" \
  "v_and_or_b32 v46, s75, %[mask], v22\n\t" \
  "ds_read_b64 v[40:41], v40\n\t" \
  "ds_read_b64 v[42:43], v42\n\t" \
  "ds_read_b64 v[44:45], v44\n\t" \
  "ds_read_b64 v[46:47], v46\n\t" \
  "v_and_or_b32 v48, s76, %[mask], v22\n\t" \
  "ds_read_b64 v[48:49], v48\n\t" \
  "v_mul_f64 v[24:25], v[24:25], s[62:63]\n\t" \
  "v_mul_f64 v[26:27], v[26:27], s[64:65]\n\t" \
  "v_mul_f64 v[28:29], v[28:29], s[66:67]\n\t" \
  "v_mul_f64 v[30:31], v[30:31], s[68:69]\n\t" \
  "v_mul_f64 v[32:33], v[32:33], s[70:71]\n\t" \
  "s_set_gpr_idx_on s56, gpr_idx(SRC1,DST)\n\t" \
  "v_add_f64 v[56:57], v[24:25], v[56:57]\n\t" \
  "s_set_gpr_idx_idx s57\n\t" \
  "v_add_f64 v[56:57], v[26:27], v[56:57]\n\t" \
  "s_set_gpr_idx_idx s58\n\t" \
  "v_add_f64 v[56:57], v[28:29], v[56:57]\n\t" \
  "s_set_gpr_idx_idx s59\n\t" \
  "v_add_f64 v[56:57], v[30:31], v[56:57]\n\t" \
  "s_set_gpr_idx_idx s60\n\t" \
  "v_add_f64 v[56:57], v[32:33], v[56:57]\n\t" \
  "s_set_gpr_idx_off\n\t" \
  "s_waitcnt lgkmcnt(0)\n\t" \
  "s_load_dwordx16 s[56:71], s[36:37], 0x100\n\t" \
  "s_cbranch_vccz 6f\n\t" \
  "s_mov_b32 m0, s89\n\t" \
  "s_add_u32 s89, s89, 0x8000\n\t" \
  "buffer_load_dwordx4 %[voff], %[srd], %[soff] offen lds\n\t" \
  "s_add_u32 %[soff], %[soff], %[step]\n\t" \
  "s_lshr_b64 vcc, vcc, 1\n\t" \
  "6:\n\t" \
  "s_sub_u32 s38, s38, 1\n\t" \
  "s_cbranch_scc1 32f\n\t" \
  "v_and_or_b32 v24, s40, %[mask], v22\n\t" \
  "v_and_or_b32 v26, s41, %[mask], v22\n\t" \
  "v_and_or_b32 v28, s42, %[mask], v22\n\t" \
  "v_and_or_b32 v30, s43, %[mask], v22\n\t" \
  "ds_read_b64 v[24:25], v24\n\t" \
  "ds_read_b64 v[26:27], v26\n\t" \
  "ds_read_b64 v[28:29], v28\n\t" \
  "ds_read_b64 v[30:31], v30\n\t" \
  "v_and_or_b32 v32, s44, %[mask], v22\n\t" \
  "ds_read_b64 v[32:33], v32\n\t" \
  "v_mul_f64 v[40:41], v[40:41], s[78:79]\n\t" \
  "v_mul_f64 v[42:43], v[42:43], s[80:81]\n\t" \
  "v_mul_f64 v[44:45], v[44:45], s[82:83]\n\t" \
  "v_mul_f64 v[46:47], v[46:47], s[84:85]\n\t" \
  "v_mul_f64 v[48:49], v[48:49], s[86:87]\n\t" \
  "s_set_gpr_idx_on s72, gpr_idx(SRC1,DST)\n\t" \
  "v_add_f64 v[56:57], v[40:41], v[56:57]\n\t" \
  "s_set_gpr_idx_idx s73\n\t" \
  "v_add_f64 v[56:57], v[42:43], v[56:57]\n\t" \
  "s_set_gpr_idx_idx s74\n\t" \
  "v_add_f64 v[56:57], v[44:45], v[56:57]\n\t" \
  "s_set_gpr_idx_idx s75\n\t" \
  "v_add_f64 v[56:57], v[46:47], v[56:57]\n\t" \
  "s_set_gpr_idx_idx s76\n\t" \
  "v_add_f64 v[56:57], v[48:49], v[56:57]\n\t" \
  "s_set_gpr_idx_off\n\t" \
  "s_waitcnt lgkmcnt(0)\n\t" \
// ... 627 lines not shown
  "s_set_gpr_idx_on s40, gpr_idx(SRC1,DST)\n\t" \
  "v_add_f64 v[56:57], v[40:41], v[56:57]\n\t" \
  "s_set_gpr_idx_idx s41\n\t" \
  "v_add_f64 v[56:57], v[42:43], v[56:57]\n\t" \
  "s_set_gpr_idx_idx s42\n\t" \
  "v_add_f64 v[56:57], v[44:45], v[56:57]\n\t" \
  "s_set_gpr_idx_idx s43\n\t" \
  "v_add_f64 v[56:57], v[46:47], v[56:57]\n\t" \
  "s_set_gpr_idx_idx s44\n\t" \
  "v_add_f64 v[56:57], v[48:49], v[56:57]\n\t" \
  "s_set_gpr_idx_off\n\t" \
  "s_waitcnt lgkmcnt(0)\n\t" \
  "s_cbranch_vccz 6f\n\t" \
  "s_mov_b32 m0, s89\n\t" \
  "s_add_u32 s89, s89, 0x8000\n\t" \
  "buffer_load_dwordx4 %[voff], %[srd], %[soff] offen lds\n\t" \
  "s_add_u32 %[soff], %[soff], %[step]\n\t" \
  "s_lshr_b64 vcc, vcc, 1\n\t" \
  "6:\n\t" \
  "s_cmp_lt_u32 s38, 2\n\t" \
  "s_cbranch_scc1 12f\n\t" \
  "s_cmp_lt_u32 s38, 3\n\t" \
  "s_cbranch_scc1 7f\n\t" \
  "v_and_or_b32 v40, s72, %[mask], v22\n\t" \
  "v_and_or_b32 v42, s73, %[mask], v22\n\t" \
  "v_and_or_b32 v44, s74, %[mask], v22\n\t" \
  "v_and_or_b32 v46, s75, %[mask], v22\n\t" \
  "ds_read_b64 v[40:41], v40\n\t" \
  "ds_read_b64 v[42:43], v42\n\t" \
  "ds_read_b64 v[44:45], v44\n\t" \
  "ds_read_b64 v[46:47], v46\n\t" \
  "v_and_or_b32 v48, s76, %[mask], v22\n\t" \
  "ds_read_b64 v[48:49], v48\n\t" \
  "7:\n\t" \
  "v_mul_f64 v[24:25], v[24:25], s[62:63]\n\t" \
  "v_mul_f64 v[26:27], v[26:27], s[64:65]\n\t" \
  "v_mul_f64 v[28:29], v[28:29], s[66:67]\n\t" \
  "v_mul_f64 v[30:31], v[30:31], s[68:69]\n\t" \
  "v_mul_f64 v[32:33], v[32:33], s[70:71]\n\t" \
  "s_set_gpr_idx_on s56, gpr_idx(SRC1,DST)\n\t" \
  "v_add_f64 v[56:57], v[24:25], v[56:57]\n\t" \
  "s_set_gpr_idx_idx s57\n\t" \
  "v_add_f64 v[56:57], v[26:27], v[56:57]\n\t" \
  "s_set_gpr_idx_idx s58\n\t" \
  "v_add_f64 v[56:57], v[28:29], v[56:57]\n\t" \
  "s_set_gpr_idx_idx s59\n\t" \
  "v_add_f64 v[56:57], v[30:31], v[56:57]\n\t" \
  "s_set_gpr_idx_idx s60\n\t" \
  "v_add_f64 v[56:57], v[32:33], v[56:57]\n\t" \
  "s_set_gpr_idx_off\n\t" \
  "s_waitcnt lgkmcnt(0)\n\t" \
  "s_cbranch_vccz 6f\n\t" \
  "s_mov_b32 m0, s89\n\t" \
  "s_add_u32 s89, s89, 0x8000\n\t" \
  "buffer_load_dwordx4 %[voff], %[srd], %[soff] offen lds\n\t" \
  "s_add_u32 %[soff], %[soff], %[step]\n\t" \
  "s_lshr_b64 vcc, vcc, 1\n\t" \
  "6:\n\t" \
  "s_cmp_lt_u32 s38, 3\n\t" \
  "s_cbranch_scc1 12f\n\t" \
  "v_mul_f64 v[40:41], v[40:41], s[78:79]\n\t" \
  "v_mul_f64 v[42:43], v[42:43], s[80:81]\n\t" \
  "v_mul_f64 v[44:45], v[44:45], s[82:83]\n\t" \
  "v_mul_f64 v[46:47], v[46:47], s[84:85]\n\t" \
  "v_mul_f64 v[48:49], v[48:49], s[86:87]\n\t" \
  "s_set_gpr_idx_on s72, gpr_idx(SRC1,DST)\n\t" \
  "v_add_f64 v[56:57], v[40:41], v[56:57]\n\t" \
  "s_set_gpr_idx_idx s73\n\t" \
  "v_add_f64 v[56:57], v[42:43], v[56:57]\n\t" \
  "s_set_gpr_idx_idx s74\n\t" \
  "v_add_f64 v[56:57], v[44:45], v[56:57]\n\t" \
  "s_set_gpr_idx_idx s75\n\t" \
  "v_add_f64 v[56:57], v[46:47], v[56:57]\n\t" \
  "s_set_gpr_idx_idx s76\n\t" \
  "v_add_f64 v[56:57], v[48:49], v[56:57]\n\t" \
  "s_set_gpr_idx_off\n\t" \
  "s_cbranch_vccz 6f\n\t" \
  "s_mov_b32 m0, s89\n\t" \
  "s_add_u32 s89, s89, 0x8000\n\t" \
  "buffer_load_dwordx4 %[voff], %[srd], %[soff] offen lds\n\t" \
  "s_add_u32 %[soff], %[soff], %[step]\n\t" \
  "s_lshr_b64 vcc, vcc, 1\n\t" \
  "6:\n\t" \
  "12:\n\t" \
  "13:\n\t" \
  "s_cbranch_vccz 14f\n\t" \
  "s_mov_b32 m0, s89\n\t" \
  "s_add_u32 s89, s89, 0x8000\n\t" \
  "buffer_load_dwordx4 %[voff], %[srd], %[soff] offen lds\n\t" \
  "s_add_u32 %[soff], %[soff], %[step]\n\t" \
  "s_lshr_b64 vcc, vcc, 1\n\t" \
  "s_branch 13b\n\t" \
  "14:\n\t" \
  "s_add_u32 s88, s90, 1\n\t" \
  "s_cmp_lt_u32 s88, %[te]\n\t" \
  "s_cbranch_scc0 21f\n\t" \
  "s_lshl_b32 s36, s92, 6\n\t" \
  "s_lshr_b32 s37, s92, 26\n\t" \
  "s_add_u32 s36, s36, %[blo]\n\t" \
  "s_addc_u32 s37, s37, %[bhi]\n\t" \
  "s_sub_u32 s88, s93, s92\n\t" \
  "s_cmp_lt_u32 s88, 3\n\t" \
  "s_cbranch_scc1 23f\n\t" \
  "s_load_dwordx16 s[40:55], s[36:37], 0x0\n\t" \
  "s_load_dwordx16 s[56:71], s[36:37], 0x40\n\t" \
  "s_load_dwordx16 s[72:87], s[36:37], 0x80\n\t" \
  "21:\n\t" \
  "s_add_u32 s38, s90, 3\n\t" \
  "s_min_u32 s38, s38, %[ntiles]\n\t" \
  "s_sub_u32 s38, s38, %[obase]\n\t" \
  "s_lshl_b32 s94, s93, 6\n\t" \
  "s_lshr_b32 s95, s93, 26\n\t" \
  "s_add_u32 s94, s94, %[blo]\n\t" \
  "s_addc_u32 s95, s95, %[bhi]\n\t" \
  "v_readlane_b32 s88, %[offreg], s38\n\t" \
  "s_mov_b32 s91, s92\n\t" \
  "s_mov_b32 s92, s93\n\t" \
  "v_xor_b32 v22, 0x400, v22\n\t" \
  "s_sub_u32 s89, s89, 0x28000\n\t" \
  "s_xor_b32 s89, s89, 0x400\n\t" \
  "global_load_dword v23, %[toff], s[94:95]\n\t" \
  "s_mov_b32 s93, s88\n\t" \
  "s_waitcnt vmcnt(1)\n\t" \
  "s_barrier\n\t" \
  "s_add_u32 s90, s90, 1\n\t" \
  "s_cmp_lt_u32 s90, %[te]\n\t" \
  "s_cbranch_scc1 1b\n\t" \
  "s_waitcnt lgkmcnt(0)\n\t" \
  "s_branch 29f\n\t" \
  "22:\n\t" \
  "s_cmp_eq_u32 s88, 0\n\t" \
  "s_cbranch_scc1 20b\n\t" \
  "s_load_dwordx16 s[40:55], s[36:37], 0x0\n\t" \
  "s_cmp_lt_u32 s88, 2\n\t" \
  "s_cbranch_scc1 20b\n\t" \
  "s_load_dwordx16 s[56:71], s[36:37], 0x40\n\t" \
  "s_branch 20b\n\t" \
  "23:\n\t" \
  "s_cmp_eq_u32 s88, 0\n\t" \
  "s_cbranch_scc1 21b\n\t" \
  "s_load_dwordx16 s[40:55], s[36:37], 0x0\n\t" \
  "s_cmp_lt_u32 s88, 2\n\t" \
  "s_cbranch_scc1 21b\n\t" \
  "s_load_dwordx16 s[56:71], s[36:37], 0x40\n\t" \
  "s_branch 21b\n\t" \
  "29:\n\t"

#define TL_ASM_PHASES_I32 \
  "s_mov_b32 s39, 0\n\t" \
  "s_mov_b32 s90, %[t0]\n\t" \
  "s_mov_b32 s91, %[o0]\n\t" \
  "s_mov_b32 s92, %[o1]\n\t" \
  "s_mov_b32 s93, %[o2]\n\t" \
  "s_add_u32 s88, s90, 1\n\t" \
  "s_and_b32 s88, s88, 1\n\t" \
  "s_lshl_b32 s88, s88, 10\n\t" \
  "s_add_u32 s89, s88, %[m0wave]\n\t" \
  "s_and_b32 s88, s90, 1\n\t" \
  "s_lshl_b32 s88, s88, 10\n\t" \
  "v_or_b32 v22, s88, %[lane8]\n\t" \
  "s_lshl_b32 s36, s91, 6\n\t" \
  "s_lshr_b32 s37, s91, 26\n\t" \
  "s_add_u32 s36, s36, %[blo]\n\t" \
  "s_addc_u32 s37, s37, %[bhi]\n\t" \
  "s_sub_u32 s88, s92, s91\n\t" \
  "s_cmp_lt_u32 s88, 3\n\t" \
  "s_cbranch_scc1 22f\n\t" \
  "s_load_dwordx16 s[40:55], s[36:37], 0x0\n\t" \
  "s_load_dwordx16 s[56:71], s[36:37], 0x40\n\t" \
  "s_load_dwordx16 s[72:87], s[36:37], 0x80\n\t" \
  "20:\n\t" \
  "1:\n\t" \
  "s_sub_u32 s38, s92, s91\n\t" \
  "s_add_u32 s88, s90, 1\n\t" \
  "s_cmp_lt_u32 s88, %[nfull]\n\t" \
  "s_cselect_b64 vcc, 31, 0\n\t" \
  "s_cmp_eq_u32 s38, 0\n\t" \
  "s_cbranch_scc1 12f\n\t" \
  "s_cbranch_vccz 6f\n\t" \
  "s_mov_b32 m0, s89\n\t" \
  "s_add_u32 s89, s89, 0x8000\n\t" \
  "buffer_load_dwordx4 %[voff], %[srd], %[soff] offen lds\n\t" \
  "s_add_u32 %[soff], %[soff], %[step]\n\t" \
  "s_lshr_b64 vcc, vcc, 1\n\t" \
  "6:\n\t" \
  "s_cbranch_vccz 6f\n\t" \
  "s_mov_b32 m0, s89\n\t" \
  "s_add_u32 s89, s89, 0x8000\n\t" \
  "buffer_load_dwordx4 %[voff], %[srd], %[soff] offen lds\n\t" \
  "s_add_u32 %[soff], %[soff], %[step]\n\t" \
  "s_lshr_b64 vcc, vcc, 1\n\t" \
  "6:\n\t" \
  "s_waitcnt lgkmcnt(0)\n\t" \
  "v_and_or_b32 v40, s40, %[mask], v22\n\t" \
  "v_and_or_b32 v42, s42, %[mask], v22\n\t" \
  "v_and_or_b32 v44, s44, %[mask], v22\n\t" \
  "v_and_or_b32 v46, s46, %[mask], v22\n\t" \
  "ds_read_b64 v[40:41], v40\n\t" \
  "ds_read_b64 v[42:43], v42\n\t" \
  "ds_read_b64 v[44:45], v44\n\t" \
  "ds_read_b64 v[46:47], v46\n\t" \
  "v_and_or_b32 v48, s48, %[mask], v22\n\t" \
  "v_and_or_b32 v50, s50, %[mask], v22\n\t" \
  "v_and_or_b32 v52, s52, %[mask], v22\n\t" \
  "v_and_or_b32 v54, s54, %[mask], v22\n\t" \
  "ds_read_b64 v[48:49], v48\n\t" \
  "ds_read_b64 v[50:51], v50\n\t" \
  "ds_read_b64 v[52:53], v52\n\t" \
  "ds_read_b64 v[54:55], v54\n\t" \
  "s_waitcnt lgkmcnt(0)\n\t" \
  "s_cmp_lt_u32 s38, 4\n\t" \
  "s_cbranch_scc1 40f\n\t" \
  "s_sub_u32 s38, s38, 3\n\t" \
  "11:\n\t" \
  "s_sub_u32 s38, s38, 1\n\t" \
  "s_cbranch_scc1 30f\n\t" \
  "v_and_or_b32 v24, s56, %[mask], v22\n\t" \
  "v_and_or_b32 v26, s58, %[mask], v22\n\t" \
  "v_and_or_b32 v28, s60, %[mask], v22\n\t" \
  "v_and_or_b32 v30, s62, %[mask], v22\n\t" \
  "ds_read_b64 v[24:25], v24\n\t" \
  "ds_read_b64 v[26:27], v26\n\t" \
  "ds_read_b64 v[28:29], v28\n\t" \
  "ds_read_b64 v[30:31], v30\n\t" \
  "v_and_or_b32 v32, s64, %[mask], v22\n\t" \
  "v_and_or_b32 v34, s66, %[mask], v22\n\t" \
  "v_and_or_b32 v36, s68, %[mask], v22\n\t" \
  "v_and_or_b32 v38, s70, %[mask], v22\n\t" \
  "ds_read_b64 v[32:33], v32\n\t" \
  "ds_read_b64 v[34:35], v34\n\t" \
  "ds_read_b64 v[36:37], v36\n\t" \
  "ds_read_b64 v[38:39], v38\n\t" \
  "v_mul_lo_u32 v40, v40, s41\n\t" \
  "v_mul_lo_u32 v41, v41, s41\n\t" \
  "v_mul_lo_u32 v42, v42, s43\n\t" \
  "v_mul_lo_u32 v43, v43, s43\n\t" \
  "v_mul_lo_u32 v44, v44, s45\n\t" \
  "v_mul_lo_u32 v45, v45, s45\n\t" \
  "v_mul_lo_u32 v46, v46, s47\n\t" \
  "v_mul_lo_u32 v47, v47, s47\n\t" \
  "v_mul_lo_u32 v48, v48, s49\n\t" \
  "v_mul_lo_u32 v49, v49, s49\n\t" \
  "v_mul_lo_u32 v50, v50, s51\n\t" \
  "v_mul_lo_u32 v51, v51, s51\n\t" \
  "v_mul_lo_u32 v52, v52, s53\n\t" \
  "v_mul_lo_u32 v53, v53, s53\n\t" \
  "v_mul_lo_u32 v54, v54, s55\n\t" \
  "v_mul_lo_u32 v55, v55, s55\n\t" \
  "s_set_gpr_idx_on s40, gpr_idx(SRC1,DST)\n\t" \
  "v_add_u32 v56, v40, v56\n\t" \
  "v_add_u32 v57, v41, v57\n\t" \
  "s_set_gpr_idx_idx s42\n\t" \
  "v_add_u32 v56, v42, v56\n\t" \
  "v_add_u32 v57, v43, v57\n\t" \
  "s_set_gpr_idx_idx s44\n\t" \
  "v_add_u32 v56, v44, v56\n\t" \
  "v_add_u32 v57, v45, v57\n\t" \
  "s_set_gpr_idx_idx s46\n\t" \
  "v_add_u32 v56, v46, v56\n\t" \
  "v_add_u32 v57, v47, v57\n\t" \
  "s_set_gpr_idx_idx s48\n\t" \
  "v_add_u32 v56, v48, v56\n\t" \
  "v_add_u32 v57, v49, v57\n\t" \
  "s_set_gpr_idx_idx s50\n\t" \
  "v_add_u32 v56, v50, v56\n\t" \
  "v_add_u32 v57, v51, v57\n\t" \
  "s_set_gpr_idx_idx s52\n\t" \
  "v_add_u32 v56, v52, v56\n\t" \
  "v_add_u32 v57, v53, v57\n\t" \
  "s_set_gpr_idx_idx s54\n\t" \
  "v_add_u32 v56, v54, v56\n\t" \
  "v_add_u32 v57, v55, v57\n\t" \
  "s_set_gpr_idx_off\n\t" \
  "s_waitcnt lgkmcnt(0)\n\t" \
  "s_load_dwordx16 s[40:55], s[36:37], 0xc0\n\t" \
  "s_cbranch_vccz 6f\n\t" \
  "s_mov_b32 m0, s89\n\t" \
  "s_add_u32 s89, s89, 0x8000\n\t" \
  "buffer_load_dwordx4 %[voff], %[srd], %[soff] offen lds\n\t" \
  "s_add_u32 %[soff], %[soff], %[step]\n\t" \
  "s_lshr_b64 vcc, vcc, 1\n\t" \
  "6:\n\t" \
  "s_sub_u32 s38, s38, 1\n\t" \
  "s_cbranch_scc1 31f\n\t" \
  "v_and_or_b32 v40, s72, %[mask], v22\n\t" \
  "v_and_or_b32 v42, s74, %[mask], v22\n\t" \
  "v_and_or_b32 v44, s76, %[mask], v22\n\t" \
  "v_and_or_b32 v46, s78, %[mask], v22\n\t" \
  "ds_read_b64 v[40:41], v40\n\t" \
  "ds_read_b64 v[42:43], v42\n\t" \
  "ds_read_b64 v[44:45], v44\n\t" \
  "ds_read_b64 v[46:47], v46\n\t" \
  "v_and_or_b32 v48, s80, %[mask], v22\n\t" \
  "v_and_or_b32 v50, s82, %[mask], v22\n\t" \
  "v_and_or_b32 v52, s84, %[mask], v22\n\t" \
  "v_and_or_b32 v54, s86, %[mask], v22\n\t" \
  "ds_read_b64 v[48:49], v48\n\t" \
  "ds_read_b64 v[50:51], v50\n\t" \
  "ds_read_b64 v[52:53], v52\n\t" \
  "ds_read_b64 v[54:55], v54\n\t" \
  "v_mul_lo_u32 v24, v24, s57\n\t" \
  "v_mul_lo_u32 v25, v25, s57\n\t" \
  "v_mul_lo_u32 v26, v26, s59\n\t" \
  "v_mul_lo_u32 v27, v27, s59\n\t" \
  "v_mul_lo_u32 v28, v28, s61\n\t" \
  "v_mul_lo_u32 v29, v29, s61\n\t" \
  "v_mul_lo_u32 v30, v30, s63\n\t" \
  "v_mul_lo_u32 v31, v31, s63\n\t" \
  "v_mul_lo_u32 v32, v32, s65\n\t" \
  "v_mul_lo_u32 v33, v33, s65\n\t" \
  "v_mul_lo_u32 v34, v34, s67\n\t" \
// ... 2536 lines not shown
```

Before: 30170 GFLOP/s.

## Make tiled SpMM kernel persistent with cross-item tile0 prefetch

Result: no change. 29960 GFLOP/s (-0.7%).

```diff
diff --git a/sparse_amd/_kernels.py b/sparse_amd/_kernels.py
--- a/sparse_amd/_kernels.py
+++ b/sparse_amd/_kernels.py
@@ -1486,7 +1486,7 @@
     return TiledLayout(blocks, blk_off, dtype, nnz / epb / max(nseg, 1) + 0.5, group_ends=True, pending=state)
 
 
-def dot_csr_ndarray_tiled(layout, out_shape, Kd, b, out=None, exact=False):
+def dot_csr_ndarray_tiled(layout, out_shape, Kd, b, out=None, exact=False, max_workgroups=None):
     blocks, blk_off, dtype = layout
     M, N = int(out_shape[0]), int(b.shape[1])
     Nout = int(out_shape[1])
@@ -1508,6 +1508,10 @@
     ends = _ffi.TILED_GROUP_ENDS if getattr(layout, "group_ends", False) else 0
     ints = _ffi.TILED_INT32 if dtype == torch.int32 else 0
     flags = (_ffi.EXACT_MULADD if exact and not ints else 0) | ends | ints | (hint << 8) | (last_cols << 16)
+    if max_workgroups is not None:
+        if int(max_workgroups) < 1:
+            raise ValueError("max_workgroups must be positive")
+        flags |= min(255, (int(max_workgroups) + 7) // 8) << 24
     rowmap = getattr(layout, "rowmap", None)
     if rowmap is not None:
         _ffi.call("spamd_spmm_tiled_mapped", code_of(_tiled_layout_dtype(dtype)), M, int(layout.groups), Kd, N, ptr(blocks), ptr(blk_off),
diff --git a/sparse_amd/csrc/build.py b/sparse_amd/csrc/build.py
--- a/sparse_amd/csrc/build.py
+++ b/sparse_amd/csrc/build.py
@@ -63,24 +63,43 @@
             sg = int(ln.split("SGPRs Spill:")[1].split()[0])
         elif "VGPRs Spill:" in ln and name is not None:
             vg = int(ln.split("VGPRs Spill:")[1].split()[0])
-            if needle in name and (sg or vg):
+            if needle in name:
                 out.append((name, sg, vg))
     return out
+
+
+def _verdict_path(obj):
+    return obj[:-2] + ".nospill"
+
+
+def _verdict_ok(obj):
+    v = _verdict_path(obj)
+    if not os.path.exists(v) or os.path.getmtime(v) < os.path.getmtime(obj):
+        return False
+    lines = open(v).read().splitlines()
+    return bool(lines) and lines[0] == "ok"
 
 
 def _compile(src, force):
     obj = os.path.join(OBJ_DIR, os.path.basename(src)[:-4] + ".o")
     newest = max(os.path.getmtime(p) for p in [src] + _own_deps(src, obj))
-    if not force and os.path.exists(obj) and os.path.getmtime(obj) >= newest:
+    needle = NO_SPILL.get(os.path.basename(src))
+    if not force and os.path.exists(obj) and os.path.getmtime(obj) >= newest and (not needle or _verdict_ok(obj)):
         return obj, ""
-    needle = NO_SPILL.get(os.path.basename(src))
     extra = ["-Rpass-analysis=kernel-resource-usage"] if needle else []
     cmd = [_hipcc(), *CXXFLAGS, *extra, "-MD", "-MF", obj[:-2] + ".d", "-c", src, "-o", obj]
     r = subprocess.run(cmd, capture_output=True, text=True)
     if r.returncode != 0:
         raise RuntimeError(f"hipcc failed for {src}:\n{' '.join(cmd)}\n{r.stdout}\n{r.stderr}")
     if needle:
-        bad = _spills(r.stderr, needle)
+        seen = _spills(r.stderr, needle)
+        if not seen:
+            os.remove(obj)
+            raise RuntimeError(f"{os.path.basename(src)}: no kernel-resource-usage remark for {needle}* in the compiler's "
+                               "output - cannot tell whether registers were spilled; refused (see NO_SPILL in sparse_amd/csrc/build.py)")
+        bad = [x for x in seen if x[1] or x[2]]
+        with open(_verdict_path(obj), "w") as f:
+            f.write(("spill" if bad else "ok") + "\n" + "".join(f"{n} sgpr_spill={s} vgpr_spill={v}\n" for n, s, v in seen))
         if bad:
             os.remove(obj)
             raise RuntimeError(f"{os.path.basename(src)}: the compiler spilled registers in " +
diff --git a/sparse_amd/csrc/spmm_tiled.hip b/sparse_amd/csrc/spmm_tiled.hip
--- a/sparse_amd/csrc/spmm_tiled.hip
+++ b/sparse_amd/csrc/spmm_tiled.hip
@@ -332,7 +332,7 @@
 template <int MODE>
 __device__ __forceinline__ void tl_phases(const int* stream, int t0, int te, int o0, int o1, int o2, int offreg, int obase,
                                           int ntiles, int nfull, int toff, int mask, unsigned m0wave,
-                                          unsigned row_step, int voff, tl_srd_t srd, unsigned& soff) {
+                                          unsigned row_step, int voff, tl_srd_t srd, unsigned& soff, unsigned par) {
   const int lane = threadIdx.x & 63;
   const unsigned blo = (unsigned)((uintptr_t)stream & 0xffffffffu), bhi = (unsigned)((uintptr_t)stream >> 32);
   const int lane8 = lane * 8;
@@ -340,6 +340,7 @@
   [soff] "+s"(soff)                                                                                               \
   : [blo] "s"(blo), [bhi] "s"(bhi), [t0] "s"(t0), [te] "s"(te), [o0] "s"(o0), [o1] "s"(o1), [o2] "s"(o2),         \
     [obase] "s"(obase), [ntiles] "s"(ntiles), [nfull] "s"(nfull), [m0wave] "s"(m0wave), [step] "s"(row_step),      \
+    [par] "s"(par),                                                                                               \
     [toff] "v"(toff), [lane8] "v"(lane8), [mask] "v"(mask), [offreg] "v"(offreg), [voff] "v"(voff), [srd] "s"(srd)  \
   : "memory", "m0", "scc", "vcc", TL_CLOB_SGPR, TL_CLOB_TMP, TL_CLOB_ACC
   if (MODE == 6)
@@ -368,91 +369,157 @@
   bx = uniform((int)((seq / pin) * 8u + (l & 7u)));
 }
 
-template <int DBG, int MODE, typename T>
-__global__ void __launch_bounds__(TL_WAVES * 64) __attribute__((amdgpu_num_vgpr(TL_ASM_COMP)))
-spmm_tiled_kernel(int64_t M, int64_t K, int ntiles, int touch_lines, const int* __restrict__ stream,
-                  const int* __restrict__ blk_off, const T* __restrict__ b, int64_t ldb,
-                  T* __restrict__ out, int64_t ldo, int last_cols, int npanels, int nblocks, const int* __restrict__ rowmap) {
-  constexpr int PANEL = TlFmt<T>::PANEL;
-  constexpr int CPL = PANEL / 64;
-  extern __shared__ __attribute__((aligned(16))) char lds[];
-  const int tid = threadIdx.x;
-  const int lane = tid & 63;
+template <typename T>
+struct TlArgs {
+  int64_t M, K;
+  const int* stream;
+  const int* blk_off;
+  const T* b;
+  T* out;
+  int64_t ldo;
+  const int* rowmap;
+  unsigned row_bytes;
+  int ntiles, nfull, has_partial;
+  int touch_lines, ends;
+  int last_cols, npanels, nblocks;
+  int nitems, grid;
+};
+
+template <typename T>
+__device__ __forceinline__ const __attribute__((address_space(4))) TlArgs<T>* tl_args() {
+  auto p = (const __attribute__((address_space(4))) TlArgs<T>*)__builtin_amdgcn_kernarg_segment_ptr();
+  asm volatile("" : "+s"(p));
+  return p;
+}
+
+__device__ __forceinline__ int tl_tid() {
+  int tid = threadIdx.x;
+  asm volatile("" : "+v"(tid));
+  return tid;
+}
+
+template <typename T>
+__device__ __forceinline__ void tl_item_map(int i, int& bx, int& by) {
+  const auto A = tl_args<T>();
+  const unsigned G = (unsigned)A->grid;
+  unsigned w = blockIdx.x;
+  if (A->rowmap != nullptr && (i & 1)) w = G - 8u - (w & ~7u) + (w & 7u);
+  const unsigned L = (unsigned)i * G + w;
+  if (L >= (unsigned)A->nitems) {
+    bx = by = -1;
+    return;
+  }
+  tl_block_map(L, A->npanels, A->nblocks, bx, by);
+}
+
+template <typename T>
+__device__ __forceinline__ int tl_next_item(int i) {
+  for (++i;; ++i) {
+    int bx, by;
+    tl_item_map<T>(i, bx, by);
+    if (bx < 0) return -1;
+    const auto A = tl_args<T>();
+    if (bx < A->nblocks && by < A->npanels) return i;
+  }
+}
+
+template <typename T>
+__device__ __forceinline__ void tl_issue_partial(int by, int t, unsigned par) {
+  const auto A = tl_args<T>();
+  const int tid = tl_tid();
   const int wv = uniform(tid >> 6);
+  const int64_t K = A->K;
+  const char* const bp = reinterpret_cast<const char*>(A->b + (int64_t)by * TlFmt<T>::PANEL);
+  const unsigned row_bytes = A->row_bytes;
+#pragma unroll
+  for (int j = 0; j < TL_DMA_PER_TILE; ++j) {
+    const int e = (j * (TL_WAVES * 64) + tid) * 16;
+    int64_t r = (int64_t)t * TL_KB + (e >> 9);
+    if (r >= K) r = K - 1;
+    tl_dma16(((unsigned)(j * TL_WAVES + wv) * 2u + (((unsigned)t + par) & 1u)) * 1024u,
+             bp + r * (int64_t)row_bytes + (e & 511));
+  }
+}
+
+template <typename T>
+__device__ __forceinline__ int tl_voff() {
+  const int tid = tl_tid();
+  return (int)((unsigned)(tid >> 5) * tl_args<T>()->row_bytes) + (tid & 31) * 16;
+}
+
+template <int DBG, typename T>
+__device__ __forceinline__ void tl_issue_tile0(int i, unsigned par, tl_srd_t& srd, unsigned& soff) {
   int bx, by;
-  tl_block_map(blockIdx.x, npanels, nblocks, bx, by);
-  if (bx >= nblocks || by >= npanels) return;
-  const int g = bx * TL_WAVES + wv;
-  b += (int64_t)by * PANEL;
-  out += (int64_t)by * PANEL;
-
-  asm volatile(TL_ASM_ZERO ::: "memory", TL_CLOB_ACC);
-
-  const int nfull = DBG == 2 ? 0 : (int)(K / TL_KB);
-  const unsigned row_step = (unsigned)((2 * TL_WAVES) * ldb * (int64_t)sizeof(T));
-  const unsigned m0wave = (unsigned)wv * 2048u;
-  const uint64_t bbase = (uint64_t)(uintptr_t)b;
-  tl_srd_t srd;
+  tl_item_map<T>(i, bx, by);
+  const auto A = tl_args<T>();
+  const uint64_t bbase = (uint64_t)(uintptr_t)(A->b + (int64_t)by * TlFmt<T>::PANEL);
   srd[0] = (int)(bbase & 0xffffffffu);
   srd[1] = (int)((bbase >> 32) & 0xffffu);
   srd[2] = (int)0xffffffffu;
   srd[3] = 0x00020000;
-  const int voff = (int)((int64_t)(tid >> 5) * ldb * (int64_t)sizeof(T)) + (tid & 31) * 16;
-  unsigned soff = 0;
-  auto issue_partial = [&](int t) {
-#pragma unroll
-    for (int i = 0; i < TL_DMA_PER_TILE; ++i) {
-      const int e = (i * (TL_WAVES * 64) + tid) * 16;
-      int64_t r = (int64_t)t * TL_KB + (e >> 9);
-      if (r >= K) r = K - 1;
-      tl_dma16(((unsigned)(i * TL_WAVES + wv) * 2u + (unsigned)(t & 1)) * 1024u,
-               reinterpret_cast<const char*>(b + r * ldb) + (e & 511));
-    }
-  };
-  const bool has_partial = DBG != 2 && (int64_t)nfull * TL_KB < K;
-
-  if (nfull > 0)
-    asm volatile(TL_ASM_TILE0 : [soff] "+s"(soff) : [m0wave] "s"(m0wave), [step] "s"(row_step), [voff] "v"(voff), [srd] "s"(srd) : "memory", "m0", "scc", "vcc", "s89");
-  else if (has_partial)
-    issue_partial(0);
-  asm volatile("s_waitcnt vmcnt(0)" ::: "memory");
-  __syncthreads();
-
-  const int* const myoff = blk_off + (int64_t)g * (ntiles + (touch_lines >> 16));
-  touch_lines &= 0xffff;
-  const int toff = (lane < touch_lines ? lane : touch_lines - 1) * 64;
-  int t = 0;
-  while (t < ntiles) {
-    const int obase = t;
-    const int q = obase + lane;
-    int offreg = myoff[q < ntiles ? q : ntiles];
-    asm volatile("" : "+v"(offreg));
-    int te = obase + 61 < ntiles ? obase + 61 : ntiles;
-    if (has_partial && t < nfull - 1 && nfull - 1 < te) te = nfull - 1;
-    if (has_partial && t == nfull - 1) issue_partial(nfull);
-    auto o = [&](int tt) { return wave_bcast(offreg, (tt < ntiles ? tt : ntiles) - obase); };
-    const int o0 = o(t), o1 = o(t + 1), o2 = o(t + 2);
-    if (t == 0) {
-      const int n = o2 - o0, l = lane < n ? lane : 0;
-      asm volatile("global_load_dword " TL_ASM_TOUCH ", %0, off" ::"v"(reinterpret_cast<const char*>(stream + (int64_t)o0 * 16) + l * 64)
-                   : "memory", TL_ASM_TOUCH);
-    }
-    tl_phases<MODE>(stream, t, te, o0, o1, o2, offreg, obase, ntiles, nfull, toff, (int)0xfffffe00, m0wave, row_step, voff, srd, soff);
-    t = te;
-  }
-  asm volatile("s_waitcnt vmcnt(0) lgkmcnt(0)" ::: "memory");
-
-  const int64_t row0 = (int64_t)g * TL_RG;
-  const int64_t left = M - row0;
-  const int nvalid = left <= 0 ? 0 : (left < TL_RG ? (int)left : TL_RG);
-  T* const obase_p = out + row0 * ldo + lane * CPL;
+  soff = 0;
+  if (DBG == 2) return;
+  if (A->nfull > 0) {
+    const unsigned m0tile = (unsigned)uniform(tl_tid() >> 6) * 2048u + par * 1024u;
+    const unsigned row_step = A->row_bytes * (2 * TL_WAVES);
+    const int voff = tl_voff<T>();
+    asm volatile(TL_ASM_TILE0 : [soff] "+s"(soff) : [m0wave] "s"(m0tile), [step] "s"(row_step), [voff] "v"(voff), [srd] "s"(srd) : "memory", "m0", "scc", "vcc", "s89");
+  } else if (A->has_partial) {
+    tl_issue_partial<T>(by, 0, par);
+  }
+}
+
+template <typename T>
+__device__ __forceinline__ const int* tl_offsets_ptr(int i, int obase) {
+  int bx, by;
+  tl_item_map<T>(i, bx, by);
+  const auto A = tl_args<T>();
+  const int ntiles = A->ntiles;
+  const int g = bx * TL_WAVES + uniform(tl_tid() >> 6);
+  const int* const myoff = A->blk_off + (int64_t)g * (ntiles + A->ends);
+  const int q = obase + (tl_tid() & 63);
+  return myoff + (q < ntiles ? q : ntiles);
+}
+
+template <typename T>
+__device__ __forceinline__ int tl_load_offsets(int i, int obase) {
+  return *tl_offsets_ptr<T>(i, obase);
+}
+
+template <typename T>
+__device__ __forceinline__ void tl_prefetch_offsets(int i) {
+  asm volatile("global_load_dword " TL_ASM_TOUCH ", %0, off" ::"v"(tl_offsets_ptr<T>(i, 0)) : "memory", TL_ASM_TOUCH);
+}
+
+template <typename T>
+__device__ __forceinline__ void tl_touch_first_lists(int off0) {
+  const auto A = tl_args<T>();
+  const int ntiles = A->ntiles;
+  const int lane = tl_tid() & 63;
+  const int o0 = wave_bcast(off0, 0), o2 = wave_bcast(off0, ntiles < 2 ? ntiles : 2);
+  const int n = o2 - o0, l = lane < n ? lane : 0;
+  asm volatile("global_load_dword " TL_ASM_TOUCH ", %0, off" ::"v"(reinterpret_cast<const char*>(A->stream + (int64_t)o0 * 16) + l * 64)
+               : "memory", TL_ASM_TOUCH);
+}
+
+template <typename T>
+__device__ __forceinline__ void tl_store_item(int i) {
+  constexpr int PANEL = TlFmt<T>::PANEL;
+  constexpr int CPL = PANEL / 64;
+  int bx, by;
+  tl_item_map<T>(i, bx, by);
+  const auto A = tl_args<T>();
+  const int lane = tl_tid() & 63;
+  const int g = bx * TL_WAVES + uniform(tl_tid() >> 6);
+  const int64_t ldo = A->ldo;
+  T* const outp = A->out + (int64_t)by * PANEL;
   const int64_t stride_bytes = ldo * (int64_t)sizeof(T);
-  int bx2, by2;
-  tl_block_map(blockIdx.x, npanels, nblocks, bx2, by2);
-  const int ncols = (last_cols > 0 && by2 == npanels - 1) ? last_cols : PANEL;
+  const int last_cols = A->last_cols;
+  const int ncols = (last_cols > 0 && by == A->npanels - 1) ? last_cols : PANEL;
+  const int* const rowmap = A->rowmap;
   if (rowmap) {
     const int* const rm = rowmap + (int64_t)g * TL_RG;
-    T* const base_p = out + lane * CPL;
+    T* const base_p = outp + lane * CPL;
     if (lane * CPL + CPL <= ncols)
       asm volatile(TL_ASM_STORE_PERM
                    :
@@ -469,6 +536,10 @@
     }
     return;
   }
+  const int64_t row0 = (int64_t)g * TL_RG;
+  const int64_t left = A->M - row0;
+  const int nvalid = left <= 0 ? 0 : (left < TL_RG ? (int)left : TL_RG);
+  T* const obase_p = outp + row0 * ldo + lane * CPL;
   if (lane * CPL + CPL <= ncols)
     asm volatile(TL_ASM_STORE
                  :
@@ -482,6 +553,76 @@
                    : [lo] "v"((unsigned)((uintptr_t)obase_p & 0xffffffffu)), [hi] "v"((unsigned)((uintptr_t)obase_p >> 32)),
                      [stride] "s"(stride_bytes), [n] "s"(nvalid)
                    : "memory", "scc", "s36", TL_ASM_BASE, TL_ASM_TOUCH);
+  }
+}
+
+template <int DBG, int MODE, typename T>
+__global__ void __launch_bounds__(TL_WAVES * 64) __attribute__((amdgpu_num_vgpr(TL_ASM_COMP)))
+spmm_tiled_kernel(const TlArgs<T> args_in_the_segment) {
+  extern __shared__ __attribute__((aligned(16))) char lds[];
+  int i = tl_next_item<T>(-1);
+  if (i < 0) return;
+
+  asm volatile(TL_ASM_ZERO ::: "memory", TL_CLOB_ACC);
+
+  unsigned par = 0, soff;
+  tl_srd_t srd;
+  tl_issue_tile0<DBG, T>(i, par, srd, soff);
+  int offreg = tl_load_offsets<T>(i, 0);
+  asm volatile("s_waitcnt vmcnt(0)" : "+v"(offreg) : : "memory");
+  __syncthreads();
+  tl_touch_first_lists<T>(offreg);
+
+  for (;;) {
+    const int inext = tl_next_item<T>(i);
+    int nextoff = 0;
+    bool pending = inext >= 0;
+    if (pending) tl_prefetch_offsets<T>(inext);
+    int t = 0, obase = 0;
+    for (;;) {
+      const auto A = tl_args<T>();
+      const int ntiles = A->ntiles;
+      if (t >= ntiles) break;
+      const int nfull = DBG == 2 ? 0 : A->nfull;
+      const bool has_partial = DBG != 2 && A->has_partial;
+      if ((t + 3 < ntiles ? t + 3 : ntiles) - obase > 63) {
+        obase = t;
+        offreg = tl_load_offsets<T>(i, obase);
+        asm volatile("s_waitcnt vmcnt(0)" : "+v"(offreg) : : "memory");
+      }
+      int te = ntiles - obase <= 63 ? ntiles : obase + 61;
+      if (has_partial && t < nfull - 1 && nfull - 1 < te) te = nfull - 1;
+      if (t < ntiles - 1 && ntiles - 1 < te) te = ntiles - 1;
+      if (pending && te >= ntiles - 1) {
+        nextoff = tl_load_offsets<T>(inext, 0);
+        asm volatile("s_waitcnt vmcnt(0)" : "+v"(nextoff) : : "memory");
+        pending = false;
+        tl_touch_first_lists<T>(nextoff);
+      }
+      if (has_partial && t == nfull - 1) {
+        int bx, by;
+        tl_item_map<T>(i, bx, by);
+        tl_issue_partial<T>(by, nfull, par);
+      }
+      if (t == ntiles - 1 && inext >= 0) tl_issue_tile0<DBG, T>(inext, (par + (unsigned)ntiles) & 1u, srd, soff);
+      auto o = [&](int tt) { return wave_bcast(offreg, (tt < ntiles ? tt : ntiles) - obase); };
+      const int o0 = o(t), o1 = o(t + 1), o2 = o(t + 2);
+      const int lane = tl_tid() & 63;
+      const int touch_lines = A->touch_lines;
+      const int toff = (lane < touch_lines ? lane : touch_lines - 1) * 64;
+      tl_phases<MODE>(A->stream, t, te, o0, o1, o2, offreg, obase, ntiles, nfull, toff, (int)0xfffffe00,
+                      (unsigned)uniform(tl_tid() >> 6) * 2048u,
+                      A->row_bytes * (2 * TL_WAVES),
+                      tl_voff<T>(), srd, soff, par);
+      t = te;
+    }
+    asm volatile("s_waitcnt vmcnt(0) lgkmcnt(0)" ::: "memory");
+    tl_store_item<T>(i);
+    if (inext < 0) break;
+    asm volatile(TL_ASM_ZERO ::: "memory", TL_CLOB_ACC);
+    par = (par + (unsigned)tl_args<T>()->ntiles) & 1u;
+    offreg = nextoff;
+    i = inext;
   }
 }
 
@@ -1404,18 +1545,60 @@
 
 static int tl_set_lds_once(const void* kern) { return set_max_dynamic_lds(kern, TL_LDS); }
 
+static int tl_resident_cap(int* cap) {
+  static std::mutex mu;
+  static int cus[64];
+  int dev = 0;
+  if (hipError_t e = hipGetDevice(&dev); e != hipSuccess) return (int)e;
+  if (dev < 0 || dev >= 64) return SPAMD_EINVAL;
+  std::lock_guard<std::mutex> lock(mu);
+  if (!cus[dev]) {
+    int n = 0;
+    if (hipError_t e = hipDeviceGetAttribute(&n, hipDeviceAttributeMultiprocessorCount, dev); e != hipSuccess) return (int)e;
+    cus[dev] = n < 8 ? 8 : n / 8 * 8;
+  }
+  *cap = cus[dev];
+  return 0;
+}
+
 template <typename T, typename KERN>
 static int tl_launch(KERN kern, int64_t M, int64_t K, int64_t N, const int* blocks, const int* blk_off, const T* b,
-                     int64_t ldb, T* out, int64_t ldo, int touch_lines, bool group_ends, int last_cols, hipStream_t s,
+                     int64_t ldb, T* out, int64_t ldo, int touch_lines, bool group_ends, int last_cols, int grid_cap8, hipStream_t s,
                      const int* rowmap = nullptr, int64_t map_groups = 0) {
   if (int rc = tl_set_lds_once(reinterpret_cast<const void*>(kern))) return rc;
   const int64_t blocks_n = (rowmap ? map_groups : tl_grid_groups(M)) / TL_WAVES;
   const int64_t npanels = N / TlFmt<T>::PANEL;
-  const int64_t grid = ceil_div(blocks_n, (int64_t)8) * 8 * (npanels > 1 ? ceil_div(npanels, (int64_t)2) * 2 : 1);
-  if (grid >= ((int64_t)1 << 31) || blocks_n >= ((int64_t)1 << 31)) return SPAMD_EINVAL;
-  hipLaunchKernelGGL(kern, dim3((unsigned)grid), dim3(TL_WAVES * 64), TL_LDS, s, M, K,
-                     (int)ceil_div(K, (int64_t)TL_KB), touch_lines | (group_ends ? 1 << 16 : 0), blocks, blk_off, b, ldb, out, ldo,
-                     last_cols, (int)npanels, (int)blocks_n, rowmap);
+  const int64_t items = ceil_div(blocks_n, (int64_t)8) * 8 * (npanels > 1 ? ceil_div(npanels, (int64_t)2) * 2 : 1);
+  if (items >= ((int64_t)1 << 31) || blocks_n >= ((int64_t)1 << 31)) return SPAMD_EINVAL;
+  int cap = 0;
+  if (grid_cap8 > 0) {
+    cap = grid_cap8 * 8;
+  } else {
+    if (int rc = tl_resident_cap(&cap)) return rc;
+    if (npanels > 1 && cap >= 16) cap = cap / 16 * 16;
+  }
+  const int64_t grid = items < cap ? items : cap;
+  TlArgs<T> a;
+  a.M = M;
+  a.K = K;
+  a.stream = blocks;
+  a.blk_off = blk_off;
+  a.b = b;
+  a.out = out;
+  a.ldo = ldo;
+  a.rowmap = rowmap;
+  a.row_bytes = (unsigned)(ldb * (int64_t)sizeof(T));
+  a.ntiles = (int)ceil_div(K, (int64_t)TL_KB);
+  a.nfull = (int)(K / TL_KB);
+  a.has_partial = (int64_t)a.nfull * TL_KB < K;
+  a.touch_lines = touch_lines;
+  a.ends = group_ends ? 1 : 0;
+  a.last_cols = last_cols;
+  a.npanels = (int)npanels;
+  a.nblocks = (int)blocks_n;
+  a.nitems = (int)items;
+  a.grid = (int)grid;
+  hipLaunchKernelGGL(kern, dim3((unsigned)grid), dim3(TL_WAVES * 64), TL_LDS, s, a);
   return launch_status();
 }
 
@@ -1456,23 +1639,24 @@
   int touch = (int)((flags >> 8) & 0xffu);
   if (touch == 0) touch = 12;
   if (touch > 64) touch = 64;
+  const int grid_cap8 = (int)((flags >> 24) & 0xffu);
   if (val_dtype == SPAMD_F64) {
     const double* bb = (const double*)b;
     double* oo = (double*)out;
-    return exact ? tl_launch<double>(&spmm_tiled_kernel<0, 5, double>, M, K, N, blocks, blk_off, bb, ldb, oo, ldo, touch, ends, last_cols, s, rowmap, map_groups)
-                 : tl_launch<double>(&spmm_tiled_kernel<0, 4, double>, M, K, N, blocks, blk_off, bb, ldb, oo, ldo, touch, ends, last_cols, s, rowmap, map_groups);
+    return exact ? tl_launch<double>(&spmm_tiled_kernel<0, 5, double>, M, K, N, blocks, blk_off, bb, ldb, oo, ldo, touch, ends, last_cols, grid_cap8, s, rowmap, map_groups)
+                 : tl_launch<double>(&spmm_tiled_kernel<0, 4, double>, M, K, N, blocks, blk_off, bb, ldb, oo, ldo, touch, ends, last_cols, grid_cap8, s, rowmap, map_groups);
   }
   const float* bb = (const float*)b;
   float* oo = (float*)out;
 #ifdef SPAMD_TUNING
   const char* dbg_env = getenv("SPAMD_TILED_DBG");
   const int dbg = dbg_env ? atoi(dbg_env) : 0;
-  if (dbg == 2) return tl_launch<float>(&spmm_tiled_kernel<2, 0, float>, M, K, N, blocks, blk_off, bb, ldb, oo, ldo, touch, ends, last_cols, s, rowmap, map_groups);
-  if (dbg == 5) return tl_launch<float>(&spmm_tiled_kernel<0, 1, float>, M, K, N, blocks, blk_off, bb, ldb, oo, ldo, touch, ends, last_cols, s, rowmap, map_groups);
-  if (dbg == 6) return tl_launch<float>(&spmm_tiled_kernel<0, 2, float>, M, K, N, blocks, blk_off, bb, ldb, oo, ldo, touch, ends, last_cols, s, rowmap, map_groups);
-  if (dbg == 7) return tl_launch<float>(&spmm_tiled_kernel<2, 2, float>, M, K, N, blocks, blk_off, bb, ldb, oo, ldo, touch, ends, last_cols, s, rowmap, map_groups);
+  if (dbg == 2) return tl_launch<float>(&spmm_tiled_kernel<2, 0, float>, M, K, N, blocks, blk_off, bb, ldb, oo, ldo, touch, ends, last_cols, grid_cap8, s, rowmap, map_groups);
+  if (dbg == 5) return tl_launch<float>(&spmm_tiled_kernel<0, 1, float>, M, K, N, blocks, blk_off, bb, ldb, oo, ldo, touch, ends, last_cols, grid_cap8, s, rowmap, map_groups);
+  if (dbg == 6) return tl_launch<float>(&spmm_tiled_kernel<0, 2, float>, M, K, N, blocks, blk_off, bb, ldb, oo, ldo, touch, ends, last_cols, grid_cap8, s, rowmap, map_groups);
+  if (dbg == 7) return tl_launch<float>(&spmm_tiled_kernel<2, 2, float>, M, K, N, blocks, blk_off, bb, ldb, oo, ldo, touch, ends, last_cols, grid_cap8, s, rowmap, map_groups);
 #endif
-  if (i32) return tl_launch<float>(&spmm_tiled_kernel<0, 6, float>, M, K, N, blocks, blk_off, bb, ldb, oo, ldo, touch, ends, last_cols, s, rowmap, map_groups);
-  return exact ? tl_launch<float>(&spmm_tiled_kernel<0, 3, float>, M, K, N, blocks, blk_off, bb, ldb, oo, ldo, touch, ends, last_cols, s, rowmap, map_groups)
-               : tl_launch<float>(&spmm_tiled_kernel<0, 0, float>, M, K, N, blocks, blk_off, bb, ldb, oo, ldo, touch, ends, last_cols, s, rowmap, map_groups);
-}
+  if (i32) return tl_launch<float>(&spmm_tiled_kernel<0, 6, float>, M, K, N, blocks, blk_off, bb, ldb, oo, ldo, touch, ends, last_cols, grid_cap8, s, rowmap, map_groups);
+  return exact ? tl_launch<float>(&spmm_tiled_kernel<0, 3, float>, M, K, N, blocks, blk_off, bb, ldb, oo, ldo, touch, ends, last_cols, grid_cap8, s, rowmap, map_groups)
+               : tl_launch<float>(&spmm_tiled_kernel<0, 0, float>, M, K, N, blocks, blk_off, bb, ldb, oo, ldo, touch, ends, last_cols, grid_cap8, s, rowmap, map_groups);
+}
diff --git a/sparse_amd/csrc/spmm_tiled_asm.inc b/sparse_amd/csrc/spmm_tiled_asm.inc
--- a/sparse_amd/csrc/spmm_tiled_asm.inc
+++ b/sparse_amd/csrc/spmm_tiled_asm.inc
@@ -13,11 +13,12 @@
   "s_mov_b32 s91, %[o0]\n\t" \
   "s_mov_b32 s92, %[o1]\n\t" \
   "s_mov_b32 s93, %[o2]\n\t" \
-  "s_add_u32 s88, s90, 1\n\t" \
+  "s_add_u32 s88, s90, %[par]\n\t" \
+  "s_add_u32 s89, s88, 1\n\t" \
+  "s_and_b32 s89, s89, 1\n\t" \
+  "s_lshl_b32 s89, s89, 10\n\t" \
+  "s_add_u32 s89, s89, %[m0wave]\n\t" \
   "s_and_b32 s88, s88, 1\n\t" \
-  "s_lshl_b32 s88, s88, 10\n\t" \
-  "s_add_u32 s89, s88, %[m0wave]\n\t" \
-  "s_and_b32 s88, s90, 1\n\t" \
   "s_lshl_b32 s88, s88, 10\n\t" \
   "v_or_b32 v22, s88, %[lane8]\n\t" \
   "s_lshl_b32 s36, s91, 6\n\t" \
@@ -1086,11 +1087,12 @@
   "s_mov_b32 s91, %[o0]\n\t" \
   "s_mov_b32 s92, %[o1]\n\t" \
   "s_mov_b32 s93, %[o2]\n\t" \
-  "s_add_u32 s88, s90, 1\n\t" \
+  "s_add_u32 s88, s90, %[par]\n\t" \
+  "s_add_u32 s89, s88, 1\n\t" \
+  "s_and_b32 s89, s89, 1\n\t" \
+  "s_lshl_b32 s89, s89, 10\n\t" \
+  "s_add_u32 s89, s89, %[m0wave]\n\t" \
   "s_and_b32 s88, s88, 1\n\t" \
-  "s_lshl_b32 s88, s88, 10\n\t" \
-  "s_add_u32 s89, s88, %[m0wave]\n\t" \
-  "s_and_b32 s88, s90, 1\n\t" \
   "s_lshl_b32 s88, s88, 10\n\t" \
   "v_or_b32 v22, s88, %[lane8]\n\t" \
   "s_lshl_b32 s36, s91, 6\n\t" \
@@ -2393,11 +2395,12 @@
   "s_mov_b32 s91, %[o0]\n\t" \
   "s_mov_b32 s92, %[o1]\n\t" \
   "s_mov_b32 s93, %[o2]\n\t" \
-  "s_add_u32 s88, s90, 1\n\t" \
+  "s_add_u32 s88, s90, %[par]\n\t" \
+  "s_add_u32 s89, s88, 1\n\t" \
+  "s_and_b32 s89, s89, 1\n\t" \
+  "s_lshl_b32 s89, s89, 10\n\t" \
+  "s_add_u32 s89, s89, %[m0wave]\n\t" \
   "s_and_b32 s88, s88, 1\n\t" \
-  "s_lshl_b32 s88, s88, 10\n\t" \
-  "s_add_u32 s89, s88, %[m0wave]\n\t" \
-  "s_and_b32 s88, s90, 1\n\t" \
   "s_lshl_b32 s88, s88, 10\n\t" \
   "v_or_b32 v22, s88, %[lane8]\n\t" \
   "s_lshl_b32 s36, s91, 6\n\t" \
@@ -2989,11 +2992,12 @@
   "s_mov_b32 s91, %[o0]\n\t" \
   "s_mov_b32 s92, %[o1]\n\t" \
   "s_mov_b32 s93, %[o2]\n\t" \
-  "s_add_u32 s88, s90, 1\n\t" \
+  "s_add_u32 s88, s90, %[par]\n\t" \
+  "s_add_u32 s89, s88, 1\n\t" \
+  "s_and_b32 s89, s89, 1\n\t" \
+  "s_lshl_b32 s89, s89, 10\n\t" \
+  "s_add_u32 s89, s89, %[m0wave]\n\t" \
   "s_and_b32 s88, s88, 1\n\t" \
-  "s_lshl_b32 s88, s88, 10\n\t" \
-  "s_add_u32 s89, s88, %[m0wave]\n\t" \
-  "s_and_b32 s88, s90, 1\n\t" \
   "s_lshl_b32 s88, s88, 10\n\t" \
   "v_or_b32 v22, s88, %[lane8]\n\t" \
   "s_lshl_b32 s36, s91, 6\n\t" \
@@ -3231,11 +3235,12 @@
   "s_mov_b32 s91, %[o0]\n\t" \
   "s_mov_b32 s92, %[o1]\n\t" \
   "s_mov_b32 s93, %[o2]\n\t" \
-  "s_add_u32 s88, s90, 1\n\t" \
+  "s_add_u32 s88, s90, %[par]\n\t" \
+  "s_add_u32 s89, s88, 1\n\t" \
+  "s_and_b32 s89, s89, 1\n\t" \
+  "s_lshl_b32 s89, s89, 10\n\t" \
+  "s_add_u32 s89, s89, %[m0wave]\n\t" \
   "s_and_b32 s88, s88, 1\n\t" \
-  "s_lshl_b32 s88, s88, 10\n\t" \
-  "s_add_u32 s89, s88, %[m0wave]\n\t" \
-  "s_and_b32 s88, s90, 1\n\t" \
   "s_lshl_b32 s88, s88, 10\n\t" \
   "v_or_b32 v22, s88, %[lane8]\n\t" \
   "s_lshl_b32 s36, s91, 6\n\t" \
@@ -4016,11 +4021,12 @@
   "s_mov_b32 s91, %[o0]\n\t" \
   "s_mov_b32 s92, %[o1]\n\t" \
   "s_mov_b32 s93, %[o2]\n\t" \
-  "s_add_u32 s88, s90, 1\n\t" \
+  "s_add_u32 s88, s90, %[par]\n\t" \
+  "s_add_u32 s89, s88, 1\n\t" \
+  "s_and_b32 s89, s89, 1\n\t" \
+  "s_lshl_b32 s89, s89, 10\n\t" \
+  "s_add_u32 s89, s89, %[m0wave]\n\t" \
   "s_and_b32 s88, s88, 1\n\t" \
-  "s_lshl_b32 s88, s88, 10\n\t" \
-  "s_add_u32 s89, s88, %[m0wave]\n\t" \
-  "s_and_b32 s88, s90, 1\n\t" \
   "s_lshl_b32 s88, s88, 10\n\t" \
   "v_or_b32 v22, s88, %[lane8]\n\t" \
   "s_lshl_b32 s36, s91, 6\n\t" \
@@ -4954,11 +4960,12 @@
   "s_mov_b32 s91, %[o0]\n\t" \
   "s_mov_b32 s92, %[o1]\n\t" \
   "s_mov_b32 s93, %[o2]\n\t" \
-  "s_add_u32 s88, s90, 1\n\t" \
+  "s_add_u32 s88, s90, %[par]\n\t" \
+  "s_add_u32 s89, s88, 1\n\t" \
+  "s_and_b32 s89, s89, 1\n\t" \
+  "s_lshl_b32 s89, s89, 10\n\t" \
+  "s_add_u32 s89, s89, %[m0wave]\n\t" \
   "s_and_b32 s88, s88, 1\n\t" \
-  "s_lshl_b32 s88, s88, 10\n\t" \
-  "s_add_u32 s89, s88, %[m0wave]\n\t" \
-  "s_and_b32 s88, s90, 1\n\t" \
   "s_lshl_b32 s88, s88, 10\n\t" \
   "v_or_b32 v22, s88, %[lane8]\n\t" \
   "s_lshl_b32 s36, s91, 6\n\t" \
```
